# ZJU-Robotics-Lab/GEM

Measured on AMD Instinct MI355X. Metric: fused points/sec into 600x600 grid; achieved HBM GB/s vs roofline, higher is better.
Workload: dtype f32

## Files before the change

gem_amd/build.py:

```python
from __future__ import annotations

import os
import shutil
import subprocess
from pathlib import Path

ROOT = Path(__file__).resolve().parent
CSRC = ROOT / "csrc"
LIBDIR = ROOT / "lib"
LIB = LIBDIR / "libgem_hip.so"

SOURCES = [CSRC / "gem_kernels.hip", CSRC / "gem_frame_lean.hip", CSRC / "gem_sort.hip", CSRC / "gem_capi.cpp", CSRC / "gem_capi_core.cpp", CSRC / "gem_capi_pipeline.cpp", CSRC / "gem_capi_comm.cpp",
           CSRC / "gem_clean.hip", CSRC / "gem_capi_clean.cpp", CSRC / "gem_local.hip", CSRC / "gem_capi_local.cpp",
           CSRC / "gem_voxel.hip", CSRC / "gem_capi_voxel.cpp", CSRC / "gem_global.hip", CSRC / "gem_capi_global.cpp",
           CSRC / "gem_compose.hip", CSRC / "gem_capi_compose.cpp", CSRC / "gem_costmap.hip", CSRC / "gem_capi_costmap.cpp",
           CSRC / "gem_octree.hip", CSRC / "gem_capi_octree.cpp", CSRC / "gem_depth.hip", CSRC / "gem_capi_depth.cpp",
           CSRC / "gem_history.hip", CSRC / "gem_capi_history.cpp",
           CSRC / "gem_footprint.hip", CSRC / "gem_capi_footprint.cpp", CSRC / "gem_inflate.hip", CSRC / "gem_capi_inflate.cpp",
           CSRC / "gem_mapgrid.hip", CSRC / "gem_capi_mapgrid.cpp", CSRC / "gem_critics.hip", CSRC / "gem_capi_critics.cpp",
           CSRC / "gem_trajgen.hip", CSRC / "gem_capi_trajgen.cpp", CSRC / "gem_navplan.hip", CSRC / "gem_capi_navplan.cpp",
           CSRC / "gem_frontier.hip", CSRC / "gem_capi_frontier.cpp", CSRC / "gem_obstacle.hip", CSRC / "gem_capi_obstacle.cpp"]
HEADERS = [CSRC / "gem_device.hpp", CSRC / "gem_kernels.hpp", CSRC / "gem_frame_lean.hpp", CSRC / "gem_frame_tile.hpp", CSRC / "gem_frame_sort.hpp", CSRC / "gem_wave.hpp", CSRC / "gem_compact.hpp", CSRC / "gem_transport.hpp", CSRC / "gem_hostcopy.hpp", CSRC / "gem_capi_internal.hpp", CSRC / "gem_plan.hpp", CSRC / "gem_clean.hpp", CSRC / "gem_local.hpp", CSRC / "gem_voxel.hpp", CSRC / "gem_global.hpp", CSRC / "gem_compose.hpp", CSRC / "gem_costmap.hpp", CSRC / "gem_lsd.hpp", CSRC / "gem_octree.hpp", CSRC / "gem_depth.hpp", CSRC / "gem_history.hpp", CSRC / "gem_footprint.hpp", CSRC / "gem_inflate.hpp", CSRC / "gem_mapgrid.hpp", CSRC / "gem_score_device.hpp", CSRC / "gem_critics.hpp", CSRC / "gem_trajgen.hpp", CSRC / "gem_sincos.hpp",
           CSRC / "gem_navplan.hpp", CSRC / "gem_navpath.hpp", CSRC / "gem_frontier.hpp", CSRC / "gem_costmap_host.hpp", CSRC / "gem_rounds.hpp", CSRC / "gem_tile_round.hpp", CSRC / "gem_obstacle.hpp", ROOT.parent / "include" / "gem_hip_frontier.h", ROOT.parent / "include" / "gem_hip_obstacle.h",
           ROOT.parent / "include" / "gem_hip_debug.h", ROOT.parent / "include" / "gem_hip.h", ROOT.parent / "include" / "gem_hip_history.h",
           ROOT.parent / "include" / "gem_hip_footprint.h", ROOT.parent / "include" / "gem_hip_inflate.h", ROOT.parent / "include" / "gem_hip_mapgrid.h",
           ROOT.parent / "include" / "gem_hip_critics.h", ROOT.parent / "include" / "gem_hip_trajgen.h", ROOT.parent / "include" / "gem_hip_navplan.h"]

FLAGS = [
    "--offload-arch=gfx950", "-O3", *(["-g"] if os.environ.get("GEM_DEBUG_BUILD") else []), "-std=c++17", "-ffp-contract=off", "-fPIC", "-shared",
    "-Wno-unused-value", "-Wno-unused-result",
    *os.environ.get("GEM_BUILD_DEFINES", "").split(),
]

SOURCE_FLAGS = {
    "gem_frame_lean.hip": ["-mllvm", "-amdgpu-kernarg-preload-count=14"],
}


def compile_flags(src: Path, extra=()) -> list:
    return [f for f in FLAGS if f != "-shared"] + list(extra) + SOURCE_FLAGS.get(src.name, [])


def flag_line(extra=()) -> str:
    own = "".join(f" [{name}: {' '.join(fl)}]" for name, fl in sorted(SOURCE_FLAGS.items()))
    return " ".join(compile_flags(Path("-"), extra)) + own


def hipcc_path() -> str:
    for cand in (os.environ.get("HIPCC"), shutil.which("hipcc"), "/opt/rocm/bin/hipcc"):
        if cand and os.path.exists(cand):
            return cand
    raise RuntimeError("hipcc not found (need ROCm to build libgem_hip.so)")


def is_stale() -> bool:
    if not LIB.exists():
        return True
    t = LIB.stat().st_mtime
    return any(p.stat().st_mtime > t for p in SOURCES + HEADERS)


def _stale(target: Path, deps) -> bool:
    if not target.exists():
        return True
    t = target.stat().st_mtime
    return any(p.stat().st_mtime > t for p in deps)


def build(force: bool = False, verbose: bool = False) -> Path:
    if not force and not is_stale():
        return LIB
    LIBDIR.mkdir(exist_ok=True)
    objdir = LIBDIR / "obj"
    objdir.mkdir(exist_ok=True)
    rocm = os.environ.get("ROCM_PATH", "/opt/rocm")
    tag = objdir / ".flags"
    line = flag_line()
    if not tag.exists() or tag.read_text() != line:
        force = True
    jobs = []
    for src in SOURCES:
        obj = objdir / (src.stem + ".o")
        if force or _stale(obj, [src] + HEADERS):
            cmd = [hipcc_path(), *compile_flags(src), "-c", str(src), "-o", str(obj)]
            if verbose:
                print(" ".join(cmd))
            jobs.append((src, subprocess.Popen(cmd, stdout=subprocess.PIPE, stderr=subprocess.STDOUT, text=True)))
    errors = []
    for src, proc in jobs:
        out, _ = proc.communicate()
        if proc.returncode != 0:
            errors.append(f"{src.name}: hipcc failed ({proc.returncode}):\n{out}")
    if errors:
        raise RuntimeError("\n".join(errors))
    tag.write_text(line)
    cmd = [hipcc_path(), "--offload-arch=gfx950", "-shared", "-fPIC", *[str(objdir / (s.stem + ".o")) for s in SOURCES], "-o", str(LIB),
           f"-L{rocm}/lib", "-lrccl", "-pthread", f"-Wl,-rpath,{rocm}/lib"]
    if verbose:
        print(" ".join(cmd))
    res = subprocess.run(cmd, capture_output=True, text=True)
    if res.returncode != 0:
        raise RuntimeError(f"hipcc (link) failed ({res.returncode}):\n{res.stdout}\n{res.stderr}")
    return LIB


def build_variant(name: str, defines: str, verbose: bool = False) -> Path:
    out = ROOT / "lib_ab" / name
    objdir = out / "obj"
    objdir.mkdir(parents=True, exist_ok=True)
    rocm = os.environ.get("ROCM_PATH", "/opt/rocm")
    jobs = []
    for src in SOURCES:
        obj = objdir / (src.stem + ".o")
        cmd = [hipcc_path(), *compile_flags(src, defines.split()), "-c", str(src), "-o", str(obj)]
        if verbose:
            print(" ".join(cmd))
        jobs.append((src, subprocess.Popen(cmd, stdout=subprocess.PIPE, stderr=subprocess.STDOUT, text=True)))
    for src, proc in jobs:
        o, _ = proc.communicate()
        if proc.returncode != 0:
            raise RuntimeError(f"{src.name}: hipcc failed ({proc.returncode}):\n{o}")
    lib = out / "libgem_hip.so"
    res = subprocess.run([hipcc_path(), "--offload-arch=gfx950", "-shared", "-fPIC", *[str(objdir / (s.stem + ".o")) for s in SOURCES], "-o", str(lib),
                          f"-L{rocm}/lib", "-lrccl", "-pthread", f"-Wl,-rpath,{rocm}/lib"], capture_output=True, text=True)
    if res.returncode != 0:
        raise RuntimeError(f"hipcc (link) failed ({res.returncode}):\n{res.stdout}\n{res.stderr}")
    return lib


if __name__ == "__main__":
    import sys
    if len(sys.argv) >= 3 and sys.argv[1] == "--variant":
        print(build_variant(sys.argv[2], " ".join(sys.argv[3:]), verbose=True))
    else:
        print(build(force=True, verbose=True))
```

gem_amd/csrc/gem_capi.cpp:

```cpp
#include "gem_capi_internal.hpp"
#include "gem_clean.hpp"
#include "gem_costmap.hpp"

namespace gemi {

int ensure_ray(gem_handle* h)
{
    if (h->ray.p) return GEM_OK;
    const int rc = ensure(h, h->ray, ((size_t)h->cells * 2 + 4) * sizeof(uint32_t));
    if (rc) return rc;
    GEM_HIP(h, hipMemsetAsync(static_cast<uint32_t*>(h->ray.p) + h->cells, 0, 4 * sizeof(uint32_t), h->stream));
    return GEM_OK;
}

static int queue_increment(gem_handle* h, float var_update)
{
    if (!(var_update >= 0.f)) h->floor_dirty = true;
    if (h->n_pending == kMaxPending) { int rc = flush_pending(h, false); if (rc) return rc; }
    h->pending[h->n_pending++] = var_update;
    return GEM_OK;
}

static int run_batch(gem_handle* h, int n_sweeps, const gem_frame_params* params, const float4* xyzi, const long long* offsets, const float* var_updates, bool caller_device)
{
// ... 74 lines not shown
                depth = src; color = colour ? src + dp.o_color : nullptr;
            }
            slot = reinterpret_cast<float4*>(d + dp.o_xyzi);
            uint32_t* rgb = colour ? reinterpret_cast<uint32_t*>(d + dp.o_rgb) : nullptr;
            if ((rc = depth_unproject(h, ds, depth, color, fe.kind == FrontEnd::clean ? fe.clean : nullptr, slot, rgb))) return release_half(h, half, rc);
            in.xyzi = slot; in.rgb = rgb;
            break;
        }
        }
        if (fe.kind == FrontEnd::clean && c.source != AddSource::depth) {
            const hipError_t e = launch_clean_mask(h->stream, in.xyzi, slot, c.n, fe.clean->mode, fe.clean->z_min, fe.clean->z_max);
            if (e != hipSuccess) return release_half(h, half, fail(h, GEM_ERR_HIP, "launch_clean_mask", e));
            in.xyzi = slot;
        }
        if (fe.kind == FrontEnd::voxel && (rc = voxel_front(h, fe.stages, fe.n_stages, c.n, in.xyzi, in.rgb, &in.xyzi, &in.rgb)))
            return release_half(h, half, rc);
        if (c.source == AddSource::aos || c.source == AddSource::depth || fe.kind != FrontEnd::none) h->main_reads_pb = true;
    }
    return release_half(h, half, run_pipeline(h, in));
}

}

extern "C" {

int gem_abi_version(void) { return GEM_ABI_VERSION; }

const char* gem_last_error(const gem_handle* h) { return h ? h->err.c_str() : g_create_error.c_str(); }

int gem_create(const gem_map_config* cfg, gem_handle** out)
{
    if (!cfg || !out) return fail(nullptr, GEM_ERR_INVALID, "gem_create: null argument");
    *out = nullptr;
    if (cfg->length <= 0 || cfg->length > 32768 || !(cfg->resolution > 0.f))
        return fail(nullptr, GEM_ERR_INVALID, "gem_create: bad length / resolution");
    int ndev = 0;
    hipError_t e = hipGetDeviceCount(&ndev);
    if (e != hipSuccess || ndev <= 0)
        return fail(nullptr, GEM_ERR_NO_DEVICE, "gem_create: no HIP device (libgem_hip has no CPU fallback)", e);
    int dev = cfg->device;
    if (dev < 0) { if (hipGetDevice(&dev) != hipSuccess) dev = 0; }
    if (dev >= ndev) return fail(nullptr, GEM_ERR_INVALID, "gem_create: device ordinal out of range");
    if ((e = hipSetDevice(dev)) != hipSuccess) return fail(nullptr, GEM_ERR_NO_DEVICE, "hipSetDevice", e);

    gem_handle* h = new gem_handle();
    h->device = dev;
    h->cfg = *cfg;
    if (!(h->cfg.variance_floor > 0.f)) h->cfg.variance_floor = 0.0001f;
    if (!(h->cfg.mahalanobis_threshold > 0.f)) h->cfg.mahalanobis_threshold = 5.f;
    h->L = cfg->length; h->cells = cfg->length * cfg->length; h->res = cfg->resolution;
    h->row0 = 0; h->row1 = h->L;
    if (cfg->strip_rows > 0) {
        if (cfg->strip_row0 < 0 || cfg->strip_row0 + cfg->strip_rows > h->L) { delete h; return fail(nullptr, GEM_ERR_INVALID, "gem_create: bad strip"); }
        h->row0 = cfg->strip_row0; h->row1 = cfg->strip_row0 + cfg->strip_rows;
    }
    h->fuse_variant = 12;
    h->ts = 0;

    auto bail = [&](const char* what, hipError_t err) { int rc = fail(nullptr, GEM_ERR_HIP, what, err); gem_destroy(h); return rc; };
    if ((e = acquire_streams(dev, h->streams)) != hipSuccess) return bail("hipStreamCreate", e);
    h->own_stream = h->streams.s[0]; h->bin_stream = h->streams.s[1]; h->bin_stream2 = h->streams.s[2]; h->tab_stream = h->streams.s[3];
    h->stream = h->own_stream;
    if ((e = hipEventCreateWithFlags(&h->copy_done, hipEventDisableTiming)) != hipSuccess) return bail("hipEventCreate", e);
    if ((e = hipEventCreateWithFlags(&h->switch_done, hipEventDisableTiming)) != hipSuccess) return bail("hipEventCreate", e);
    for (auto& b : h->pb) {
        if ((e = hipEventCreateWithFlags(&b.bin_done, kDeviceEventFlags)) != hipSuccess) return bail("hipEventCreate", e);
        if ((e = hipEventCreateWithFlags(&b.fuse_done, kDeviceEventFlags)) != hipSuccess) return bail("hipEventCreate", e);
    }
    void* base = nullptr;
    const size_t layer_bytes = ((size_t)h->cells * 4 + 255) & ~(size_t)255;
    if ((e = hipMalloc(&base, layer_bytes * GEM_LAYER_COUNT)) != hipSuccess) return bail("hipMalloc(layers)", e);
    unsigned char* b = static_cast<unsigned char*>(base);
    h->layers.elevation = reinterpret_cast<float*>(b + layer_bytes * GEM_LAYER_ELEVATION);
    h->layers.variance  = reinterpret_cast<float*>(b + layer_bytes * GEM_LAYER_VARIANCE);
    h->layers.intensity = reinterpret_cast<float*>(b + layer_bytes * GEM_LAYER_INTENSITY);
    h->layers.traver    = reinterpret_cast<float*>(b + layer_bytes * GEM_LAYER_TRAVER);
    h->layers.lowest    = reinterpret_cast<float*>(b + layer_bytes * GEM_LAYER_LOWEST);
    h->layers.colorR    = reinterpret_cast<int*>(b + layer_bytes * GEM_LAYER_COLOR_R);
    h->layers.colorG    = reinterpret_cast<int*>(b + layer_bytes * GEM_LAYER_COLOR_G);
    h->layers.colorB    = reinterpret_cast<int*>(b + layer_bytes * GEM_LAYER_COLOR_B);
    h->layers.rough     = reinterpret_cast<float*>(b + layer_bytes * GEM_LAYER_ROUGH);
    h->layers.slope     = reinterpret_cast<float*>(b + layer_bytes * GEM_LAYER_SLOPE);
    if ((e = hipMalloc(reinterpret_cast<void**>(&h->d_counters), 2 * sizeof(unsigned long long))) != hipSuccess) return bail("hipMalloc(counters)", e);
    if ((e = launch_init(h->stream, h->layers, h->cells, 1)) != hipSuccess) return bail("k_init", e);
    if ((e = hipStreamSynchronize(h->stream)) != hipSuccess) return bail("hipStreamSynchronize", e);
    h->floor_dirty = true;
    *out = h;
    return GEM_OK;
}

void gem_destroy(gem_handle* h)
{
    if (!h) return;
    hipSetDevice(h->device);
    if (h->step.valid) {
        h->step.valid = false;
        if (h->tp_x) h->tp_x->abort();
        if (h->tp_g) h->tp_g->abort();
    }
    if (h->stream) { settle(h); hipStreamSynchronize(h->stream); }
    if (h->bin_stream) hipStreamSynchronize(h->bin_stream);
    if (h->bin_stream2) hipStreamSynchronize(h->bin_stream2);
    if (h->tab_stream) hipStreamSynchronize(h->tab_stream);
    if (h->comm_stream) hipStreamSynchronize(h->comm_stream);
    if (h->gather_stream) hipStreamSynchronize(h->gather_stream);
    h->tp_g.reset(); h->tp_x.reset();
    release_comm_stream(h->device, h->comm_stream);
    release_comm_stream(h->device, h->gather_stream);
    for (hipEvent_t e : {h->ev_sorted, h->ev_exchanged, h->ev_bounds[0], h->ev_bounds[1], h->ev_walked[0], h->ev_walked[1], h->ev_vu[0], h->ev_vu[1],
                         h->ev_published[0], h->ev_published[1], h->ev_gathered[0], h->ev_gathered[1]}) if (e) hipEventDestroy(e);
    for (hipEvent_t e : h->ev_t) if (e) hipEventDestroy(e);
    fold_events(h);
    for (auto& ep : h->pool) { hipEventDestroy(ep.a); hipEventDestroy(ep.b); }
    local_free(h);
    global_free(h);
    costmap_free(h);
    history_free(h);
    octree_free(h);
    if (h->layers.elevation) hipFree(h->layers.elevation);
    if (h->d_counters) hipFree(h->d_counters);
    for (Arena* a : {&h->stage, &h->scratch, &h->dbg, &h->color, &h->ray, &h->sh_dev, &h->sh_recv_hv[0], &h->sh_recv_key[0], &h->sh_recv_rng[0],
                     &h->sh_recv_hv[1], &h->sh_recv_key[1], &h->sh_recv_rng[1], &h->sh_ranges, &h->published[0], &h->published[1],
                     &h->clean_cnt, &h->vox_state, &h->vox_hist, &h->vox_rec, &h->vox_tmp, &h->vox_out[0], &h->vox_out[1]}) if (a->p) hipFree(a->p);
    if (h->sh_host) hipHostFree(h->sh_host);
    if (h->form_seen) hipHostFree(h->form_seen);
    for (auto& b : h->pb) {
        for (Arena* a : {&b.rec, &b.srt, &b.seg, &b.flag, &b.gflag, &b.tables, &b.s_hv1, &b.s_hv2, &b.s_key1, &b.s_key2, &b.s_src1, &b.s_src2,
                         &b.s_cnt1, &b.s_cnt2, &b.s_misc, &b.s_ranges, &b.s_shard, &b.s_blkcnt}) if (a->p) hipFree(a->p);
        if (b.host_tables) hipHostFree(b.host_tables);
        if (b.tables_done) hipEventDestroy(b.tables_done);
        if (b.bin_done) hipEventDestroy(b.bin_done);
        if (b.fuse_done) hipEventDestroy(b.fuse_done);
    }
    if (h->copy_done) hipEventDestroy(h->copy_done);
    if (h->hstage) hipHostFree(h->hstage);
    for (auto& ev : h->ev_stage) if (ev) hipEventDestroy(ev);
    if (h->stage_read) hipEventDestroy(h->stage_read);
    for (auto& ev : h->ev_half) if (ev) hipEventDestroy(ev);
    if (h->switch_done) hipEventDestroy(h->switch_done);
    release_streams(h->device, h->streams);
    delete h;
}

int gem_set_stream(gem_handle* h, void* hip_stream)
{
    if (!h) return GEM_ERR_INVALID;
    std::lock_guard<std::mutex> lk(h->mu);
    hipSetDevice(h->device);
    { const int rcd = settle(h); if (rcd) return rcd; }
    GEM_HIP(h, hipStreamSynchronize(h->stream));
    if (h->bin_stream) GEM_HIP(h, hipStreamSynchronize(h->bin_stream));
    if (h->bin_stream2) GEM_HIP(h, hipStreamSynchronize(h->bin_stream2));
    h->stream = hip_stream ? static_cast<hipStream_t>(hip_stream) : h->own_stream;
    return GEM_OK;
}

int gem_wait_event(gem_handle* h, void* hip_event)
{
    if (!h || !hip_event) return GEM_ERR_INVALID;
    std::lock_guard<std::mutex> lk(h->mu);
    hipSetDevice(h->device);
    hipEvent_t ev = static_cast<hipEvent_t>(hip_event);
    GEM_HIP(h, hipStreamWaitEvent(h->stream, ev, 0));
    if (h->bin_stream) GEM_HIP(h, hipStreamWaitEvent(h->bin_stream, ev, 0));
    if (h->bin_stream2) GEM_HIP(h, hipStreamWaitEvent(h->bin_stream2, ev, 0));
    h->main_reads_pb = true;
    return GEM_OK;
}

int gem_synchronize(gem_handle* h)
{
    ApiRange api_range(h, "gem_synchronize");
    if (!h) return GEM_ERR_INVALID;
    std::lock_guard<std::mutex> lk(h->mu);
    hipSetDevice(h->device);
    { const int rcd = settle(h); if (rcd) return rcd; }
    GEM_HIP(h, hipStreamSynchronize(h->stream));
    return GEM_OK;
}

int gem_get_pose(gem_handle* h, float out_center[2], int out_start[2])
{
    if (!h) return GEM_ERR_INVALID;
    std::lock_guard<std::mutex> lk(h->mu);
    if (out_center) { out_center[0] = h->center[0]; out_center[1] = h->center[1]; }
    if (out_start) { out_start[0] = h->start[0]; out_start[1] = h->start[1]; }
    return GEM_OK;
}

int gem_move(gem_handle* h, const float position[3], float out_center[2], int out_start[2], float out_aligned_shift[2])
{
    ApiRange api_range(h, "gem_move");
    if (!h || !position) return GEM_ERR_INVALID;
    std::lock_guard<std::mutex> lk(h->mu);
    hipSetDevice(h->device);
    { const int rcd = settle(h); if (rcd) return rcd; }
    const int L = h->L; const float res = h->res;
    h->sensor_z = position[2];
    int shift[2]; float aligned[2];
    for (int i = 0; i < 2; ++i) {
        const float d = position[i] - h->center[i];
        shift[i] = static_cast<int>(static_cast<double>(d / res) + 0.5 * (d > 0 ? 1 : -1));
        aligned[i] = static_cast<float>(shift[i]) * res;
    }
    for (int i = 0; i < 2; ++i) {
        if (shift[i] != 0) {
            h->floor_dirty = true;
            if (shift[i] >= L || shift[i] <= -L) {
                GEM_HIP(h, launch_init(h->stream, h->layers, h->cells, 0));
            } else {
                const int sign = shift[i] > 0 ? 1 : -1;
                const int start_index = h->start[i] - (sign > 0 ? 1 : 0);
                const int end_index = start_index + sign - shift[i];
                const int n_cells = std::abs(shift[i]);
                int index = index_to_range(sign < 0 ? start_index : end_index, L);
                if (index + n_cells <= L) {
                    GEM_HIP(h, launch_clear_strip(h->stream, h->layers, L, index, n_cells, i == 0));
                } else {
                    const int first_n = L - index;
                    GEM_HIP(h, launch_clear_strip(h->stream, h->layers, L, index, first_n, i == 0));
                    GEM_HIP(h, launch_clear_strip(h->stream, h->layers, L, 0, n_cells - first_n, i == 0));
                }
            }
        }
        h->start[i] = index_to_range(h->start[i] - shift[i], L);
        const int p_index = static_cast<int>(roundf(h->center[i] / res));
        const int s_index = static_cast<int>(roundf(aligned[i] / res));
        h->center[i] = static_cast<float>(p_index + s_index) * res;
    }
    if (out_center) { out_center[0] = h->center[0]; out_center[1] = h->center[1]; }
    if (out_start) { out_start[0] = h->start[0]; out_start[1] = h->start[1]; }
    if (out_aligned_shift) { out_aligned_shift[0] = aligned[0]; out_aligned_shift[1] = aligned[1]; }
    return GEM_OK;
}

int gem_process_points(gem_handle* h, const gem_frame_params* p, int n, float* x, float* y, float* z,
                       const int* orig_index, int write_back_xyz,
                       int* map_index, float* var, float* x_ts, float* y_ts, float* z_ts)
{
    ApiRange api_range(h, "gem_process_points");
    if (!h || !p || n < 0 || (n > 0 && (!x || !y || !z))) return h ? fail(h, GEM_ERR_INVALID, "gem_process_points: bad argument") : GEM_ERR_INVALID;
    std::lock_guard<std::mutex> lk(h->mu);
    hipSetDevice(h->device);
    if (n == 0) return GEM_OK;
    const size_t N = (size_t)n, S = N * 4;
    int rc;
    FrameConst fc; fill_frame(h, p, fc);
    constexpr int kRange = 65536;
    const size_t SP = (S + 255) & ~(size_t)255;
    unsigned char* stg = S >= (64u << 10) ? host_stage(h, SP * 9) : nullptr;
    if (stg && (n + kRange - 1) / kRange <= gem_handle::kStageEvents) {
        { const int rcd = drain_staging(h); if (rcd) return rcd; }
        float* sx = reinterpret_cast<float*>(stg);            float* sy = reinterpret_cast<float*>(stg + SP);
        float* sz = reinterpret_cast<float*>(stg + 2 * SP);   int* sorig = reinterpret_cast<int*>(stg + 3 * SP);
        int* sidx = reinterpret_cast<int*>(stg + 4 * SP);     float* svar = reinterpret_cast<float*>(stg + 5 * SP);
        float* sxt = reinterpret_cast<float*>(stg + 6 * SP);  float* syt = reinterpret_cast<float*>(stg + 7 * SP);
        float* szt = reinterpret_cast<float*>(stg + 8 * SP);
        const int ranges = (n + kRange - 1) / kRange;
        auto out_of = [&](int c) {
            const int first = c * kRange, cnt = std::min(kRange, n - first);
            const size_t b = (size_t)cnt * 4;
            gem::CopySeg segs[8]; int ns = 0;
            if (map_index) segs[ns++] = {map_index + first, sidx + first, b};
            if (var)  segs[ns++] = {var + first, svar + first, b};
            if (x_ts) segs[ns++] = {x_ts + first, sxt + first, b};
            if (y_ts) segs[ns++] = {y_ts + first, syt + first, b};
            if (z_ts) segs[ns++] = {z_ts + first, szt + first, b};
            if (write_back_xyz) { segs[ns++] = {x + first, sx + first, b}; segs[ns++] = {y + first, sy + first, b}; segs[ns++] = {z + first, sz + first, b}; }
            gem::CopyPool::get().run(segs, ns, h->copy_threads);
        };
        for (int c = 0; c < ranges; ++c) {
            const int first = c * kRange, cnt = std::min(kRange, n - first);
            const size_t b = (size_t)cnt * 4;
            gem::CopySeg in[4] = {{sx + first, x + first, b}, {sy + first, y + first, b}, {sz + first, z + first, b}, {sorig + first, orig_index ? orig_index + first : nullptr, orig_index ? b : 0}};
            long long t0 = host_ns();
            gem::CopyPool::get().run(in, orig_index ? 4 : 3, h->copy_threads);
            long long t1 = host_ns();
            GEM_HIP(h, launch_project(h->stream, fc, first, cnt, sx + first, sy + first, sz + first, orig_index ? sorig + first : nullptr, write_back_xyz,
                                      sidx + first, svar + first, sxt + first, syt + first, szt + first));
            GEM_HIP(h, hipEventRecord(h->ev_stage[c], h->stream));
            long long t2 = host_ns();
            h->xfer_ns[0] += t1 - t0; h->xfer_ns[1] += t2 - t1;
            if (c > 0) {
                GEM_HIP(h, hipEventSynchronize(h->ev_stage[c - 1]));
                t0 = host_ns();
                out_of(c - 1);
                h->xfer_ns[3] += t0 - t2; h->xfer_ns[4] += host_ns() - t0;
            }
        }
        long long t0 = host_ns();
        GEM_HIP(h, hipEventSynchronize(h->ev_stage[ranges - 1]));
        long long t1 = host_ns();
        out_of(ranges - 1);
        h->xfer_ns[3] += t1 - t0; h->xfer_ns[4] += host_ns() - t1;
        return GEM_OK;
    }
    if ((rc = ensure(h, h->stage, stage_words_bytes(n, 9)))) return rc;
    unsigned char* d = static_cast<unsigned char*>(h->stage.p);
    float* dx = reinterpret_cast<float*>(d);           float* dy = reinterpret_cast<float*>(d + S);
    float* dz = reinterpret_cast<float*>(d + 2 * S);   int* dorig = reinterpret_cast<int*>(d + 3 * S);
    int* didx = reinterpret_cast<int*>(d + 4 * S);     float* dvar = reinterpret_cast<float*>(d + 5 * S);
    float* dxt = reinterpret_cast<float*>(d + 6 * S);  float* dyt = reinterpret_cast<float*>(d + 7 * S);
    float* dzt = reinterpret_cast<float*>(d + 8 * S);
    HostXfer up[4] = {{x, dx, S}, {y, dy, S}, {z, dz, S}, {const_cast<int*>(orig_index), dorig, S}};
    HostXfer down[8]; int nd = 0;
    if (map_index) down[nd++] = {map_index, didx, S};
    if (var)  down[nd++] = {var, dvar, S};
    if (x_ts) down[nd++] = {x_ts, dxt, S};
    if (y_ts) down[nd++] = {y_ts, dyt, S};
    if (z_ts) down[nd++] = {z_ts, dzt, S};
    if (write_back_xyz) { down[nd++] = {x, dx, S}; down[nd++] = {y, dy, S}; down[nd++] = {z, dz, S}; }
    if ((rc = upload_arrays(h, up, orig_index ? 4 : 3))) return rc;
    GEM_HIP(h, launch_project(h->stream, fc, 0, n, dx, dy, dz, orig_index ? dorig : nullptr, write_back_xyz, didx, dvar, dxt, dyt, dzt));
    if (nd) return download_arrays(h, down, nd, SP * 4);
    GEM_HIP(h, hipStreamSynchronize(h->stream));
    return GEM_OK;
}

int gem_fuse(gem_handle* h, int n, const int* index, const int* R, const int* G, const int* B,
             const float* intensity, const float* height, const float* var)
{
    ApiRange api_range(h, "gem_fuse");
    if (!h || n < 0 || (n > 0 && (!index || !height || !var))) return h ? fail(h, GEM_ERR_INVALID, "gem_fuse: bad argument") : GEM_ERR_INVALID;
    std::lock_guard<std::mutex> lk(h->mu);
    hipSetDevice(h->device);
    { const int rcs = shard_finish_locked(h); if (rcs) return rcs; }
    const bool attr = R && G && B && intensity;
    const size_t S = (size_t)n * 4;
    PassInput in; in.src = 1; in.n = n;
    int half = -1;
    if (n > 0) {
        int rc;
        const size_t P = (S + 255) & ~(size_t)255;
        if ((rc = ensure(h, h->stage, stage_words_bytes(n, 7)))) return rc;
        unsigned char* d = static_cast<unsigned char*>(h->stage.p);
        HostXfer up[7] = {{const_cast<int*>(index), d, S}, {const_cast<float*>(height), d + P, S}, {const_cast<float*>(var), d + 2 * P, S},
                          {const_cast<int*>(R), d + 3 * P, S}, {const_cast<int*>(G), d + 4 * P, S}, {const_cast<int*>(B), d + 5 * P, S},
                          {const_cast<float*>(intensity), d + 6 * P, S}};
        unsigned char* region = nullptr;
        if ((rc = upload_arrays(h, up, attr ? 7 : 3, true, &region, &half))) return rc;
        if (region) d = region;
        in.f_index = reinterpret_cast<const int*>(d); in.f_height = reinterpret_cast<const float*>(d + P);
        in.f_var = reinterpret_cast<const float*>(d + 2 * P);
        if (attr) {
            in.f_R = reinterpret_cast<const int*>(d + 3 * P); in.f_G = reinterpret_cast<const int*>(d + 4 * P);
            in.f_B = reinterpret_cast<const int*>(d + 5 * P); in.f_I = reinterpret_cast<const float*>(d + 6 * P);
        }
    }
    return release_half(h, half, run_pipeline(h, in));
}

// ... 2 lines not shown
    ApiRange api_range(h, "gem_add_device");
    if (!h || !p || n < 0 || (n > 0 && !d_xyzi)) return h ? fail(h, GEM_ERR_INVALID, "gem_add_device: bad argument") : GEM_ERR_INVALID;
    std::lock_guard<std::mutex> lk(h->mu);
    return add_cloud(h, p, {AddSource::device, n, d_xyzi, d_rgb, d_orig_index}, {});
}

int gem_add(gem_handle* h, const gem_frame_params* p, int n, const float* xyzi, const uint32_t* rgb, const int* orig_index)
{
    ApiRange api_range(h, "gem_add");
    if (!h || !p || n < 0 || (n > 0 && !xyzi)) return h ? fail(h, GEM_ERR_INVALID, "gem_add: bad argument") : GEM_ERR_INVALID;
    std::lock_guard<std::mutex> lk(h->mu);
    return add_cloud(h, p, {AddSource::host, n, xyzi, rgb, orig_index}, {});
}

int gem_add_batch(gem_handle* h, int n_sweeps, const gem_frame_params* params, const float* const* clouds, const int* counts, const float* var_updates)
{
    ApiRange api_range(h, "gem_add_batch");
    if (!h || n_sweeps <= 0 || !params || !clouds || !counts) return h ? fail(h, GEM_ERR_INVALID, "gem_add_batch: bad argument") : GEM_ERR_INVALID;
    std::lock_guard<std::mutex> lk(h->mu);
    hipSetDevice(h->device);
    { const int rcs = shard_finish_locked(h); if (rcs) return rcs; }
    std::vector<long long> offsets(n_sweeps + 1, 0);
    for (int s = 0; s < n_sweeps; ++s) {
        if (counts[s] < 0 || (counts[s] > 0 && !clouds[s])) return fail(h, GEM_ERR_INVALID, "gem_add_batch: bad sweep");
        offsets[s + 1] = offsets[s] + counts[s];
    }
    const long long N = offsets[n_sweeps];
    if (N >= (1ll << 31)) return fail(h, GEM_ERR_INVALID, "gem_add_batch: batch too large");
    int rc;
    if ((rc = ensure(h, h->stage, (size_t)N * 16 + 256))) return rc;
    unsigned char* d = static_cast<unsigned char*>(h->stage.p);
    if (N > 0) {
        std::vector<HostXfer> up;
        for (int s = 0; s < n_sweeps; ++s)
            if (counts[s] > 0) up.push_back({const_cast<float*>(clouds[s]), d + (size_t)offsets[s] * 16, (size_t)counts[s] * 16});
        size_t i0 = 0;
        while (i0 < up.size()) {
            size_t i1 = i0, bytes = 0;
            while (i1 < up.size() && (i1 == i0 || bytes + up[i1].bytes <= (64u << 20))) bytes += (up[i1++].bytes + 255) & ~(size_t)255;
            if ((rc = upload_arrays(h, up.data() + i0, (int)(i1 - i0), true))) return rc;
            i0 = i1;
        }
    }
    return run_batch(h, n_sweeps, params, reinterpret_cast<const float4*>(d), offsets.data(), var_updates, false);
}

int gem_add_aos(gem_handle* h, const gem_frame_params* p, int n, const void* points, int point_step,
                int off_x, int off_y, int off_z, int off_intensity, int off_rgb)
{
    ApiRange api_range(h, "gem_add_aos");
    if (!h || !p || n < 0 || (n > 0 && !points)) return h ? fail(h, GEM_ERR_INVALID, "gem_add_aos: bad argument") : GEM_ERR_INVALID;
    if (!aos_fields_ok(point_step, off_x, off_y, off_z, off_intensity, off_rgb))
        return fail(h, GEM_ERR_INVALID, "gem_add_aos: fields must be 4-byte aligned inside point_step");
    std::lock_guard<std::mutex> lk(h->mu);
    return add_cloud(h, p, {AddSource::aos, n, points, nullptr, nullptr, point_step, off_x, off_y, off_z, off_intensity, off_rgb}, {});
}

int gem_add_batch_device(gem_handle* h, int n_sweeps, const gem_frame_params* params, const void* d_xyzi,
                         const long long* offsets, const float* var_updates)
{
    ApiRange api_range(h, "gem_add_batch_device");
    if (!h || n_sweeps <= 0 || !params || !offsets) return h ? fail(h, GEM_ERR_INVALID, "gem_add_batch_device: bad argument") : GEM_ERR_INVALID;
    std::lock_guard<std::mutex> lk(h->mu);
    hipSetDevice(h->device);
    { const int rcs = shard_finish_locked(h); if (rcs) return rcs; }
    for (int s = 0; s < n_sweeps; ++s) if (offsets[s + 1] < offsets[s]) return fail(h, GEM_ERR_INVALID, "gem_add_batch_device: offsets not monotone");
    return run_batch(h, n_sweeps, params, static_cast<const float4*>(d_xyzi), offsets, var_updates, true);
}

int gem_mapvar_update(gem_handle* h, float var_update)
{
    ApiRange api_range(h, "gem_mapvar_update");
    if (!h) return GEM_ERR_INVALID;
    std::lock_guard<std::mutex> lk(h->mu);
    hipSetDevice(h->device);
    { const int rcs = shard_finish_locked(h); if (rcs) return rcs; }
    return queue_increment(h, var_update);
}

static void* layer_ptr(gem_handle* h, int layer)
{
    switch (layer) {
    case GEM_LAYER_ELEVATION: return h->layers.elevation;
    case GEM_LAYER_VARIANCE:  return h->layers.variance;
    case GEM_LAYER_INTENSITY: return h->layers.intensity;
    case GEM_LAYER_TRAVER:    return h->layers.traver;
    case GEM_LAYER_LOWEST:    return h->layers.lowest;
    case GEM_LAYER_COLOR_R:   return h->layers.colorR;
    case GEM_LAYER_COLOR_G:   return h->layers.colorG;
    case GEM_LAYER_COLOR_B:   return h->layers.colorB;
    case GEM_LAYER_ROUGH:     return h->layers.rough;
    case GEM_LAYER_SLOPE:     return h->layers.slope;
    default: return nullptr;
    }
}

int gem_get_layer(gem_handle* h, int layer, int layout, void* dst_host)
{
    ApiRange api_range(h, "gem_get_layer");
    if (!h || !dst_host) return GEM_ERR_INVALID;
    std::lock_guard<std::mutex> lk(h->mu);
    hipSetDevice(h->device);
    void* src = layer_ptr(h, layer);
    if (!src) return fail(h, GEM_ERR_INVALID, "gem_get_layer: bad layer");
    int rc = flush_pending(h, false);
    if (rc) return rc;
    const size_t bytes = (size_t)h->cells * 4;
    if (layout == GEM_LAYOUT_STORAGE_ROWMAJOR) {
        HostXfer down{dst_host, src, bytes};
        return download_arrays(h, &down, 1, 0);
    } else if (layout == GEM_LAYOUT_GRIDMAP_COLMAJOR_NAN) {
        if (layer == GEM_LAYER_LOWEST) return fail(h, GEM_ERR_INVALID, "gem_get_layer: the LOWEST layer is indexed by geographic cell, it has no grid_map layout");
        if ((rc = ensure(h, h->scratch, bytes))) return rc;
        const int is_int = layer >= GEM_LAYER_COLOR_R && layer <= GEM_LAYER_COLOR_B;
        GEM_HIP(h, launch_export_gridmap(h->stream, src, h->layers.elevation, static_cast<float*>(h->scratch.p), h->L, is_int));
        HostXfer down{dst_host, h->scratch.p, bytes};
        return download_arrays(h, &down, 1, 0);
    }
    return fail(h, GEM_ERR_INVALID, "gem_get_layer: bad layout");
}

int gem_set_layer(gem_handle* h, int layer, const void* src_host)
{
    if (!h || !src_host) return GEM_ERR_INVALID;
    std::lock_guard<std::mutex> lk(h->mu);
    hipSetDevice(h->device);
    void* dst = layer_ptr(h, layer);
    if (!dst) return fail(h, GEM_ERR_INVALID, "gem_set_layer: bad layer");
    int rc = flush_pending(h, false);
    if (rc) return rc;
    HostXfer up{const_cast<void*>(src_host), dst, (size_t)h->cells * 4};
    if ((rc = upload_arrays(h, &up, 1))) return rc;
    GEM_HIP(h, hipStreamSynchronize(h->stream));
    if (layer == GEM_LAYER_VARIANCE) h->floor_dirty = true;
    return GEM_OK;
}

int gem_layer_device_ptr(gem_handle* h, int layer, void** out_device_ptr)
{
    if (!h || !out_device_ptr) return GEM_ERR_INVALID;
    std::lock_guard<std::mutex> lk(h->mu);
    hipSetDevice(h->device);
    { const int rcd = flush_pending(h, false); if (rcd) return rcd; }
    *out_device_ptr = layer_ptr(h, layer);
    return *out_device_ptr ? GEM_OK : fail(h, GEM_ERR_INVALID, "gem_layer_device_ptr: bad layer");
}

int gem_map_optmove(gem_handle* h, const float opt_position[2], float height_update, float out_aligned_position[2])
{
    if (!h || !opt_position) return GEM_ERR_INVALID;
    std::lock_guard<std::mutex> lk(h->mu);
    hipSetDevice(h->device);
    { const int rcd = settle(h); if (rcd) return rcd; }
    for (int i = 0; i < 2; ++i) {
        const float d = opt_position[i] - h->center[i];
        const int shift = static_cast<int>(static_cast<double>(d / h->res) + 0.5 * (d > 0 ? 1 : -1));
        h->center[i] = h->center[i] + h->res * static_cast<float>(shift);
    }
    if (out_aligned_position) { out_aligned_position[0] = h->center[0]; out_aligned_position[1] = h->center[1]; }
    GEM_HIP(h, launch_update_height(h->stream, h->layers.elevation, h->cells, height_update));
    return GEM_OK;
}

int gem_map_closeloop(gem_handle* h, const float update_position[2], float height_update)
{
    if (!h || !update_position) return GEM_ERR_INVALID;
    std::lock_guard<std::mutex> lk(h->mu);
    hipSetDevice(h->device);
    { const int rcd = settle(h); if (rcd) return rcd; }
    for (int i = 0; i < 2; ++i) {
        const float d = update_position[i] - h->center[i];
        const int shift = static_cast<int>(static_cast<double>(d / h->res) + 0.5 * (d > 0 ? 1 : -1));
        const float aligned = static_cast<float>(shift) * h->res;
        const int p_index = static_cast<int>(roundf(h->center[i] / h->res));
        const int s_index = static_cast<int>(roundf(aligned / h->res));
        h->center[i] = static_cast<float>(p_index + s_index) * h->res;
    }
    GEM_HIP(h, launch_update_height(h->stream, h->layers.elevation, h->cells, height_update));
    return GEM_OK;
}

int gem_map_feature(gem_handle* h, float* elevation, float* variance, int* colorR, int* colorG, int* colorB,
                    float* rough, float* slope, float* traver, float* intensity)
{
    ApiRange api_range(h, "gem_map_feature");
    if (!h) return GEM_ERR_INVALID;
    std::lock_guard<std::mutex> lk(h->mu);
    hipSetDevice(h->device);
    int rc = flush_pending(h, false);
    if (rc) return rc;
    GEM_HIP(h, launch_map_feature(h->stream, h->layers.elevation, h->layers.traver, h->layers.rough, h->layers.slope,
                                  h->L, h->res, h->start[0], h->start[1], h->row0, h->row1));
    const size_t bytes = (size_t)h->cells * 4;
    struct { void* dst; const void* src; } out[9] = {
        {elevation, h->layers.elevation}, {variance, h->layers.variance}, {colorR, h->layers.colorR}, {colorG, h->layers.colorG},
        {colorB, h->layers.colorB}, {rough, h->layers.rough}, {slope, h->layers.slope}, {traver, h->layers.traver},
        {intensity, h->layers.intensity}};
    HostXfer down[9]; int nd = 0;
    for (auto& o : out) if (o.dst) down[nd++] = {o.dst, const_cast<void*>(o.src), bytes};
    return nd ? download_arrays(h, down, nd, 0) : GEM_OK;
}

int gem_show(gem_handle* h, double map_length, double resolution, const double position[2],
             float* visual, float* points_xyz, unsigned char* points_rgb, int* out_count, unsigned char* image_bgr)
{
    ApiRange api_range(h, "gem_show");
    if (!h) return GEM_ERR_INVALID;
    std::lock_guard<std::mutex> lk(h->mu);
    hipSetDevice(h->device);
    int rc = flush_pending(h, false);
    if (rc) return rc;
    const size_t cells = (size_t)h->cells, blocks = (cells + 1023) / 1024;
    const size_t o_cnt = 0, o_total = o_cnt + blocks * 4, o_vis = (o_total + 4 + 255) & ~(size_t)255, o_xyz = o_vis + cells * 36,
                 o_rgb = o_xyz + cells * 12, o_img = (o_rgb + cells * 3 + 255) & ~(size_t)255, total_bytes = o_img + cells * 3;
    if ((rc = ensure(h, h->scratch, total_bytes))) return rc;
    unsigned char* d = static_cast<unsigned char*>(h->scratch.p);
    const double res = resolution > 0.0 ? resolution : (double)h->res;
    const double len = map_length > 0.0 ? map_length : (double)h->L * res;
    const double px = position ? position[0] : (double)h->center[0], py = position ? position[1] : (double)h->center[1];
    if (image_bgr) GEM_HIP(h, hipMemsetAsync(d + o_img, 0, cells * 3, h->stream));
    GEM_HIP(h, launch_show(h->stream, h->layers, h->L, h->start[0], h->start[1], len, res, px, py, reinterpret_cast<uint32_t*>(d + o_cnt),
                           visual ? reinterpret_cast<float*>(d + o_vis) : nullptr, (points_xyz || points_rgb) ? reinterpret_cast<float*>(d + o_xyz) : nullptr,
                           points_rgb ? d + o_rgb : nullptr, image_bgr ? d + o_img : nullptr, reinterpret_cast<uint32_t*>(d + o_total)));
    uint32_t n = 0;
    {
        HostXfer down[3] = {{&n, d + o_total, 4}, {nullptr, nullptr, 0}, {nullptr, nullptr, 0}};
        int nd = 1;
        if (visual) down[nd++] = {visual, d + o_vis, cells * 36};
        if (image_bgr) down[nd++] = {image_bgr, d + o_img, cells * 3};
        if ((rc = download_arrays(h, down, nd, 0))) return rc;
    }
    if (n) {
        HostXfer down[2]; int nd = 0;
        if (points_xyz) down[nd++] = {points_xyz, d + o_xyz, (size_t)n * 12};
        if (points_rgb) down[nd++] = {points_rgb, d + o_rgb, (size_t)n * 3};
        if (nd && (rc = download_arrays(h, down, nd, 0))) return rc;
    }
    if (out_count) *out_count = (int)n;
    return GEM_OK;
}

static int colorize_device(gem_handle* h, const gem_camera* cam, int n, float* d_xyzi, const unsigned char* d_image, size_t stride, uint32_t* d_rgb)
{
    if (!cam || n < 0 || (n > 0 && (!d_xyzi || !d_image || !d_rgb))) return fail(h, GEM_ERR_INVALID, "gem_colorize: null argument");
    if (cam->width <= 0 || cam->height <= 0 || (long long)cam->width * cam->height > (1ll << 26))
        return fail(h, GEM_ERR_INVALID, "gem_colorize: image size out of range");
    if (stride == 0) stride = (size_t)cam->width * 3;
    if (stride < (size_t)cam->width * 3) return fail(h, GEM_ERR_INVALID, "gem_colorize: row stride below width * 3");
    if (n == 0) return GEM_OK;
    const long long pixels = (long long)cam->width * cam->height;
    SortArgs sa{};
    sa.id_bits = std::max(2, ceil_log2((int)std::min<long long>(pixels, 1ll << 30)));
    sa.n_passes = sa.id_bits <= 10 ? 1 : (sa.id_bits <= 20 ? 2 : 3);
    int shift = 0;
    for (int i = 0; i < sa.n_passes; ++i) {
        const int left = sa.n_passes - i;
        const int bits = i == sa.n_passes - 1 ? sa.id_bits - shift : (sa.id_bits - shift + left - 1) / left;
        sa.dshift[i] = shift; sa.dbits[i] = bits;
        sa.dbins[i] = i == sa.n_passes - 1 ? (int)((pixels - 1) >> shift) + 1 : 1 << bits;
        shift += bits;
    }
    const size_t N = (size_t)n, NC = (N + kSortChunkRecords - 1) / kSortChunkRecords;
    size_t o = 0;
    auto take = [&](size_t bytes) { const size_t at = o; o = (o + bytes + 255) & ~(size_t)255; return at; };
    const SortPlan sp = sort_plan(sa.n_passes, sa.dbins, n, NC, NC, 1, false, 0, false);
    const size_t o_hv1 = take(sp.hv), o_hv2 = take(sp.hv), o_key1 = take(sp.key), o_key2 = take(sp.key);
    const size_t o_cnt1 = take(sp.cnt1), o_cnt2 = take(sp.cnt2), o_misc = take(sp.misc);
    const size_t o_first = take((size_t)pixels * 4), o_pix = take(N * 4), o_link = take(N * 4);
    int rc;
    if ((rc = ensure(h, h->color, o))) return rc;
    unsigned char* d = static_cast<unsigned char*>(h->color.p);
    sa.n_sweeps = 1; sa.n = n; sa.xyzi = reinterpret_cast<const float4*>(d_xyzi);
    for (int k = 0; k < 12; ++k) sa.cam.P[k] = cam->lidar_to_image[k];
    sa.cam.width = cam->width; sa.cam.height = cam->height;
    sa.tiles_per_row = 1; sa.T = 1; sa.n_chunks1 = (int)NC; sa.chunk = kSortChunkRecords;
    bind_sort_buffers(sp, sa.n_passes, {d + o_hv1, d + o_hv2, d + o_key1, d + o_key2, nullptr, nullptr, d + o_cnt1, d + o_cnt2, d + o_misc}, sa);
    sa.odd_flag = nullptr;
    const LaunchEvents ev[9] = {};
    GEM_HIP(h, hipMemsetAsync(d + o_first, 0xff, (size_t)pixels * 4, h->stream));
    GEM_HIP(h, hipMemsetAsync(d + o_pix, 0xff, N * 4, h->stream));
    GEM_HIP(h, launch_sort(h->stream, sa, 3, false, ev));
    const bool final_b = (sa.n_passes & 1) != 0;
    ColorArgs ca{};
    ca.key = final_b ? sa.key_b : sa.key_a; ca.hv = final_b ? sa.hv_b : sa.hv_a; ca.total = sa.total;
    ca.first = reinterpret_cast<uint32_t*>(d + o_first); ca.pix = reinterpret_cast<uint32_t*>(d + o_pix); ca.link = reinterpret_cast<uint32_t*>(d + o_link);
    ca.n = n; ca.width = cam->width; ca.height = cam->height; ca.image = d_image; ca.stride = stride;
    ca.xyzi = reinterpret_cast<float4*>(d_xyzi); ca.rgb = d_rgb;
    GEM_HIP(h, launch_colorize(h->stream, ca));
    return GEM_OK;
}

int gem_colorize_device(gem_handle* h, const gem_camera* cam, int n, float* d_xyzi, const unsigned char* d_image_bgr, size_t row_stride,
                        uint32_t* d_rgb)
{
    ApiRange api_range(h, "gem_colorize_device");
    if (!h) return GEM_ERR_INVALID;
    std::lock_guard<std::mutex> lk(h->mu);
    hipSetDevice(h->device);
    return colorize_device(h, cam, n, d_xyzi, d_image_bgr, row_stride, d_rgb);
}

int gem_colorize(gem_handle* h, const gem_camera* cam, int n, float* xyzi, const unsigned char* image_bgr, size_t row_stride, uint32_t* rgb)
{
    ApiRange api_range(h, "gem_colorize");
    if (!h) return GEM_ERR_INVALID;
    std::lock_guard<std::mutex> lk(h->mu);
    hipSetDevice(h->device);
    if (!cam || n < 0 || (n > 0 && (!xyzi || !image_bgr || !rgb))) return fail(h, GEM_ERR_INVALID, "gem_colorize: null argument");
    if (cam->width <= 0 || cam->height <= 0) return fail(h, GEM_ERR_INVALID, "gem_colorize: image size out of range");
    if (n == 0) return GEM_OK;
    if (row_stride == 0) row_stride = (size_t)cam->width * 3;
    { const int rcd = settle(h); if (rcd) return rcd; }
    const size_t N = (size_t)n, b_xyzi = (N * 16 + 255) & ~(size_t)255, b_rgb = (N * 4 + 255) & ~(size_t)255, b_img = row_stride * cam->height;
    int rc;
    if ((rc = ensure(h, h->stage, b_xyzi + b_rgb + b_img))) return rc;
    unsigned char* d = static_cast<unsigned char*>(h->stage.p);
    HostXfer up[2] = {{xyzi, d, N * 16}, {const_cast<unsigned char*>(image_bgr), d + b_xyzi + b_rgb, b_img}};
    if ((rc = upload_arrays(h, up, 2))) return rc;
    if ((rc = colorize_device(h, cam, n, reinterpret_cast<float*>(d), d + b_xyzi + b_rgb, row_stride, reinterpret_cast<uint32_t*>(d + b_xyzi)))) return rc;
    HostXfer down[2] = {{xyzi, d, N * 16}, {rgb, d + b_xyzi, N * 4}};
    return download_arrays(h, down, 2, 0);
}

int gem_set_lowest_tracking(gem_handle* h, int enabled)
{
    if (!h) return GEM_ERR_INVALID;
    std::lock_guard<std::mutex> lk(h->mu);
    hipSetDevice(h->device);
    { const int rcd = settle(h); if (rcd) return rcd; }
    h->track_lowest = enabled != 0;
    return GEM_OK;
}

int gem_raytracing(gem_handle* h)
{
    ApiRange api_range(h, "gem_raytracing");
    if (!h) return GEM_ERR_INVALID;
    std::lock_guard<std::mutex> lk(h->mu);
    hipSetDevice(h->device);
    if (h->row0 != 0 || h->row1 != h->L) return fail(h, GEM_ERR_INVALID, "gem_raytracing: not available on a row-strip handle");
    int rc = flush_pending(h, false);
    if (rc) return rc;
    if ((rc = ensure_ray(h))) return rc;
    uint32_t* list = static_cast<uint32_t*>(h->ray.p);
    GEM_HIP(h, launch_raytracing(h->stream, h->layers, h->L, h->start[0], h->start[1], h->sensor_z, h->cfg.obstacle_threshold,
                                 h->row0, h->row1, list, list + h->cells, (int)(h->ray_calls++ & 1u), reinterpret_cast<float*>(list + h->cells + 4), h->ray_depth, h->ray_lanes));
    return GEM_OK;
}

int gem_set_timing(gem_handle* h, int enabled)
{
    if (!h) return GEM_ERR_INVALID;
    std::lock_guard<std::mutex> lk(h->mu);
    hipSetDevice(h->device);
    { const int rcd = settle(h); if (rcd) return rcd; }
    h->timing = enabled != 0;
    h->step_timed = h->timing && h->tp_x != nullptr && h->nranks > 1;
    return GEM_OK;
}

int gem_set_counting(gem_handle* h, int enabled)
{
    if (!h) return GEM_ERR_INVALID;
    std::lock_guard<std::mutex> lk(h->mu);
    hipSetDevice(h->device);
    { const int rcd = settle(h); if (rcd) return rcd; }
    h->counting = enabled != 0;
    return GEM_OK;
}

int gem_get_stats(gem_handle* h, gem_stats* out, int reset)
{
    if (!h || !out) return GEM_ERR_INVALID;
    std::lock_guard<std::mutex> lk(h->mu);
    hipSetDevice(h->device);
    { const int rcd = settle(h); if (rcd) return rcd; }
    GEM_HIP(h, hipStreamSynchronize(h->stream));
    fold_events(h);
    if (h->counting) {
        unsigned long long c[2] = {0, 0};
        GEM_HIP(h, hipMemcpy(c, h->d_counters, sizeof(c), hipMemcpyDeviceToHost));
        h->stats.points_binned = (long long)c[0];
        h->stats.cells_touched = (long long)c[1];
    }
    *out = h->stats;
    if (reset) { const long long pin = h->stats.points_in; h->stats = gem_stats{}; h->stats.points_in = pin; }
    return GEM_OK;
}

int gem_debug_set(gem_handle* h, const char* key, long long value)
{
    if (!h || !key) return GEM_ERR_INVALID;
    std::lock_guard<std::mutex> lk(h->mu);
    hipSetDevice(h->device);
    { const int rcd = settle(h); if (rcd) return rcd; }
    const std::string k(key);
    if (k == "fuse_variant")            { if (value < 10 || value > 12) return fail(h, GEM_ERR_INVALID, "fuse_variant: 10..12"); h->fuse_variant = (int)value; }
    else if (k == "tile_shift")         { if (value != 0 && value != 4 && value != 5) return fail(h, GEM_ERR_INVALID, "tile_shift: 0, 4 or 5"); h->ts = (int)value; }
    else if (k == "defer")              h->defer = value != 0;
    else if (k == "walk_always_wait")   h->walk_always_wait = value != 0;
    else if (k == "defer_walk")         { const int rcw = flush_walk(h); if (rcw) return rcw; h->defer_walk = value != 0; }
    else if (k == "dense_min")          { if (value < 0 || value > 0xffffffffll) return fail(h, GEM_ERR_INVALID, "dense_min: 0 .. 2^32 - 1"); h->dense_min = (unsigned)value; }
    else if (k == "dbg_sweep")          h->dbg_sweep = (int)value;
    else if (k == "dbg_frame")          h->dbg_frame = value != 0;
    else if (k == "frame_lean")         { if (value < 0 || value > 2) return fail(h, GEM_ERR_INVALID, "frame_lean: 0 (generic), 1 (lean) or 2 (the host picks)"); h->frame_lean = (int)value; }
    else if (k == "overlap")            h->overlap = value != 0;
    else if (k == "overlap_min_points") { if (value < 0) return fail(h, GEM_ERR_INVALID, "overlap_min_points: >= 0"); h->overlap_min_points = value; h->sort_overlap_min_points = value; }
    else if (k == "sort_path")          h->sort_path = value != 0;
    else if (k == "sort_min_points")    { if (value < 0) return fail(h, GEM_ERR_INVALID, "sort_min_points: >= 0"); h->sort_min_points = value; h->sort_min_points_batch = value; }
    else if (k == "walk_permute")       h->walk_permute = value != 0;
    else if (k == "trace")              h->trace = value != 0;
    else if (k == "stream_roles") {
        if (h->stream != h->own_stream) return fail(h, GEM_ERR_INVALID, "stream_roles: caller-provided stream in use");
        for (hipStream_t st : {h->own_stream, h->bin_stream, h->bin_stream2, h->tab_stream}) hipStreamSynchronize(st);
        const hipStream_t cur[4] = {h->own_stream, h->bin_stream, h->bin_stream2, h->tab_stream};
        const int d[4] = {(int)(value / 1000 % 10), (int)(value / 100 % 10), (int)(value / 10 % 10), (int)(value % 10)};
        bool seen[4] = {false, false, false, false};
        for (int i = 0; i < 4; ++i) { if (d[i] < 0 || d[i] > 3 || seen[d[i]]) return fail(h, GEM_ERR_INVALID, "stream_roles: not a permutation of 0123"); seen[d[i]] = true; }
        h->own_stream = cur[d[0]]; h->bin_stream = cur[d[1]]; h->bin_stream2 = cur[d[2]]; h->tab_stream = cur[d[3]];
        h->stream = h->own_stream;
    }
    else if (k == "sort_ring")          { if (value < 2 || value > 4) return fail(h, GEM_ERR_INVALID, "sort_ring: 2..4"); h->sort_ring = (int)value; }
    else if (k == "sort_streams")       { if (value != 1 && value != 2) return fail(h, GEM_ERR_INVALID, "sort_streams: 1 or 2"); h->sort_streams = (int)value; }
    else if (k == "sort_passes")        { if (value < 0 || value > 3) return fail(h, GEM_ERR_INVALID, "sort_passes: 0..3"); h->sort_passes = (int)value; }
    else if (k == "rank_by_ballot")     h->rank_by_ballot = value != 0;
    else if (k == "lane_sort")          h->lane_sort = value != 0;
    else if (k == "plain_loop")         h->plain_loop = value != 0;
    else if (k == "cache_tables")       h->cache_tables = value != 0;
    else if (k == "light_fast")         h->light_fast = value != 0;
    else if (k == "walk_lds_pad")       { if (value < 0 || value > 100 * 1024) return fail(h, GEM_ERR_INVALID, "walk_lds_pad: 0 .. 102400 bytes"); h->walk_lds_pad = (int)value; }
    else if (k == "ride_events")        { if (value < 0 || value > 1) return fail(h, GEM_ERR_INVALID, "ride_events: 0 or 1"); h->ride_events = value != 0; }
    else if (k == "roctx")              { if (value != 0 && !roctx_load()) return fail(h, GEM_ERR_INVALID, "roctx: no ROCm marker library (librocprofiler-sdk-roctx / libroctx64) to load"); h->roctx = value != 0; }
    else if (k == "download_groups")    { if (value < 1 || value > 14) return fail(h, GEM_ERR_INVALID, "download_groups: 1 .. 14"); h->download_groups = (int)value; }
    else if (k == "copy_threads")       { if (value < 0 || value > gem::CopyPool::kMaxThreads) return fail(h, GEM_ERR_INVALID, "copy_threads: 0 (the runtime's pageable path) .. 16"); h->copy_threads = (int)value; }
    else if (k == "fuse_count")         { if (value < 0 || value > 2) return fail(h, GEM_ERR_INVALID, "fuse_count: 0 (never), 1 (small passes) or 2 (always)"); h->fuse_count = (int)value; }
    else if (k == "sort_chunk")         { if (value != 0 && value != kSortChunkSmall && value != kSortChunkRecords) return fail(h, GEM_ERR_INVALID, "sort_chunk: 0 (by pass), 1024 or 4096"); h->sort_chunk = (int)value; }
    else if (k == "walk_prio")          { if (value < 0 || value > (1 << 30)) return fail(h, GEM_ERR_INVALID, "walk_prio: 0 (off) or a record count"); h->walk_prio = (int)value; }
    else if (k == "blk_batch")          { if (value != 0 && value != 512 && value != 2048) return fail(h, GEM_ERR_INVALID, "blk_batch: 0 (by pass), 512 or 2048"); h->blk_batch = (int)value; }
    else if (k == "few_bins")           { if (value < -1 || value > 64) return fail(h, GEM_ERR_INVALID, "few_bins: -1 (one ballot per digit bit), 0 (by pass), 1..64"); h->few_bins = (int)value; }
    else if (k == "ray_depth")          { if (value != 4 && value != 8) return fail(h, GEM_ERR_INVALID, "ray_depth: 4 or 8"); h->ray_depth = (int)value; }
    else if (k == "ray_lanes")          { if (value != 1 && value != 4 && value != 8 && value != 16) return fail(h, GEM_ERR_INVALID, "ray_lanes: 1, 4, 8 or 16"); h->ray_lanes = (int)value; }
    else if (k == "fast_laser")         h->fast_laser = value != 0;
    else if (k == "sort_form")          { if (value < 0 || value > 2) return fail(h, GEM_ERR_INVALID, "sort_form: 0 (by pass), 1 (cell-sorted), 2 (block-sorted)"); h->sort_form = (int)value; }
    else if (k == "history_cull")       { if (value < 0 || value > 1) return fail(h, GEM_ERR_INVALID, "history_cull: 0 or 1"); h->history_cull = value != 0; }
    else if (k == "obstacle_direct")    { if (value < 0 || value > 1) return fail(h, GEM_ERR_INVALID, "obstacle_direct: 0 or 1"); h->obstacle_direct = value != 0; }
    else if (k == "nav_chunk")          { if (value < 0 || value > (1 << 20)) return fail(h, GEM_ERR_INVALID, "nav_chunk: 0 (tiles_x + tiles_y) or 1 .. 2^20 rounds"); h->nav_chunk = (int)value; }
    else if (k == "front_chunk")        { if (value < 0 || value > (1 << 20)) return fail(h, GEM_ERR_INVALID, "front_chunk: 0 (tiles_x + tiles_y) or 1 .. 2^20 rounds"); h->front_chunk = (int)value; }
    else return fail(h, GEM_ERR_INVALID, "gem_debug_set: unknown key");
    return GEM_OK;
}

int gem_debug_get(gem_handle* h, const char* key, long long* out)
{
    if (!h || !key || !out) return GEM_ERR_INVALID;
    std::lock_guard<std::mutex> lk(h->mu);
    const std::string k(key);
    if (k == "arena_allocations") *out = h->arena_allocations;
    else if (k == "hstage_allocations") *out = h->hstage_allocations;
    else if (k == "copy_threads") *out = h->copy_threads;
    else if (k == "xfer_upload_memcpy_ns") *out = h->xfer_ns[0];
    else if (k == "xfer_upload_enqueue_ns") *out = h->xfer_ns[1];
    else if (k == "xfer_download_enqueue_ns") *out = h->xfer_ns[2];
    else if (k == "xfer_download_wait_ns") *out = h->xfer_ns[3];
    else if (k == "xfer_download_memcpy_ns") *out = h->xfer_ns[4];
    else if (k == "sort_fallbacks") *out = h->sort_fallbacks;
    else if (k == "compose_far_points") *out = h->compose.far_points;
    else if (k == "compose_sum_ns") *out = h->compose.sum_ns;
    else if (k == "walks_unwaited") *out = h->walks_unwaited;
    else if (k == "frame_lean_launches") *out = h->frame_lean_launches;
    else if (k == "frame_generic_launches") *out = h->frame_generic_launches;
    else if (k == "frame_form_seen") *out = h->form_seen ? (long long)*static_cast<volatile const uint32_t*>(h->form_seen) : 0;
    else if (k == "walks_left") *out = h->walks_left;
    else if (k == "history_cull") *out = h->history_cull ? 1 : 0;
    else if (k == "obstacle_direct") *out = h->obstacle_direct ? 1 : 0;
    else if (k == "nav_chunk") *out = h->nav_chunk;
    else if (k == "front_chunk") *out = h->front_chunk;
    else if (k == "history_blocks") *out = h->history.enabled ? cost_mark_blocks(h->history.len) : 0;
    else if (k == "history_blocks_culled") { hipSetDevice(h->device); return history_blocks_culled(h, out); }
    else if (k == "step_pending") *out = h->step.valid ? 1 : 0;
    else if (k == "step_exchange_bytes_out") *out = h->xbytes_out;
    else if (k == "step_exchange_bytes_in") *out = h->xbytes_in;
    else if (k == "gather_bytes_out") *out = h->gbytes_out;
    else if (k == "gather_bytes_in") *out = h->gbytes_in;
    else if (k.rfind("step_", 0) == 0) {
        int a = -1, b = -1;
        if (k == "step_exchange_ns") { a = 2; b = 3; }
        else if (k == "step_walk_ns") { a = 4; b = 5; }
        else if (k == "step_publish_ns") { a = 6; b = 7; }
        else if (k == "step_gather_ns") { a = 7; b = 8; }
        else if (k == "step_exchange_to_walk_ns") { a = 3; b = 4; }
        else return fail(h, GEM_ERR_INVALID, "gem_debug_get: unknown key");
        hipSetDevice(h->device);
        float ms = 0.f;
        if (!h->ev_t[a] || hipEventElapsedTime(&ms, h->ev_t[a], h->ev_t[b]) != hipSuccess) { (void)hipGetLastError(); *out = -(1ll << 62); return GEM_OK; }
        *out = (long long)((double)ms * 1e6);
    }
    else return fail(h, GEM_ERR_INVALID, "gem_debug_get: unknown key");
    return GEM_OK;
}

int gem_debug_fuse_stamps(gem_handle* h, int enable, unsigned long long* out, int max_tiles)
{
    if (!h) return GEM_ERR_INVALID;
    std::lock_guard<std::mutex> lk(h->mu);
    hipSetDevice(h->device);
    { const int rcd = settle(h); if (rcd) return rcd; }
    h->dbg_on = enable != 0;
    if (out && h->dbg.p) {
        GEM_HIP(h, hipStreamSynchronize(h->stream));
        const int rows = h->dbg_rows ? h->dbg_rows : h->T;
        const int n = max_tiles < rows ? max_tiles : rows;
        GEM_HIP(h, hipMemcpy(out, h->dbg.p, (size_t)n * 16 * 8, hipMemcpyDeviceToHost));
        return n;
    }
    return 0;
}

int gem_comm_unique_id(void* out_128_bytes)
{
    if (!out_128_bytes) return GEM_ERR_INVALID;
    static_assert(sizeof(ncclUniqueId) == 128, "ncclUniqueId is 128 bytes");
    ncclUniqueId id;
    if (ncclGetUniqueId(&id) != ncclSuccess) return GEM_ERR_COMM;
    memcpy(out_128_bytes, &id, sizeof(id));
    return GEM_OK;
}

}
```

gem_amd/csrc/gem_capi_comm.cpp:

```cpp
#include "gem_capi_internal.hpp"


namespace gemi {

int comm_attach(gem_handle* h, int nranks, int rank, bool tile_strips)
{
    h->nranks = nranks; h->rank = rank; h->tile_strips = tile_strips;
    if (!h->comm_stream) {
        GEM_HIP(h, acquire_comm_stream(h->device, &h->comm_stream));
        GEM_HIP(h, acquire_comm_stream(h->device, &h->gather_stream));
        for (hipEvent_t* e : {&h->ev_sorted, &h->ev_exchanged, &h->ev_bounds[0], &h->ev_bounds[1], &h->ev_walked[0], &h->ev_walked[1], &h->ev_vu[0], &h->ev_vu[1],
                              &h->ev_published[0], &h->ev_published[1], &h->ev_gathered[0], &h->ev_gathered[1]})
            GEM_HIP(h, hipEventCreateWithFlags(e, hipEventDisableTiming));
        for (hipEvent_t& e : h->ev_t) GEM_HIP(h, hipEventCreate(&e));
    }
    const int tile_rows = (h->L + 31) / 32;
    for (int k = 0; k <= nranks; ++k)
        h->strip_row[k] = tile_strips ? std::min(h->L, 32 * (int)((long long)tile_rows * k / nranks)) : (int)((long long)h->L * k / nranks);
    h->row0 = h->strip_row[rank]; h->row1 = h->strip_row[rank + 1];
    if (nranks > 1)
        for (int g = 0; g < 2; ++g) { const int rc = ensure(h, h->published[g], (size_t)(h->row1 - h->row0) * h->L * 4 * 6 + 256); if (rc) return rc; }
    return GEM_OK;
}

int comm_init_common(gem_handle* h, const void* unique_id_128_bytes, int nranks, int rank, bool tile_strips)
{
    if (!h || !unique_id_128_bytes || nranks <= 0 || nranks > kMaxRanks || rank < 0 || rank >= nranks) return GEM_ERR_INVALID;
    std::lock_guard<std::mutex> lk(h->mu);
    hipSetDevice(h->device);
    { const int rcd = settle(h); if (rcd) return rcd; }
    if (h->tp_x) return fail(h, GEM_ERR_COMM, "gem_comm_init: the handle already joined a communicator");
    ncclUniqueId id;
    memcpy(&id, unique_id_128_bytes, sizeof(id));
    std::unique_ptr<RcclTransport> x(new RcclTransport()), g(new RcclTransport());
    ncclResult_t r = ncclCommInitRank(&x->comm, nranks, id, rank);
    if (r != ncclSuccess) { x->comm = nullptr; return fail(h, GEM_ERR_COMM, ncclGetErrorString(r)); }
    r = ncclCommSplit(x->comm, 0, rank, &g->comm, nullptr);
    if (r != ncclSuccess || !g->comm) { g->comm = x->comm; g->owns = false; }
    x->nranks = g->nranks = nranks; x->rank = g->rank = rank;
    h->tp_x = std::move(x); h->tp_g = std::move(g);
    return comm_attach(h, nranks, rank, tile_strips);
}

}

extern "C" {

int gem_comm_init(gem_handle* h, const void* unique_id_128_bytes, int nranks, int rank)
{
    return comm_init_common(h, unique_id_128_bytes, nranks, rank, false);
}

int gem_comm_init_tiles(gem_handle* h, const void* unique_id_128_bytes, int nranks, int rank)
{
    return comm_init_common(h, unique_id_128_bytes, nranks, rank, true);
}

int gem_comm_init_loopback(gem_handle* h, long long world_id, int nranks, int rank, int tile_strips)
{
    if (!h || nranks <= 0 || nranks > kMaxRanks || rank < 0 || rank >= nranks) return GEM_ERR_INVALID;
    std::lock_guard<std::mutex> lk(h->mu);
    hipSetDevice(h->device);
    { const int rcd = settle(h); if (rcd) return rcd; }
    if (h->tp_x) return fail(h, GEM_ERR_COMM, "gem_comm_init_loopback: the handle already joined a communicator");
    std::string why;
    std::shared_ptr<LoopWorld> w = loop_world(world_id, nranks, &why);
    if (!w) return fail(h, GEM_ERR_COMM, why.c_str());
    std::unique_ptr<LoopbackTransport> x(new LoopbackTransport()), g(new LoopbackTransport());
    if (!x->join(w, 0, rank)) return fail(h, GEM_ERR_COMM, x->err.c_str());
    if (!g->join(w, 1, rank)) return fail(h, GEM_ERR_COMM, g->err.c_str());
    h->tp_x = std::move(x); h->tp_g = std::move(g);
    return comm_attach(h, nranks, rank, tile_strips != 0);
}

int gem_get_strip(gem_handle* h, int* out_row0, int* out_row1)
{
    if (!h) return GEM_ERR_INVALID;
    std::lock_guard<std::mutex> lk(h->mu);
    if (out_row0) *out_row0 = h->row0;
    if (out_row1) *out_row1 = h->row1;
    return GEM_OK;
}

}

namespace gemi {

int gather_layers_locked(gem_handle* h, int with_attributes)
{
    const int W = h->nranks;
    if (W == 1) return GEM_OK;
    const int nl = with_attributes ? 6 : 2;
    void* ptrs[6] = {h->layers.elevation, h->layers.variance, h->layers.intensity, h->layers.colorR, h->layers.colorG, h->layers.colorB};
    const size_t own = (size_t)(h->strip_row[h->rank + 1] - h->strip_row[h->rank]) * h->L;
    const int g = (int)(h->gather_seq++ & 1u);
    int rc;
    if ((rc = ensure(h, h->published[g], own * 4 * 6 + 256))) return step_abort(h, rc);
    unsigned char* pub = static_cast<unsigned char*>(h->published[g].p);
    if (h->gathered_recorded[g]) GEM_HIP_STEP(h, hipStreamWaitEvent(h->stream, h->ev_gathered[g], 0));
    if (h->step_timed) GEM_HIP_STEP(h, hipEventRecord(h->ev_t[6], h->stream));
    if (own)
        for (int l = 0; l < nl; ++l)
            GEM_HIP_STEP(h, hipMemcpyAsync(pub + (size_t)l * own * 4, static_cast<unsigned char*>(ptrs[l]) + (size_t)h->strip_row[h->rank] * h->L * 4, own * 4,
                                      hipMemcpyDeviceToDevice, h->stream));
    GEM_HIP_STEP(h, hipEventRecord(h->ev_published[g], h->stream));
    GEM_HIP_STEP(h, hipStreamWaitEvent(h->gather_stream, h->ev_published[g], 0));
    if (h->step_timed) GEM_HIP_STEP(h, hipEventRecord(h->ev_t[7], h->gather_stream));
    Transport& tp = *h->tp_g;
    bool ok = tp.group_begin();
    h->gbytes_out = h->gbytes_in = 0;
    for (int p = 0; p < W && ok; ++p) {
        if (p == h->rank) continue;
        const size_t theirs = (size_t)(h->strip_row[p + 1] - h->strip_row[p]) * h->L;
        h->gbytes_out += 4ll * (long long)own * nl; h->gbytes_in += 4ll * (long long)theirs * nl;
        for (int l = 0; l < nl && ok; ++l) {
            if (own) ok = tp.send(pub + (size_t)l * own * 4, own, p, h->gather_stream);
            if (ok && theirs) ok = tp.recv(static_cast<unsigned char*>(ptrs[l]) + (size_t)h->strip_row[p] * h->L * 4, theirs, p, h->gather_stream);
        }
    }
    ok = tp.group_end(h->gather_stream) && ok;
    if (!ok) return step_abort(h, fail(h, GEM_ERR_COMM, tp.err.c_str()));
    if (h->step_timed) GEM_HIP_STEP(h, hipEventRecord(h->ev_t[8], h->gather_stream));
    GEM_HIP_STEP(h, hipEventRecord(h->ev_gathered[g], h->gather_stream));
    h->gathered_recorded[g] = true;
    h->gather_outstanding[g] = true;
    return GEM_OK;
}

}

extern "C" {

int gem_allgather_layers(gem_handle* h, int with_attributes)
{
    ApiRange api_range(h, "gem_allgather_layers");
    if (!h) return GEM_ERR_INVALID;
    std::lock_guard<std::mutex> lk(h->mu);
    hipSetDevice(h->device);
    if (!h->tp_g) return fail(h, GEM_ERR_COMM, "gem_allgather_layers: gem_comm_init not called");
    if (h->step.valid) {
        h->step.gather = true; h->step.gather_attrs = with_attributes;
        return GEM_OK;
    }
    { const int rc = flush_local(h); if (rc) return rc; }
    if (h->n_pending) { const int rc = flush_pending(h, false); if (rc) return rc; }
    return gather_layers_locked(h, with_attributes);
}

}

namespace gemi {

int ensure_shard_tables(gem_handle* h, size_t blocks)
{
    if (!h->sh_host) GEM_HIP(h, hipHostMalloc(&h->sh_host, kShardHostBytes, hipHostMallocDefault));
    int rc = ensure(h, h->sh_dev, kShardDevBytes);
    return rc ? rc : ensure(h, h->sh_ranges, blocks * sizeof(uint2));
}

int shard_checks(gem_handle* h, int n_global_sweeps, SortGeometry* geo)
{
    if (h->track_lowest) return fail(h, GEM_ERR_INVALID, "sharded path: lowest tracking is not supported (use the replicated path)");
    *geo = sort_geometry(h, n_global_sweeps, true);
    if (!geo->ok) return fail(h, GEM_ERR_INVALID, "sharded path: map or batch too large for the record key");
    return GEM_OK;
}

int shard_sort_locked(gem_handle* h, int n_local_sweeps, const gem_frame_params* params, const void* d_xyzi, const long long* offsets,
                             int first_global_sweep, int n_global_sweeps, int first_point_in_sweep, int nstrips, const int* strip_rows,
                             uint32_t* out_bounds, const void** out_d_hv, const void** out_d_key, const void** out_d_ranges, bool bounds_stay_on_device)
{
    if (first_point_in_sweep < 0) return fail(h, GEM_ERR_INVALID, "gem_shard_sort_device: negative first_point_in_sweep");
// ... 295 lines not shown
```

gem_amd/csrc/gem_capi_core.cpp:

```cpp
#include "gem_capi_internal.hpp"

#include <cfloat>
#include <dlfcn.h>

namespace gemi {

thread_local std::string g_create_error;

namespace {
typedef int (*roctx_push_fn)(const char*);
typedef int (*roctx_pop_fn)();
std::once_flag g_roctx_once;
roctx_push_fn g_roctx_push = nullptr;
roctx_pop_fn g_roctx_pop = nullptr;
}

bool roctx_load()
{
    std::call_once(g_roctx_once, [] {
        for (const char* lib : {"librocprofiler-sdk-roctx.so", "librocprofiler-sdk-roctx.so.1", "libroctx64.so", "libroctx64.so.4"}) {
            void* so = dlopen(lib, RTLD_NOW | RTLD_GLOBAL);
            if (!so) continue;
            g_roctx_push = reinterpret_cast<roctx_push_fn>(dlsym(so, "roctxRangePushA"));
            g_roctx_pop = reinterpret_cast<roctx_pop_fn>(dlsym(so, "roctxRangePop"));
            if (g_roctx_push && g_roctx_pop) return;
            g_roctx_push = nullptr; g_roctx_pop = nullptr;
        }
    });
    return g_roctx_push != nullptr;
}
void roctx_push(const char* name) { if (g_roctx_push) g_roctx_push(name); }
void roctx_pop() { if (g_roctx_pop) g_roctx_pop(); }
ApiRange::ApiRange(const gem_handle* h, const char* name) : on(h && h->roctx && g_roctx_push != nullptr) { if (on) roctx_push(name); }

int fail(gem_handle* h, int code, const char* what, hipError_t e)
{
    char buf[512];
    if (e != hipSuccess) snprintf(buf, sizeof(buf), "%s: %s", what, hipGetErrorString(e));
    else snprintf(buf, sizeof(buf), "%s", what);
    if (h) h->err = buf; else g_create_error = buf;
    return code;
}

int ensure(gem_handle* h, Arena& a, size_t bytes)
{
    if (bytes <= a.cap) return GEM_OK;
    GEM_HIP(h, hipStreamSynchronize(h->stream));
    if (h->bin_stream) GEM_HIP(h, hipStreamSynchronize(h->bin_stream));
    if (h->bin_stream2) GEM_HIP(h, hipStreamSynchronize(h->bin_stream2));
    if (h->tab_stream) GEM_HIP(h, hipStreamSynchronize(h->tab_stream));
    if (h->comm_stream) GEM_HIP(h, hipStreamSynchronize(h->comm_stream));
    if (h->gather_stream) GEM_HIP(h, hipStreamSynchronize(h->gather_stream));
    if (a.p) GEM_HIP(h, hipFree(a.p));
    a.p = nullptr; a.cap = 0;
    size_t want = bytes + bytes / 4 + 4096;
    hipError_t e = hipMalloc(&a.p, want);
    if (e != hipSuccess) return fail(h, GEM_ERR_NOMEM, "hipMalloc(arena)", e);
    a.cap = want;
    ++h->arena_allocations;
    return GEM_OK;
}

int ensure_zeroed(gem_handle* h, Arena& a, size_t bytes)
{
    if (bytes <= a.cap) return GEM_OK;
    const int rc = ensure(h, a, bytes);
    if (rc) return rc;
    GEM_HIP(h, hipMemsetAsync(a.p, 0, a.cap, h->stream));
    GEM_HIP(h, hipStreamSynchronize(h->stream));
    return GEM_OK;
}

unsigned char* host_stage(gem_handle* h, size_t bytes)
{
    if (h->copy_threads <= 0 || h->hstage_failed || bytes > h->hstage_max) return nullptr;
    if (bytes > h->hstage_cap) {
        if (h->hstage) {
            if (hipStreamSynchronize(h->stream) != hipSuccess) return nullptr;
            h->stage_read_pending = false; h->half_pending[0] = h->half_pending[1] = false;
            hipHostFree(h->hstage); h->hstage = nullptr; h->hstage_cap = 0;
        }
        const size_t want = bytes + bytes / 4 + 4096;
        if (hipHostMalloc(&h->hstage, want, hipHostMallocDefault) != hipSuccess) { (void)hipGetLastError(); h->hstage = nullptr; h->hstage_failed = true; return nullptr; }
        h->hstage_cap = want;
        ++h->hstage_allocations;
    }
    for (auto& ev : h->ev_stage) if (!ev && hipEventCreateWithFlags(&ev, hipEventDisableTiming) != hipSuccess) { ev = nullptr; return nullptr; }
    if (!h->stage_read && hipEventCreateWithFlags(&h->stage_read, hipEventDisableTiming) != hipSuccess) { h->stage_read = nullptr; return nullptr; }
    return static_cast<unsigned char*>(h->hstage);
}

int drain_staging(gem_handle* h)
{
    for (int p = 0; p < 2; ++p) if (h->half_pending[p]) { GEM_HIP(h, hipEventSynchronize(h->ev_half[p])); h->half_pending[p] = false; }
    if (h->stage_read_pending) { GEM_HIP(h, hipEventSynchronize(h->stage_read)); h->stage_read_pending = false; }
    return GEM_OK;
}

int upload_arrays(gem_handle* h, const HostXfer* x, int n, bool defer_ok, unsigned char** zero_copy_region, int* zero_copy_half)
{
    if (zero_copy_region) *zero_copy_region = nullptr;
    size_t total = 0;
    for (int i = 0; i < n; ++i) total += (x[i].bytes + 255) & ~(size_t)255;
    unsigned char* stg = (total >= (128u << 10) && total < (16u << 20)) ? host_stage(h, defer_ok ? 2 * total + 512 : total) : nullptr;
    if (!stg) {
        for (int i = 0; i < n; ++i) if (x[i].bytes) GEM_HIP(h, hipMemcpyAsync(x[i].dev, x[i].host, x[i].bytes, hipMemcpyHostToDevice, h->stream));
        GEM_HIP(h, hipEventRecord(h->copy_done, h->stream));
        GEM_HIP(h, hipEventSynchronize(h->copy_done));
        return GEM_OK;
    }
    int par = -1;
    if (defer_ok) {
        for (auto& ev : h->ev_half) if (!ev) GEM_HIP(h, hipEventCreateWithFlags(&ev, hipEventDisableTiming));
        if (h->stage_read_pending) { GEM_HIP(h, hipEventSynchronize(h->stage_read)); h->stage_read_pending = false; }
        par = (int)(h->stage_par++ & 1u);
        const size_t half_at = (h->hstage_cap / 2) & ~(size_t)255;
        if (h->half_pending[par]) { GEM_HIP(h, hipEventSynchronize(h->ev_half[par])); h->half_pending[par] = false; }
        if (half_at < total || h->hstage_cap - half_at < total) { const int rcd = drain_staging(h); if (rcd) return rcd; par = 0; }
        else stg += (size_t)par * half_at;
        if (zero_copy_region) {
            size_t off = 0;
            gem::CopySeg segs[16]; int ns = 0;
            const long long t0 = host_ns();
            for (int i = 0; i < n; ++i) {
                if (x[i].bytes) segs[ns++] = {stg + off, x[i].host, x[i].bytes};
                off += (x[i].bytes + 255) & ~(size_t)255;
                if (ns == 16 || i == n - 1) { if (ns) gem::CopyPool::get().run(segs, ns, h->copy_threads); ns = 0; }
            }
            h->xfer_ns[0] += host_ns() - t0;
            *zero_copy_region = stg; *zero_copy_half = par;
            return GEM_OK;
        }
    } else { const int rcd = drain_staging(h); if (rcd) return rcd; }
    auto pad = [](size_t b) { return (b + 255) & ~(size_t)255; };
    size_t off = 0;
    for (int i = 0; i < n;) {
        int e = i + 1;
        size_t len = pad(x[i].bytes);
        while (e < n && e - i < 16 && static_cast<unsigned char*>(x[e].dev) == static_cast<unsigned char*>(x[i].dev) + len) len += pad(x[e++].bytes);
        const size_t real_len = len - pad(x[e - 1].bytes) + x[e - 1].bytes;
        const size_t group = pad(len <= (8u << 20) ? (par >= 0 ? len : std::max<size_t>(len / 2, 512u << 10)) : (4u << 20));
        for (size_t a = 0; a < len; a += group) {
            const size_t b = std::min(len, a + group);
            gem::CopySeg segs[16]; int ns = 0;
            size_t m_off = 0;
            for (int m = i; m < e; ++m) {
                const size_t lo = std::max(a, m_off), hi = std::min(b, m_off + x[m].bytes);
                if (lo < hi) segs[ns++] = {stg + off + lo, static_cast<const unsigned char*>(x[m].host) + (lo - m_off), hi - lo};
                m_off += pad(x[m].bytes);
            }
            const long long t0 = host_ns();
            gem::CopyPool::get().run(segs, ns, h->copy_threads);
            const long long t1 = host_ns();
            const size_t b_real = std::min(b, real_len);
            if (a < b_real) GEM_HIP(h, hipMemcpyAsync(static_cast<unsigned char*>(x[i].dev) + a, stg + off + a, b_real - a, hipMemcpyHostToDevice, h->stream));
            h->xfer_ns[0] += t1 - t0; h->xfer_ns[1] += host_ns() - t1;
        }
        off += len;
        i = e;
    }
    if (par >= 0) {
        GEM_HIP(h, hipEventRecord(h->ev_half[par], h->stream));
        h->half_pending[par] = true;
        h->main_reads_pb = true;
        return GEM_OK;
    }
    GEM_HIP(h, hipEventRecord(h->stage_read, h->stream));
    GEM_HIP(h, hipEventSynchronize(h->stage_read));
    h->stage_read_pending = false;
    return GEM_OK;
}

CloudLayout cloud_layout(long long n, bool rgb, bool orig)
{
    const size_t S = (size_t)n * 4, P = (S + 255) & ~(size_t)255, P4 = (S * 4 + 255) & ~(size_t)255;
    CloudLayout l;
    l.rgb = P4;
    l.orig = P4 + (rgb ? P : 0);
    l.bytes = l.orig + (orig ? P : 0);
    return l;
}

int stage_cloud(gem_handle* h, long long n, const float* xyzi, const uint32_t* rgb, const int* orig, StagedCloud& out)
{
    const CloudLayout l = cloud_layout(n, rgb, orig);
    int rc;
    if ((rc = ensure(h, h->stage, l.bytes))) return rc;
    unsigned char* d = static_cast<unsigned char*>(h->stage.p);
    const size_t S = (size_t)n * 4;
    HostXfer up[3] = {{const_cast<float*>(xyzi), d, S * 4}};
    int nu = 1;
    if (rgb) up[nu++] = {const_cast<uint32_t*>(rgb), d + l.rgb, S};
    if (orig) up[nu++] = {const_cast<int*>(orig), d + l.orig, S};
    unsigned char* region = nullptr;
    out.half = -1;
    if ((rc = upload_arrays(h, up, nu, true, &region, &out.half))) return rc;
    const unsigned char* src = region ? region : d;
    out.xyzi = reinterpret_cast<const float4*>(src);
    out.rgb = rgb ? reinterpret_cast<const uint32_t*>(src + l.rgb) : nullptr;
    out.orig = orig ? reinterpret_cast<const int*>(src + l.orig) : nullptr;
    out.arena_xyzi = reinterpret_cast<float4*>(d);
    return GEM_OK;
}

int release_half(gem_handle* h, int half, int rc)
{
    if (half < 0) return rc;
    const hipError_t e = hipEventRecord(h->ev_half[half], h->stream);
    if (e != hipSuccess && rc == GEM_OK) rc = fail(h, GEM_ERR_HIP, "hipEventRecord(staging half)", e);
    h->half_pending[half] = true;
    return rc;
}

float to_float_rn(double v)
{
    const double lim = (double)FLT_MAX + std::ldexp(1.0, 103);
    if (v >= lim) return INFINITY;
    if (v <= -lim) return -INFINITY;
    return static_cast<float>(v);
}

int download_arrays(gem_handle* h, const HostXfer* x, int n, size_t stage_off)
{
    size_t total = 0;
    for (int i = 0; i < n; ++i) total += (x[i].bytes + 255) & ~(size_t)255;
    stage_off = (stage_off + 255) & ~(size_t)255;
    { const int rcd = drain_staging(h); if (rcd) return rcd; }
    unsigned char* stg = total >= (128u << 10) ? host_stage(h, stage_off + total) : nullptr;
    if (!stg) {
        for (int i = 0; i < n; ++i) if (x[i].bytes) GEM_HIP(h, hipMemcpyAsync(x[i].host, x[i].dev, x[i].bytes, hipMemcpyDeviceToHost, h->stream));
        GEM_HIP(h, hipStreamSynchronize(h->stream));
        h->stage_read_pending = false;
        return GEM_OK;
    }
    stg += stage_off;
    const long long t_begin = host_ns();
    const size_t n_groups = (size_t)std::max(1, std::min(h->download_groups, (int)gem_handle::kStageEvents - 10));
    size_t group = std::max<size_t>(n_groups > 8 ? (256u << 10) : (768u << 10), (total + n_groups - 1) / n_groups);
    group = (group + 255) & ~(size_t)255;
    gem::CopySeg segs[gem_handle::kStageEvents][kCopyListMax];
    int nseg[gem_handle::kStageEvents] = {};
    int ng = 0;
    {
        CopyList cl; cl.n = 0;
        size_t in_group = 0, off = 0;
        auto flush = [&]() -> int {
            if (!cl.n) return GEM_OK;
            if (ng == gem_handle::kStageEvents) return fail(h, GEM_ERR_INVALID, "download_arrays: too many groups");
            GEM_HIP(h, launch_copy_list(h->stream, cl));
            GEM_HIP(h, hipEventRecord(h->ev_stage[ng], h->stream));
            nseg[ng++] = cl.n; cl.n = 0; in_group = 0;
            return GEM_OK;
        };
        for (int i = 0; i < n; ++i) {
            for (size_t o = 0; o < x[i].bytes;) {
                const size_t b = std::min(x[i].bytes - o, group - in_group);
                cl.piece[cl.n] = {stg + off + o, static_cast<const unsigned char*>(x[i].dev) + o, b};
                segs[ng][cl.n] = {static_cast<unsigned char*>(x[i].host) + o, stg + off + o, b};
                ++cl.n; in_group += b; o += b;
                if (in_group >= group || cl.n == kCopyListMax) { const int rcf = flush(); if (rcf) return rcf; }
            }
            off += (x[i].bytes + 255) & ~(size_t)255;
        }
        { const int rcf = flush(); if (rcf) return rcf; }
    }
    long long t0 = host_ns();
    h->xfer_ns[2] += t0 - t_begin;
    for (int g = 0; g < ng; ++g) {
        GEM_HIP(h, hipEventSynchronize(h->ev_stage[g]));
        const long long t1 = host_ns();
        gem::CopyPool::get().run(segs[g], nseg[g], h->copy_threads);
        const long long t2 = host_ns();
        h->xfer_ns[3] += t1 - t0; h->xfer_ns[4] += t2 - t1; t0 = t2;
    }
    h->stage_read_pending = false;
    return GEM_OK;
}

void fill_frame(const gem_handle* h, const gem_frame_params* p, FrameConst& f)
{
    memset(&f, 0, sizeof(f));
    if (p) {
        for (int i = 0; i < 12; ++i) f.T[i] = p->T[i];
        f.lower = p->lower; f.upper = p->upper;
        f.lower_f = (float)p->lower; if ((double)f.lower_f > p->lower) f.lower_f = nextafterf(f.lower_f, -INFINITY);
        f.upper_f = (float)p->upper; if ((double)f.upper_f < p->upper) f.upper_f = nextafterf(f.upper_f, INFINITY);
        for (int i = 0; i < 8; ++i) f.sp[i] = p->sensor_params[i];
        for (int i = 0; i < 3; ++i) { f.Js[i] = p->sensor_jacobian[i]; f.P[i] = p->P_mul_C_BM_T[i]; }
        for (int i = 0; i < 9; ++i) { f.Q[i] = p->rotation_variance[i]; f.C[i] = p->C_SB_T[i]; f.Bs[i] = p->B_r_BS_skew[i]; }
        f.filter_on = p->filter.enabled;
        f.fbx = p->filter.box_x; f.fby = p->filter.box_y; f.fband = p->filter.band_y; f.fplane = p->filter.plane_y;
        f.model = p->sensor_model;
        f.orig_width = p->original_width;
    }
    f.cx = h->center[0]; f.cy = h->center[1];
    f.sx = h->start[0];  f.sy = h->start[1];
    f.L = h->L; f.res = h->res;
    f.row0 = h->row0; f.row1 = h->row1;
    f.beam_a = (float)f.sp[1]; f.beam_c = (float)f.sp[2];
    f.t2 = 0.f; f.fast_laser = 0;
    if (p && f.model == GEM_MODEL_LASER && h->fast_laser) {
        const float min_r = (float)f.sp[0], vn = min_r * min_r;
        const float c0 = f.Js[0] * 0.0f, c1 = f.Js[1] * 0.0f, c2 = f.Js[2] * vn;
        const float b2 = c0 + (c1 + c2);
        const float t2 = b2 * f.Js[2];
        auto small = [](float v, float bound) { return std::isfinite(v) && std::fabs(v) <= bound; };
        bool ok = t2 > 0.f && std::isfinite(t2) && small(f.beam_a, 1e6f) && small(f.beam_c, 1e6f);
        for (int i = 0; i < 9; ++i) ok = ok && f.Q[i] == 0.0f && small(f.C[i], 1e6f) && small(f.Bs[i], 1e6f);
        for (int i = 0; i < 3; ++i) ok = ok && small(f.Js[i], 1e6f) && small(f.P[i], 1e6f);
        for (int i = 0; i < 3 && ok; ++i)
            for (int j = i; j < 3; ++j) {
                double d = 0.0;
                for (int k = 0; k < 3; ++k) d += (double)f.T[4 * i + k] * (double)f.T[4 * j + k];
                ok = ok && std::fabs(d - (i == j ? 1.0 : 0.0)) <= 0.01;
            }
        for (int i = 0; i < 3; ++i) ok = ok && small(f.T[4 * i + 3], 1e9f);
        ok = ok && std::isfinite(f.lower) && std::isfinite(f.upper) && std::fabs(f.lower) <= 1e9 && std::fabs(f.upper) <= 1e9;
        ok = ok && small(f.cx, 1e9f) && small(f.cy, 1e9f) && (double)f.L * (double)f.res <= 1e9;
        ok = ok && f.res >= 9.5367431640625e-7f && f.res <= 1048576.0f && f.L >= 2;
        if (ok) { f.t2 = t2; f.fast_laser = 1; }
    }
}

hipEvent_t get_event(gem_handle* h)
{
    hipEvent_t e = nullptr;
    hipEventCreate(&e);
    (void)h;
    return e;
}

void fold_events(gem_handle* h)
{
    for (auto& ep : h->events) {
        float ms = 0.f;
        if (hipEventSynchronize(ep.b) == hipSuccess && hipEventElapsedTime(&ms, ep.a, ep.b) == hipSuccess) {
            if (ep.kind == 0)      { h->stats.ms_bin += ms; h->stats.launches_bin++; }
            else if (ep.kind == 1) { h->stats.ms_fuse += ms; h->stats.launches_fuse++; }
            else if (ep.kind == 2) { h->stats.ms_frame += ms; h->stats.launches_frame++; }
            else if (ep.kind == 9) { h->stats.ms_walk += ms; h->stats.launches_walk++; }
            else                   { h->stats.ms_sort[ep.kind - 3] += ms; if (ep.kind == 3) h->stats.launches_sort++; }
        }
        else (void)hipGetLastError();
        h->pool.push_back(ep);
    }
    h->events.clear();
}

bool frame_launch_lean(gem_handle* h, bool fused_lean, bool bin_fast)
{
    const bool seen = h->form_seen && *static_cast<volatile const uint32_t*>(h->form_seen) != 0u;
    const bool lean = fused_lean && bin_fast && (h->frame_lean == 1 || (h->frame_lean == 2 && !seen));
    ++(lean ? h->frame_lean_launches : h->frame_generic_launches);
    return lean;
}

int flush_deferred(gem_handle* h)
{
    if (!h->deferred.valid) return GEM_OK;
    h->deferred.valid = false;
    h->main_reads_pb = true;
    if (h->dbg_frame) h->deferred.fa.dbg = nullptr;
    Timed t(h, 1);
    gem::BinArgs no_bin{};
    const bool lean = frame_launch_lean(h, h->deferred.lean_binned, true);
    GEM_HIP(h, launch_frame(h->stream, h->deferred.fa, no_bin, h->deferred.attr, lean, t.events()));
    return GEM_OK;
}

int flush_walk(gem_handle* h)
{
    if (!h->dwalk.valid) return GEM_OK;
    h->dwalk.valid = false;
    gem_handle::PassBuffers& pb = h->pb[h->dwalk.slot];
    if (!h->walk_always_wait && hipEventQuery(pb.bin_done) == hipSuccess) ++h->walks_unwaited;
    else { (void)hipGetLastError(); GEM_HIP(h, hipStreamWaitEvent(h->stream, pb.bin_done, 0)); }
    {
        Timed t(h, 9);
        GEM_HIP(h, h->dwalk.block_form ? launch_block_walk(h->stream, h->dwalk.wa, h->dwalk.attr, t.events()) : launch_walk(h->stream, h->dwalk.wa, h->dwalk.attr, t.events()));
    }
    GEM_HIP(h, hipEventRecord(pb.fuse_done, h->stream)); pb.fuse_recorded = true;
    return GEM_OK;
}

int flush_local(gem_handle* h)
{
    { const int rc = flush_walk(h); if (rc) return rc; }
    return flush_deferred(h);
}

int wait_gather(gem_handle* h)
{
    for (int g = 0; g < 2; ++g) {
        if (!h->gather_outstanding[g]) continue;
        GEM_HIP(h, hipStreamWaitEvent(h->stream, h->ev_gathered[g], 0));
        h->gather_outstanding[g] = false;
    }
    return GEM_OK;
}

int settle(gem_handle* h)
{
    { const int rc = shard_finish_locked(h); if (rc) return rc; }
    { const int rc = flush_local(h); if (rc) return rc; }
    return wait_gather(h);
}

int flush_pending(gem_handle* h, bool with_floor)
{
    { const int rc = settle(h); if (rc) return rc; }
    if (h->n_pending == 0 && !with_floor) return GEM_OK;
    GEM_HIP(h, launch_dense_variance(h->stream, h->layers.variance, h->cells, h->n_pending, h->pending, with_floor ? 1 : 0,
                                     h->cfg.variance_floor));
    h->n_pending = 0;
    if (with_floor) h->floor_dirty = false;
    return GEM_OK;
}

int index_to_range(int index, int L)
{
    if (index < 0) index += ((-index / L) + 1) * L;
    return index % L;
}

static std::mutex g_stream_pool_mu;
static std::vector<StreamSet> g_stream_pool[64];

hipError_t acquire_streams(int device, StreamSet& out)
{
    {
        std::lock_guard<std::mutex> lk(g_stream_pool_mu);
        if (device >= 0 && device < 64 && !g_stream_pool[device].empty()) {
            out = g_stream_pool[device].back(); g_stream_pool[device].pop_back();
            return hipSuccess;
        }
    }
    int prio_lo = 0, prio_hi = 0;
    if (hipDeviceGetStreamPriorityRange(&prio_lo, &prio_hi) != hipSuccess) { prio_lo = prio_hi = 0; (void)hipGetLastError(); }
    for (int i = 0; i < 4; ++i) {
        const hipError_t e = i == 0 ? hipStreamCreateWithPriority(&out.s[i], hipStreamNonBlocking, prio_hi)
                                    : hipStreamCreateWithFlags(&out.s[i], hipStreamNonBlocking);
        if (e != hipSuccess) { for (int j = 0; j < i; ++j) hipStreamDestroy(out.s[j]); out = StreamSet{}; return e; }
    }
    return hipSuccess;
}

static std::vector<hipStream_t> g_comm_pool[64];

hipError_t acquire_comm_stream(int device, hipStream_t* out)
{
    {
        std::lock_guard<std::mutex> lk(g_stream_pool_mu);
        if (device >= 0 && device < 64 && !g_comm_pool[device].empty()) { *out = g_comm_pool[device].back(); g_comm_pool[device].pop_back(); return hipSuccess; }
    }
    return hipStreamCreateWithFlags(out, hipStreamNonBlocking);
}

void release_comm_stream(int device, hipStream_t st)
{
    if (!st) return;
    hipStreamSynchronize(st);
    if (device < 0 || device >= 64) { hipStreamDestroy(st); return; }
    std::lock_guard<std::mutex> lk(g_stream_pool_mu);
    g_comm_pool[device].push_back(st);
}

void release_streams(int device, const StreamSet& set)
{
    if (!set.s[0]) return;
    for (hipStream_t st : set.s) hipStreamSynchronize(st);
    if (device < 0 || device >= 64) { for (hipStream_t st : set.s) hipStreamDestroy(st); return; }
    std::lock_guard<std::mutex> lk(g_stream_pool_mu);
    g_stream_pool[device].push_back(set);
}

}
```

gem_amd/csrc/gem_capi_internal.hpp:

```cpp
#pragma once

#include "../../include/gem_hip.h"
#include "../../include/gem_hip_debug.h"
#include "gem_kernels.hpp"
#include "gem_plan.hpp"
#include "gem_hostcopy.hpp"
#include "gem_transport.hpp"

#include <hip/hip_runtime.h>
#include <rccl/rccl.h>

#include <chrono>
#include <cmath>
#include <cstdio>
#include <cstdlib>
#include <cstring>
#include <memory>
#include <mutex>
#include <string>
#include <vector>

using namespace gem;

namespace gem { struct CriticsArgs; struct FootSpec; struct CostGeom; }

namespace gemi {

extern thread_local std::string g_create_error;

struct Arena {
    void*  p = nullptr;
    size_t cap = 0;
};

struct EventPair { hipEvent_t a, b; int kind; };

}

using namespace gemi;

struct StreamSet { hipStream_t s[4] = {nullptr, nullptr, nullptr, nullptr}; };

struct gem_handle {
    std::mutex  mu;
    std::string err;
    int         device = 0;
    hipStream_t own_stream = nullptr;
    StreamSet streams;
    hipStream_t stream = nullptr;
    gem_map_config cfg{};
    int   L = 0, cells = 0;
    float res = 0.f;
    LayerPtrs layers{};
    float center[2] = {0.f, 0.f};
    int   start[2] = {0, 0};
    float sensor_z = 0.f;
    int   row0 = 0, row1 = 0;
    int   ts = 0, T = 0;

    Arena stage;
    struct PassBuffers {
        Arena rec, srt, seg, flag, gflag;
        Arena bkt, bcnt, spill, fctl;
        Arena s_hv1, s_hv2, s_key1, s_key2, s_src1, s_src2, s_cnt1, s_cnt2, s_misc;
        bool blkcnt_dirty = false;
        Arena s_blkcnt;
        Arena s_ranges, s_shard;
        Arena tables;
        void* host_tables = nullptr;
        size_t host_cap = 0;
        hipEvent_t tables_done = nullptr;
        bool tables_recorded = false;
        std::vector<unsigned char> tab_key;
        int tab_src = 0;
        hipStream_t tab_upload_stream = nullptr;
        hipEvent_t bin_done = nullptr, fuse_done = nullptr;
        bool fuse_recorded = false;
        uint32_t epoch = 0;
    } pb[4];
    unsigned pass = 0, sort_pass = 0;
    uint32_t sort_epoch = 0;
    int sort_streams = 2;
    bool trace = false;
    int sort_ring = 3;
    struct Deferred { bool valid = false; FuseArgs fa{}; int ts = 0, attr = 0; bool lean_binned = false; } deferred;
    uint32_t* form_seen = nullptr;
    int  frame_lean = 2;
    long long frame_lean_launches = 0, frame_generic_launches = 0;
    struct DeferredWalk { bool valid = false; WalkArgs wa{}; bool block_form = false; int attr = 0; unsigned slot = 0; } dwalk;
    bool defer_walk = true;
    long long xbytes_out = 0, xbytes_in = 0, gbytes_out = 0, gbytes_in = 0;
    bool roctx = false;
    bool walk_always_wait = false;
    long long walks_unwaited = 0, walks_left = 0;
    bool defer = true;
    hipStream_t bin_stream = nullptr;
    hipStream_t bin_stream2 = nullptr;
    hipStream_t tab_stream = nullptr;
    hipEvent_t switch_done = nullptr;
    bool main_reads_pb = false;
    bool overlap = true;
    long long overlap_min_points = 1000000;
    long long sort_overlap_min_points = 100000;
    bool sort_path = true;
    long long sort_min_points = 200000, sort_min_points_batch = 390000;
    bool walk_permute = true;
    int  sort_passes = 0;
    int few_bins = 0;
    int blk_batch = 0;
    int ray_depth = 4, ray_lanes = 16;
    bool fast_laser = true;
    bool rank_by_ballot = false;
    bool lane_sort = true;
    bool ride_events = true;
    int  walk_lds_pad = 0;
    int  walk_prio = 4096;
    int  fuse_count = 1;
    int  sort_chunk = 0;
    bool light_fast = true;
    bool cache_tables = true;
    std::vector<unsigned char> key_scratch;
    bool plain_loop = true;
    int  sort_form = 0;
    int dbg_sweep = 0;
    bool track_lowest = false;
    unsigned dense_min = 2048;
    Arena scratch;
    unsigned long long* d_counters = nullptr;

    float pending[kMaxPending] = {0, 0, 0, 0};
    int   n_pending = 0;
    bool  floor_dirty = true;

    bool  timing = false, counting = false;
    std::vector<EventPair> events;
    std::vector<EventPair> pool;
    gem_stats stats{};
    hipEvent_t copy_done = nullptr;

    static constexpr int kStageEvents = 24;
    void*  hstage = nullptr;
    size_t hstage_cap = 0;
    bool   hstage_failed = false;
    size_t hstage_max = 256u << 20;
    int    copy_threads = 4;
    int    download_groups = 8;
    hipEvent_t ev_stage[kStageEvents] = {};
    hipEvent_t stage_read = nullptr;
    bool   stage_read_pending = false;
    hipEvent_t ev_half[2] = {nullptr, nullptr};
    bool   half_pending[2] = {false, false};
    unsigned stage_par = 0;
    long long hstage_allocations = 0;
    long long xfer_ns[5] = {0, 0, 0, 0, 0};

    std::unique_ptr<Transport> tp_x, tp_g;
    int nranks = 1, rank = 0;
    int strip_row[kMaxRanks + 1] = {0};
    bool tile_strips = false;
    struct Shard {
        bool valid = false;
        const uint2* hv = nullptr; const uint32_t* key = nullptr;
        const uint2* ranges = nullptr;
        uint32_t bounds[kMaxRanks + 1] = {0};
        const uint32_t* d_bounds = nullptr;
        int nstrips = 0, n_global_sweeps = 0;
        long long points = 0;
        int slot = -1;
        hipStream_t stream = nullptr;
    } shard;
    struct Step {
        bool valid = false;
        int parity = 0;
        int n_global_sweeps = 0;
        bool has_vu = false; float vu[512];
        Shard sd;
        bool gather = false; int gather_attrs = 0;
    } step;
    unsigned step_seq = 0;
    Arena sh_dev, sh_ranges;
    Arena sh_recv_hv[2], sh_recv_key[2], sh_recv_rng[2];
    hipStream_t comm_stream = nullptr, gather_stream = nullptr;
    hipEvent_t ev_sorted = nullptr, ev_exchanged = nullptr;
    hipEvent_t ev_bounds[2] = {nullptr, nullptr};
    hipEvent_t ev_walked[2] = {nullptr, nullptr};
    bool walk_recorded[2] = {false, false};
    hipEvent_t ev_vu[2] = {nullptr, nullptr};
    bool vu_recorded[2] = {false, false};
    unsigned vu_seq = 0;
    Arena published[2];
    hipEvent_t ev_published[2] = {nullptr, nullptr}, ev_gathered[2] = {nullptr, nullptr};
    bool gather_outstanding[2] = {false, false};
    bool gathered_recorded[2] = {false, false};
    unsigned gather_seq = 0;
    long long recv_bound = 0;
    void* sh_host = nullptr;
    hipEvent_t ev_t[10] = {};
    bool step_timed = false;

    Arena dbg;
    Arena ray;
    unsigned ray_calls = 0;
    Arena color;
    Arena clean_cnt;
    Arena vox_state, vox_hist;
    Arena vox_rec, vox_tmp;
    Arena vox_out[2];
    unsigned vox_flip = 0;
    struct Local {
        bool enabled = false;
        struct Capture { Arena rec, lin; double off = 0, res = 0, px = 0, py = 0; int sx = 0, sy = 0; } slot[2];
        int cur = -1, prev = -1;
        Arena log[2];
        int act = 0;
        Arena keys, vals;
        Arena spill_cnt, exp_cnt;
        Arena small;
        long long log_cap = 0, log_len = 0, table_cap = 0, live = 0;
    } local;
    struct Compose {
        Arena grid, dist, far;
        Arena road, obstacle;
        Arena cnt;
        Arena small;
        std::vector<float> host_dist;
        long long far_points = 0;
        long long sum_ns = 0;
    } compose;
    struct Global {
        bool enabled = false;
        Arena stack[2];
        int act = 0;
        long long cap = 0, used = 0;
        std::vector<long long> off, room, cnt;
        Arena cnts;
        Arena out[2], keys[2], tkeys[2], tvals[2], blk[2];
        Arena small;
    } global;
    struct Costmaps {
        static constexpr int kMax = 8;
        struct Map {
            bool used = false;
            gem_costmap_config cfg{};
            Arena grid[2];
            int act = 0;
            Arena stamps;
            Arena infl_table;
            gem_inflation_params infl_key{};
            bool infl_valid = false;
            Arena mg_dist[3];
            Arena mg_status;
            unsigned long long gen = 0;
            unsigned long long mg_gen[3] = {0, 0, 0};
            Arena nav_pot, nav_act, nav_path, nav_status;
            unsigned long long nav_gen = 0;
            int nav_n_path = 0;
            gem_navplan_status nav_last{};
            Arena fr_label, fr_index, fr_act, fr_rec, fr_out, fr_words;
            unsigned long long fr_gen = 0;
            int fr_n_kept = 0;
        } map[kMax];
        unsigned long long generation = 0;
        Arena small;
        Arena in, win;
        std::vector<unsigned char> host_rows;
        Arena infl_bits, infl_flags;
        void* mg_pin[2] = {nullptr, nullptr};
        size_t mg_pin_cap[2] = {0, 0};
        hipEvent_t mg_ev[2] = {nullptr, nullptr};
        bool mg_ev_pending[2] = {false, false};
        unsigned mg_turn = 0;
        Arena mg_pose, mg_traj;
        std::vector<double> mg_plan;
        Arena nav_w;
        void* nav_pin = nullptr;
        std::vector<int> nav_cells;
        Arena fr_blocks;
        void* fr_pin = nullptr;
        Arena cr_cand, cr_pose, cr_len, cr_ext, cr_total, cr_best;
        Arena tg_pose, tg_len, tg_ext;
        Arena ob_bits, ob_rays, ob_cnt;
        Arena fp_pose, fp_cost, fp_traj;
    } costmap;
    struct History {
        bool enabled = false;
        Arena log[2];
        int act = 0;
        long long len = 0, cap = 0;
        Arena box;
        long long box_cap = 0;
        Arena small;
    } history;
    int  nav_chunk = 0;
    int  front_chunk = 0;
    bool obstacle_direct = true;
    bool history_cull = true;
    struct Octree {
        static constexpr int kSlots = 4;
        Arena state, hist;
        bool dirty = false;
        Arena tab;
        double tab_key[3] = {-1, -1, -1};
        Arena in, work;
        struct Slot {
            Arena out;
            long long bytes = 0;
            gem_octree_stats stats{};
        } slot[kSlots];
    } octree;
    bool  dbg_on = false;
    bool  dbg_frame = false;
    long long sort_fallbacks = 0;
    long long arena_allocations = 0;
    int   dbg_rows = 0;
    int fuse_variant = 12;
};

namespace gemi {

int fail(gem_handle* h, int code, const char* what, hipError_t e = hipSuccess);

bool roctx_load();
void roctx_push(const char* name);
void roctx_pop();
struct ApiRange {
    bool on;
    ApiRange(const gem_handle* h, const char* name);
    ~ApiRange() { if (on) roctx_pop(); }
};

#define GEM_HIP(h, call)                                                        \
    do { hipError_t _e = (call); if (_e != hipSuccess) return fail(h, GEM_ERR_HIP, #call, _e); } while (0)

#define GEM_ENTRY(name)                                                         \
    ApiRange api_range(h, name);                                                \
    if (!h) return GEM_ERR_INVALID;                                             \
    std::lock_guard<std::mutex> lk(h->mu);                                      \
    hipSetDevice(h->device)

int step_abort(gem_handle* h, int rc);
#define GEM_HIP_STEP(h, call)                                                   \
    do { hipError_t _e = (call); if (_e != hipSuccess) return step_abort(h, fail(h, GEM_ERR_HIP, #call, _e)); } while (0)

int ensure(gem_handle* h, Arena& a, size_t bytes);
int ensure_zeroed(gem_handle* h, Arena& a, size_t bytes);
int ensure_ray(gem_handle* h);

struct HostXfer { void* host; void* dev; size_t bytes; };

inline long long host_ns()
{
    return std::chrono::duration_cast<std::chrono::nanoseconds>(std::chrono::steady_clock::now().time_since_epoch()).count();
}

unsigned char* host_stage(gem_handle* h, size_t bytes);
int drain_staging(gem_handle* h);
int upload_arrays(gem_handle* h, const HostXfer* x, int n, bool defer_ok = false, unsigned char** zero_copy_region = nullptr, int* zero_copy_half = nullptr);
int download_arrays(gem_handle* h, const HostXfer* x, int n, size_t stage_off);

struct CloudLayout { size_t rgb, orig, bytes; };
CloudLayout cloud_layout(long long n, bool rgb, bool orig);
struct StagedCloud {
    const float4* xyzi = nullptr; const uint32_t* rgb = nullptr; const int* orig = nullptr;
    float4* arena_xyzi = nullptr;
    int half = -1;
};
int stage_cloud(gem_handle* h, long long n, const float* xyzi, const uint32_t* rgb, const int* orig, StagedCloud& out);
int release_half(gem_handle* h, int half, int rc);
float to_float_rn(double v);

void fill_frame(const gem_handle* h, const gem_frame_params* p, FrameConst& f);
hipEvent_t get_event(gem_handle* h);

struct Timed {
    gem_handle* h; EventPair ep{};
    bool on;
    Timed(gem_handle* hh, int kind) : h(hh), on(hh->timing && kind >= 0)
    {
        if (!on) return;
        if (!h->pool.empty()) { ep = h->pool.back(); h->pool.pop_back(); }
        else { ep.a = get_event(h); ep.b = get_event(h); }
        ep.kind = kind;
    }
    LaunchEvents events() const { LaunchEvents e; if (on) { e.start = ep.a; e.stop = ep.b; } return e; }
    ~Timed() { if (on) h->events.push_back(ep); }
};

void fold_events(gem_handle* h);
int flush_deferred(gem_handle* h);
bool frame_launch_lean(gem_handle* h, bool fused_lean, bool bin_fast);
int flush_walk(gem_handle* h);
int flush_local(gem_handle* h);
int wait_gather(gem_handle* h);
void local_free(gem_handle* h);
int local_grid_count(gem_handle* h, uint32_t* n);
int local_export_to(gem_handle* h, void* dst, uint32_t n_grid, bool clear);
void compose_free(gem_handle* h);
int compose_check(gem_handle* h, const gem_compose_params* p, const char* what);
int compose_split(gem_handle* h, const gem_compose_params* p, bool want_road, bool want_obstacle, uint32_t tot[3], double* out_threshold);
void octree_free(gem_handle* h);
void global_free(gem_handle* h);
void history_free(gem_handle* h);
int history_check_room(gem_handle* h, long long n, const char* what);
int history_reserve(gem_handle* h, long long extra);
int history_append_device(gem_handle* h, const void* d_src, long long n);
int history_blocks_culled(gem_handle* h, long long* out);
struct CriticsCall {
    const char* what;
    const gem_critic* critics;
    int n_critics;
    const gem_footprint_pose* poses;
    const int* traj_len;
    long long n_traj;
    int T;
    const double* spec_xy;
    int n_vertices;
    const double* ext;
    int n_ext;
    double* out_total;
    gem_best_trajectory* out_best;
    bool on_device;
    bool own_arrays = false;
};
int critics_prepare(gem_handle* h, int id, const CriticsCall& c, gem::CriticsArgs& a, gem::FootSpec& spec, gem::CostGeom& geom);
void costmap_free(gem_handle* h);
int voxel_reserve(gem_handle* h, long long max_points);
int settle(gem_handle* h);
int flush_pending(gem_handle* h, bool with_floor);
int index_to_range(int index, int L);

struct PassInput {
    int src = 0;
    bool device_input = false;
    bool caller_device = false;
    int n_sweeps = 1;
    long long n = 0;
    const gem_frame_params* params = nullptr;
    const long long* offsets = nullptr;
    const float* var_updates = nullptr;
    const int* sweep_orig0 = nullptr;
    const float4* xyzi = nullptr; const uint32_t* rgb = nullptr; const int* orig = nullptr;
    const int* f_index = nullptr; const float* f_height = nullptr; const float* f_var = nullptr;
    const int* f_R = nullptr; const int* f_G = nullptr; const int* f_B = nullptr; const float* f_I = nullptr;
};

constexpr unsigned  kDeviceEventFlags = hipEventDisableTiming | hipEventDisableSystemFence;

hipError_t acquire_streams(int device, StreamSet& out);
void release_streams(int device, const StreamSet& set);
hipError_t acquire_comm_stream(int device, hipStream_t* out);
void release_comm_stream(int device, hipStream_t st);

PlanEnv plan_env(const gem_handle* h);
SortGeometry sort_geometry(const gem_handle* h, int n_sweeps, bool block_form);
struct SortBuffers { void *hv1, *hv2, *key1, *key2, *src1, *src2, *cnt1, *cnt2, *misc; };
void bind_sort_buffers(const SortPlan& p, int n_passes, const SortBuffers& b, SortArgs& sa);

constexpr size_t kShardHostBytes = 8192 + 2 * 2048, kShardDevBytes = 8192 + 2 * 2048;
struct ShardOpts { int sweep_id0; int nstrips; const int* strip_rows; bool bounds_stay_on_device; };

int run_sort_pipeline(gem_handle* h, const PassInput& in, int attr, const SortGeometry& geo, const ShardOpts* shard = nullptr);
int run_pipeline(gem_handle* h, const PassInput& in0);

enum class AddSource { host, device, aos, depth };
enum class FrontEnd { none, clean, voxel };
struct DepthSource {
    gem_depth_image img;
    float k[4], unit;
    bool on_device;
};
struct AddCloud {
    AddSource source;
    int n;
    const void* xyzi; const void* rgb = nullptr; const void* orig = nullptr;
    int point_step = 0, off_x = 0, off_y = 0, off_z = 0, off_intensity = -1, off_rgb = -1;
    const DepthSource* image = nullptr;
};
struct AddFront {
    FrontEnd kind = FrontEnd::none;
    const gem_clean_params* clean = nullptr;
    const gem_voxel_params* stages = nullptr; int n_stages = 0;
};
int add_cloud(gem_handle* h, const gem_frame_params* p, const AddCloud& c, const AddFront& fe);
bool aos_fields_ok(int point_step, int off_x, int off_y, int off_z, int off_intensity, int off_rgb);
int voxel_front(gem_handle* h, const gem_voxel_params* stages, int ns, int n, const float4* xyzi, const uint32_t* rgb,
                const float4** out, const uint32_t** rgb_out);
bool voxel_stages_ok(const gem_voxel_params* stages, int ns);
int depth_unproject(gem_handle* h, const DepthSource& s, const void* depth, const void* color, const gem_clean_params* clean,
                    float4* xyzi, uint32_t* rgb);

int shard_finish_locked(gem_handle* h);
int ensure_recv(gem_handle* h, int parity, size_t records);
int ensure_shard_tables(gem_handle* h, size_t blocks = 0);
size_t strip_blocks_of(const gem_handle* h, int p);
bool shard_sort_rotates(const gem_handle* h, long long n);
int shard_checks(gem_handle* h, int n_global_sweeps, SortGeometry* geo);

}
```

gem_amd/csrc/gem_capi_pipeline.cpp:

```cpp
#include "gem_capi_internal.hpp"
#include "gem_clean.hpp"

namespace gemi {

static bool sort_bins_fit(int bins) { return sort_shape(bins, true, kSortChunkRecords).lds <= 160 * 1024; }
PlanEnv plan_env(const gem_handle* h)
{
    PlanEnv e{};
    e.L = h->L; e.ts = h->ts; e.sort_form = h->sort_form; e.sort_passes = h->sort_passes; e.sort_chunk = h->sort_chunk; e.sort_ring = h->sort_ring;
    e.sort_path = h->sort_path; e.track_lowest = h->track_lowest; e.sort_min_points = h->sort_min_points; e.sort_min_points_batch = h->sort_min_points_batch;
    return e;
}
SortGeometry sort_geometry(const gem_handle* h, int n_sweeps, bool block_form) { return sort_digits(h->L, h->sort_passes, n_sweeps, block_form, sort_bins_fit); }

static int stage_batch_tables(gem_handle* h, gem_handle::PassBuffers& pb, const TablesPlan& t, unsigned char** host = nullptr)
{
    if (t.total > pb.tables.cap) pb.tab_key.clear();
    const int rc = ensure(h, pb.tables, t.total);
    if (rc) return rc;
    if (t.total > pb.host_cap) {
        if (pb.tables_recorded) GEM_HIP(h, hipEventSynchronize(pb.tables_done));
        if (pb.host_tables) GEM_HIP(h, hipHostFree(pb.host_tables));
        pb.host_tables = nullptr; pb.host_cap = 0;
        GEM_HIP(h, hipHostMalloc(&pb.host_tables, t.total * 2, hipHostMallocDefault));
        pb.host_cap = t.total * 2;
    }
    if (!host || !t.total) return GEM_OK;
    if (!pb.tables_done) GEM_HIP(h, hipEventCreateWithFlags(&pb.tables_done, hipEventDisableTiming));
    if (pb.tables_recorded) GEM_HIP(h, hipEventSynchronize(pb.tables_done));
    pb.tab_key.clear();
    *host = static_cast<unsigned char*>(pb.host_tables);
    memset(*host, 0, t.total);
    return GEM_OK;
}
static int fill_batch_tables(const gem_handle* h, unsigned char* host, const TablesPlan& t, const PassInput& in, const int* first0)
{
    bool laser = in.src == 0, fast = true;
    for (int s = 0; s < in.n_sweeps; ++s) {
        FrameConst& fc = reinterpret_cast<FrameConst*>(host + t.o_frames)[s];
        fill_frame(h, in.src == 0 ? &in.params[s] : nullptr, fc);
        laser = laser && in.params[s].sensor_model == GEM_MODEL_LASER;
        fast = fast && fc.fast_laser != 0;
    }
    memcpy(host + t.o_first0, first0, sizeof(int) * (in.n_sweeps + 1));
    memcpy(host + t.o_first, in.offsets, sizeof(long long) * (in.n_sweeps + 1));
    if (in.sweep_orig0) memcpy(host + t.o_orig, in.sweep_orig0, sizeof(int) * in.n_sweeps);
    if (in.var_updates) memcpy(host + t.o_var, in.var_updates, sizeof(float) * in.n_sweeps);
    return laser ? (fast ? 4 : 2) : 0;
}
static int ensure_sort_buffers(gem_handle* h, gem_handle::PassBuffers& pb, const SortPlan& p)
{
    int rc;
    if ((rc = ensure(h, pb.s_hv1, p.hv)) || (rc = ensure(h, pb.s_hv2, p.hv)) || (rc = ensure(h, pb.s_key1, p.key)) || (rc = ensure(h, pb.s_key2, p.key)) ||
        (rc = ensure(h, pb.s_src1, p.src)) || (rc = ensure(h, pb.s_src2, p.src)) ||
        (rc = ensure(h, pb.s_cnt1, p.cnt1)) || (rc = ensure(h, pb.s_cnt2, p.cnt2)) || (rc = ensure(h, pb.s_misc, p.misc)) ||
        (rc = ensure_zeroed(h, pb.s_blkcnt, p.blkcnt)) || (rc = ensure(h, pb.s_ranges, p.ranges)) || (rc = ensure(h, pb.s_shard, p.shard))) return rc;
    return stage_batch_tables(h, pb, p.tables);
}
void bind_sort_buffers(const SortPlan& p, int n_passes, const SortBuffers& b, SortArgs& sa)
{
    unsigned char* misc = static_cast<unsigned char*>(b.misc);
    for (int i = 0; i < n_passes; ++i) {
        sa.cnt[i] = static_cast<uint32_t*>(i == 0 ? b.cnt1 : b.cnt2);
        sa.segtot[i] = reinterpret_cast<uint32_t*>(misc + p.o_seg[i]);
    }
    sa.total = reinterpret_cast<uint32_t*>(misc + p.o_total); sa.bin_base = reinterpret_cast<uint32_t*>(misc + p.o_base);
    sa.odd_flag = sa.total + 1;
    sa.seg_cnt = reinterpret_cast<uint32_t*>(misc + p.o_segcnt);
    sa.hv_a = static_cast<uint2*>(b.hv2); sa.hv_b = static_cast<uint2*>(b.hv1);
    sa.key_a = static_cast<uint32_t*>(b.key2); sa.key_b = static_cast<uint32_t*>(b.key1);
    sa.src_a = p.src ? static_cast<uint32_t*>(b.src2) : nullptr; sa.src_b = p.src ? static_cast<uint32_t*>(b.src1) : nullptr;
}
static int ensure_tile_buffers(gem_handle* h, gem_handle::PassBuffers& pb, const TilePlan& p, hipStream_t st, bool frame, unsigned char** host = nullptr)
{
    int rc;
    if ((rc = ensure(h, pb.rec, p.rec)) || (rc = ensure(h, pb.srt, p.srt))) return rc;
    if (p.seg > pb.seg.cap) {
        if ((rc = ensure(h, pb.seg, p.seg))) return rc;
        GEM_HIP(h, hipMemsetAsync(pb.seg.p, 0, pb.seg.cap, st));
    }
    if (p.flag > pb.flag.cap || p.gflag > pb.gflag.cap) {
        if ((rc = ensure(h, pb.flag, p.flag)) || (rc = ensure(h, pb.gflag, p.gflag))) return rc;
        GEM_HIP(h, hipMemsetAsync(pb.flag.p, 0, pb.flag.cap, st));
        GEM_HIP(h, hipMemsetAsync(pb.gflag.p, 0, pb.gflag.cap, st));
        pb.epoch = 0;
    }
    if (!frame) return stage_batch_tables(h, pb, p.tables, host);
    if ((rc = ensure(h, pb.bkt, p.bkt)) || (rc = ensure_zeroed(h, pb.bcnt, p.bcnt)) || (rc = ensure_zeroed(h, pb.fctl, p.fctl))) return rc;
    if (!h->form_seen) {
        GEM_HIP(h, hipHostMalloc(reinterpret_cast<void**>(&h->form_seen), 64, hipHostMallocDefault));
        *h->form_seen = 0u;
    }
    if (p.spill > pb.spill.cap) {
        if ((rc = ensure(h, pb.spill, p.spill))) return rc;
        GEM_HIP(h, hipMemsetAsync(pb.spill.p, 0xff, pb.spill.cap, h->stream));
    }
    return stage_batch_tables(h, pb, p.tables, host);
}
static int pass_done(gem_handle* h, long long n)
{
    h->n_pending = 0;
    h->floor_dirty = false;
    h->stats.points_in = n;
    return GEM_OK;
}
static int switch_to_bin_streams(gem_handle* h, bool overlap)
{
    if (!overlap) h->main_reads_pb = true;
    if (!overlap || !h->main_reads_pb) return GEM_OK;
    GEM_HIP(h, hipEventRecord(h->switch_done, h->stream));
    GEM_HIP(h, hipStreamWaitEvent(h->bin_stream, h->switch_done, 0));
    if (h->bin_stream2) GEM_HIP(h, hipStreamWaitEvent(h->bin_stream2, h->switch_done, 0));
    if (h->tab_stream) GEM_HIP(h, hipStreamWaitEvent(h->tab_stream, h->switch_done, 0));
    h->main_reads_pb = false;
    for (auto& b : h->pb) b.fuse_recorded = false;
    return GEM_OK;
}

void batch_tables_key(const gem_handle* h, const PassInput& in, int kind, const void* device_tables, const std::vector<int>& first_of_sweep, std::vector<unsigned char>& key)
{
    key.clear();
    auto put = [&](const void* p, size_t n) { const unsigned char* b = static_cast<const unsigned char*>(p); key.insert(key.end(), b, b + n); };
    const int head[8] = {kind, in.n_sweeps, in.var_updates ? 1 : 0, in.sweep_orig0 ? 1 : 0, h->L, h->row0, h->row1, h->fast_laser ? 1 : 0};
    put(head, sizeof(head));
    put(&device_tables, sizeof(device_tables));
    put(h->center, sizeof(h->center)); put(h->start, sizeof(h->start)); put(&h->res, sizeof(h->res));
    put(in.params, sizeof(gem_frame_params) * in.n_sweeps);
    put(in.offsets, sizeof(long long) * (in.n_sweeps + 1));
    if (in.var_updates) put(in.var_updates, sizeof(float) * in.n_sweeps);
    if (in.sweep_orig0) put(in.sweep_orig0, sizeof(int) * in.n_sweeps);
    put(first_of_sweep.data(), sizeof(int) * first_of_sweep.size());
}


int run_sort_pipeline(gem_handle* h, const PassInput& in, int attr, const SortGeometry& geo, const ShardOpts* shard)
{
    const bool batched = in.n_sweeps > 1;
    const bool with_src = (attr & 3) != 0;
    const int chunk = sort_chunk_for(in.n, h->sort_chunk);
    const long long nc2max = (in.n + chunk - 1) / chunk;
    std::vector<int> chunk0(batched ? in.n_sweeps + 1 : 0, 0);
    for (int s = 0; batched && s < in.n_sweeps; ++s) chunk0[s + 1] = chunk0[s] + (int)((in.offsets[s + 1] - in.offsets[s] + chunk - 1) / chunk);
    const int NC1 = batched ? chunk0[in.n_sweeps] : (int)nc2max;
    const SortPlan plan = sort_plan(geo.n_passes, geo.dbins, in.n, (size_t)NC1, (size_t)nc2max, in.n_sweeps, with_src, walk_blocks(geo, shard != nullptr), shard != nullptr);
    const bool dense = h->n_pending > 0 || h->floor_dirty || (batched && in.var_updates != nullptr);
    const int T = geo.T;
    h->T = T;

    bool overlap = h->overlap && in.n >= std::min(h->overlap_min_points, h->sort_overlap_min_points) && h->stream == h->own_stream && !h->counting &&
                   (!shard || shard->bounds_stay_on_device);
    { const int rcd = flush_deferred(h); if (rcd) return rcd; }
    const bool leave_walk = overlap && !shard && h->defer_walk && in.caller_device && attr == 0 && !h->timing && !h->dbg_on;
    if (!leave_walk) { const int rcd = flush_walk(h); if (rcd) return rcd; }
    const int keep_row0 = h->row0, keep_row1 = h->row1;
    struct RestoreRows { gem_handle* h; int r0, r1; ~RestoreRows() { h->row0 = r0; h->row1 = r1; } } restore{h, keep_row0, keep_row1};
    if (shard) { h->row0 = 0; h->row1 = h->L; }
    const unsigned seq = overlap ? h->sort_pass++ : 0u;
    const unsigned slot = overlap ? seq % (unsigned)h->sort_ring : 0u;
    gem_handle::PassBuffers& pb = h->pb[slot];
    hipStream_t sbin = overlap ? (((seq & 1u) && h->sort_streams > 1 && h->bin_stream2) ? h->bin_stream2 : h->bin_stream) : h->stream;
    int rc;
    if ((rc = switch_to_bin_streams(h, overlap))) return rc;
    if (h->trace)
        fprintf(stderr, "[gem] sorted pass: n=%lld sweeps=%d overlap=%d (knob %d, min %lld, own stream %d, counting %d, shard %d) slot=%u stream=%s\n",
                (long long)in.n, in.n_sweeps, (int)overlap, (int)h->overlap, (long long)std::min(h->overlap_min_points, h->sort_overlap_min_points), (int)(h->stream == h->own_stream),
                (int)h->counting, (int)(shard != nullptr), slot, sbin == h->stream ? "main" : (sbin == h->bin_stream ? "bin" : "bin2"));

    if ((rc = ensure_sort_buffers(h, pb, plan))) return rc;
    if (overlap && pb.fuse_recorded) GEM_HIP(h, hipEventSynchronize(pb.fuse_done));

    SortArgs sa{};
    WalkArgs wa{};
    int batch_src = -1;
    if (batched) {
        const TablesPlan& t = plan.tables;
        batch_tables_key(h, in, 0, pb.tables.p, chunk0, h->key_scratch);
        const bool tables_cached = h->cache_tables && h->key_scratch == pb.tab_key;
        if (!tables_cached) {
            unsigned char* host;
            if ((rc = stage_batch_tables(h, pb, t, &host))) return rc;
            pb.tab_src = fill_batch_tables(h, host, t, in, chunk0.data());
            hipStream_t stab = sbin;
            if (overlap && h->tab_stream) stab = h->tab_stream;
            GEM_HIP(h, hipMemcpyAsync(pb.tables.p, host, t.total, hipMemcpyHostToDevice, stab));
            GEM_HIP(h, hipEventRecord(pb.tables_done, stab)); pb.tables_recorded = true;
            if (stab != sbin) GEM_HIP(h, hipStreamWaitEvent(sbin, pb.tables_done, 0));
            pb.tab_key = h->key_scratch;
            pb.tab_upload_stream = stab;
        } else if (pb.tab_upload_stream != sbin && pb.tables_recorded) {
            GEM_HIP(h, hipStreamWaitEvent(sbin, pb.tables_done, 0));
        }
        batch_src = pb.tab_src;
        unsigned char* d = static_cast<unsigned char*>(pb.tables.p);
        sa.frames = reinterpret_cast<const FrameConst*>(d + t.o_frames);
        sa.sweep_chunk0 = reinterpret_cast<const int*>(d + t.o_first0);
        sa.sweep_first = reinterpret_cast<const long long*>(d + t.o_first);
        sa.sweep_orig0 = in.sweep_orig0 ? reinterpret_cast<const int*>(d + t.o_orig) : nullptr;
        wa.var_updates = in.var_updates ? reinterpret_cast<const float*>(d + t.o_var) : nullptr;
    } else {
        fill_frame(h, in.src == 0 ? in.params : nullptr, sa.frame0);
        sa.orig0_single = in.sweep_orig0 ? in.sweep_orig0[0] : 0;
    }
    sa.n_sweeps = in.n_sweeps; sa.n = in.n; sa.sweep_id0 = shard ? shard->sweep_id0 : 0;
    sa.xyzi = in.xyzi; sa.rgb = in.rgb; sa.orig = in.orig;
    sa.f_index = in.f_index; sa.f_height = in.f_height; sa.f_var = in.f_var;
    sa.f_R = in.f_R; sa.f_G = in.f_G; sa.f_B = in.f_B; sa.f_I = in.f_I;
    sa.keep_sentinel = h->track_lowest ? 1 : 0;
    sa.rank_by_ballot = h->rank_by_ballot ? 1 : 0; sa.few_bins = h->few_bins;
    sa.tiles_per_row = geo.tiles_per_row; sa.T = T;
    sa.id_bits = geo.id_bits; sa.n_passes = geo.n_passes;
    for (int i = 0; i < 3; ++i) { sa.dshift[i] = geo.dshift[i]; sa.dbits[i] = geo.dbits[i]; sa.dbins[i] = geo.dbins[i]; }
    sa.n_chunks1 = NC1; sa.chunk = chunk;
    constexpr long long kFuseCountMaxPoints = 600000;
    sa.fuse_count = (geo.n_passes >= 2 && (h->fuse_count == 2 || (h->fuse_count == 1 && in.n <= kFuseCountMaxPoints))) ? 1 : 0;
    bind_sort_buffers(plan, geo.n_passes, {pb.s_hv1.p, pb.s_hv2.p, pb.s_key1.p, pb.s_key2.p, pb.s_src1.p, pb.s_src2.p, pb.s_cnt1.p, pb.s_cnt2.p, pb.s_misc.p}, sa);
    sa.epoch = ++h->sort_epoch; if (sa.epoch == 0u) sa.epoch = ++h->sort_epoch;
    wa.odd_flag = sa.odd_flag; wa.epoch = sa.epoch;
    sa.blk_cnt = nullptr;
    if (plan.blkcnt) {
        sa.blk_cnt = static_cast<uint32_t*>(pb.s_blkcnt.p);
        if (pb.blkcnt_dirty) GEM_HIP(h, hipMemsetAsync(pb.s_blkcnt.p, 0, pb.s_blkcnt.cap, sbin));
        pb.blkcnt_dirty = true;
    }
    sa.counters = h->counting ? h->d_counters : nullptr;

    const bool final_b = (geo.n_passes & 1) != 0;
    wa.hv = final_b ? sa.hv_b : sa.hv_a; wa.key = final_b ? sa.key_b : sa.key_a; wa.src = final_b ? sa.src_b : sa.src_a; wa.bin_base = sa.bin_base;
    wa.walk_order = (h->walk_permute && 4ll * T <= 4096) ? 1 : 0;
    wa.center_tr = ((h->L / 2 + h->start[0]) % h->L) >> 5;
    wa.T = T; wa.tiles_per_row = geo.tiles_per_row; wa.L = h->L; wa.row0 = h->row0; wa.row1 = h->row1;
    wa.id_bits = geo.id_bits; wa.bin_shift = geo.dshift[geo.n_passes - 1]; wa.n_sweeps = in.n_sweeps;
    wa.exact_bins = (geo.block_form && geo.n_passes == 1) ? 1 : 0;
    wa.lane_sort = h->lane_sort ? 1 : 0;
    wa.light_blocks = h->blk_batch ? (h->blk_batch <= 512 ? 1 : 0) : ((long long)in.n <= 768ll * 4 * T ? 1 : 0);
    if (wa.light_blocks) wa.lane_sort = 0;
    wa.mahal = h->cfg.mahalanobis_threshold; wa.var_floor = h->cfg.variance_floor;
    wa.dense = dense ? 1 : 0;
    wa.n_pending = h->n_pending;
    for (int i = 0; i < kMaxPending; ++i) wa.pending[i] = h->pending[i];
    wa.plain_env = h->plain_loop ? walk_plain_env(wa.var_floor, wa.mahal, h->pending, h->n_pending, batched ? in.var_updates : nullptr, in.n_sweeps) : 0;
    wa.prio_records = h->walk_prio; wa.lds_pad = h->walk_lds_pad; wa.light_fast = h->light_fast ? 1 : 0;
    wa.elevation = h->layers.elevation; wa.variance = h->layers.variance; wa.lowest = h->layers.lowest;
    wa.start0 = h->start[0]; wa.start1 = h->start[1];
    wa.intensity = h->layers.intensity; wa.colorR = h->layers.colorR; wa.colorG = h->layers.colorG; wa.colorB = h->layers.colorB;
    wa.xyzi = in.xyzi; wa.rgb = in.rgb; wa.f_R = in.f_R; wa.f_G = in.f_G; wa.f_B = in.f_B; wa.f_I = in.f_I;
    wa.counters = sa.counters;
    wa.count_per_pass = batched ? 0 : 1;

    if (h->counting) GEM_HIP(h, hipMemsetAsync(h->d_counters, 0, 2 * sizeof(unsigned long long), h->stream));
    bool ride_bin = false;
    {
        const bool two = geo.n_passes >= 2, three = geo.n_passes == 3;
        Timed t0(h, 3), t1(h, 4), t2(h, 5), t3(h, two && !sa.fuse_count ? 6 : -1), t4(h, two ? 7 : -1), t5(h, two ? 8 : -1), t6(h, three ? 6 : -1), t7(h, three ? 7 : -1), t8(h, three ? 8 : -1);
        LaunchEvents ev[9] = {t0.events(), t1.events(), t2.events(), t3.events(), t4.events(), t5.events(), t6.events(), t7.events(), t8.events()};
        ride_bin = overlap && h->ride_events && !h->timing && !shard && !(geo.block_form && geo.n_passes > 1);
        if (ride_bin) ev[3 * geo.n_passes - 1].stop = pb.bin_done;
        int src = in.src;
        if (src == 0 && batched) { if (batch_src > 0) src = batch_src; }
        else if (src == 0) {
            if (in.params[0].sensor_model == GEM_MODEL_LASER) src = sa.frame0.fast_laser ? 4 : 2;
        }
        GEM_HIP(h, launch_sort(sbin, sa, src, with_src, ev));
    }
    if (shard) {
        gem_handle::Shard& sd = h->shard;
        sd.valid = false;
        if ((rc = ensure_shard_tables(h))) return rc;
        uint32_t* host = static_cast<uint32_t*>(h->sh_host);
        for (int k = 0; k <= shard->nstrips; ++k) {
            const int tile_row = shard->strip_rows[k] >= h->L ? geo.tiles_per_row : shard->strip_rows[k] / 32;
            host[k] = (uint32_t)(tile_row * geo.tiles_per_row) << 10;
        }
        uint32_t* d_ids = static_cast<uint32_t*>(pb.s_shard.p), *d_bounds = d_ids + 16;
        const uint32_t* keys = final_b ? sa.key_b : sa.key_a;
        GEM_HIP(h, hipMemcpyAsync(d_ids, host, sizeof(uint32_t) * (shard->nstrips + 1), hipMemcpyHostToDevice, sbin));
        GEM_HIP(h, launch_strip_bounds(sbin, keys, sa.total, geo.id_bits, d_ids, d_bounds, shard->nstrips + 1));
        GEM_HIP(h, launch_block_prefix(sbin, sa.blk_cnt, 4 * T, static_cast<uint2*>(pb.s_ranges.p)));
        pb.blkcnt_dirty = false;
        sd.hv = final_b ? sa.hv_b : sa.hv_a; sd.key = keys; sd.ranges = static_cast<const uint2*>(pb.s_ranges.p);
        sd.d_bounds = d_bounds; sd.nstrips = shard->nstrips; sd.slot = overlap ? (int)slot : -1; sd.stream = sbin;
        h->stats.points_in = in.n;
        if (shard->bounds_stay_on_device) {
            for (int k = 0; k <= shard->nstrips; ++k) sd.bounds[k] = 0;
            if (overlap) GEM_HIP(h, hipEventRecord(pb.bin_done, sbin));
            sd.valid = true;
            return GEM_OK;
        }
        GEM_HIP(h, hipMemcpyAsync(host + 32, d_bounds, sizeof(uint32_t) * (shard->nstrips + 1), hipMemcpyDeviceToHost, sbin));
        GEM_HIP(h, hipStreamSynchronize(sbin));
        for (int k = 0; k <= shard->nstrips; ++k) sd.bounds[k] = host[32 + k];
        sd.valid = true;
        return GEM_OK;
    }
    if (geo.block_form && geo.n_passes > 1) {
        GEM_HIP(h, launch_block_prefix(sbin, sa.blk_cnt, 4 * T, static_cast<uint2*>(pb.s_ranges.p)));
        pb.blkcnt_dirty = false;
        wa.ranges = static_cast<const uint2*>(pb.s_ranges.p);
    }
    { const int rcd = flush_walk(h); if (rcd) return rcd; }
    if (leave_walk) {
        if (!ride_bin) GEM_HIP(h, hipEventRecord(pb.bin_done, sbin));
        h->dwalk.wa = wa; h->dwalk.block_form = geo.block_form; h->dwalk.attr = attr; h->dwalk.slot = slot; h->dwalk.valid = true;
        ++h->walks_left;
        h->dbg_rows = 0;
        return pass_done(h, in.n);
    }
    if (overlap) {
        if (!ride_bin) GEM_HIP(h, hipEventRecord(pb.bin_done, sbin));
        GEM_HIP(h, hipStreamWaitEvent(h->stream, pb.bin_done, 0));
    }
    h->dbg_rows = 0;
    if (h->dbg_on && geo.block_form) {
        if ((rc = ensure(h, h->dbg, (size_t)T * 4 * 16 * 8))) return rc;
        GEM_HIP(h, hipMemsetAsync(h->dbg.p, 0, (size_t)T * 4 * 16 * 8, h->stream));
        wa.dbg = static_cast<unsigned long long*>(h->dbg.p);
        h->dbg_rows = T * 4;
    }
    { Timed t(h, 9); GEM_HIP(h, geo.block_form ? launch_block_walk(h->stream, wa, attr, t.events()) : launch_walk(h->stream, wa, attr, t.events())); }
    if (overlap) { GEM_HIP(h, hipEventRecord(pb.fuse_done, h->stream)); pb.fuse_recorded = true; }
    return pass_done(h, in.n);
}

int run_pipeline(gem_handle* h, const PassInput& in0)
{
    const PlanEnv env = plan_env(h);
    const PassChoice choice = choose_pass(env, in0.n, in0.n_sweeps, sort_bins_fit);
    if (choice.fell_back) ++h->sort_fallbacks;
    int attr = 0;
    if (in0.src == 0 && in0.rgb) attr = 1;
    if (in0.src == 1 && in0.f_R && in0.f_G && in0.f_B && in0.f_I) attr = 2;
    if (h->track_lowest) attr |= 4;
    if (choice.geo.ok) return run_sort_pipeline(h, in0, attr, choice.geo);
    { const int rcw = flush_walk(h); if (rcw) return rcw; }
    TilePlan plan = tile_plan(env, in0.n, in0.n_sweeps, in0.offsets);
    if (plan.err) return fail(h, GEM_ERR_INVALID, plan.err == 1 ? "cloud too large" : "lowest tracking: the pass is too large for 16x16 tiles (cut it into smaller calls)");
    PassInput in = in0;
    std::vector<gem_frame_params> cut_params;
    std::vector<long long> cut_offsets;
    std::vector<int> orig0;
    if (plan.n_sweeps != in.n_sweeps) {
        const int ns = plan.n_sweeps;
        if (in.src == 0) cut_params.assign(ns, *in.params);
        cut_offsets.resize(ns + 1); orig0.resize(ns);
        for (int s = 0; s <= ns; ++s) cut_offsets[s] = std::min<long long>(in.n, (long long)s * kSweepPoints);
        for (int s = 0; s < ns; ++s) orig0[s] = (int)cut_offsets[s];
        in.n_sweeps = ns; in.params = in.src == 0 ? cut_params.data() : nullptr; in.offsets = cut_offsets.data(); in.var_updates = nullptr; in.sweep_orig0 = orig0.data();
    }
    const bool batched = in.n_sweeps > 1;
    const int U = kUnit, B = plan.B, bpad = plan.bpad;
    const bool dense = h->n_pending > 0 || h->floor_dirty || (batched && in.var_updates != nullptr);

    if (B == 0) {
        if (batched && in.var_updates)
            for (int s = 0; s < in.n_sweeps; ++s) {
                if (h->n_pending == kMaxPending) { int rc = flush_pending(h, true); if (rc) return rc; }
                h->pending[h->n_pending++] = in.var_updates[s];
            }
        return (h->n_pending || h->floor_dirty) ? flush_pending(h, true) : GEM_OK;
    }
    const int ts = plan.ts, tiles_per_row = plan.tiles_per_row, T = plan.T;
    h->T = T;
    if (fuse_lds_bytes(ts, h->fuse_variant, attr & 3) > 160 * 1024) return fail(h, GEM_ERR_INVALID, "fuse kernel geometry exceeds the LDS");

    bool overlap = h->overlap && in.n >= h->overlap_min_points && h->stream == h->own_stream && !h->counting && !h->dbg_on;
    const bool defer = h->defer && in.device_input && in.src == 0 && !batched && (attr & 3) == 0 && ts == 4 && !overlap &&
                       !h->counting && (!h->dbg_on || h->dbg_frame);
    if (!defer) { const int rcd = flush_deferred(h); if (rcd) return rcd; }
    gem_handle::PassBuffers& pb = h->pb[(overlap || defer) ? (h->pass++ & 1u) : 0u];
    hipStream_t sbin = overlap ? h->bin_stream : h->stream;
    int rc;
    if ((rc = switch_to_bin_streams(h, overlap))) return rc;
    if (overlap && pb.fuse_recorded) GEM_HIP(h, hipEventSynchronize(pb.fuse_done));
    static_assert(kSweepPoints <= (1ll << 22), "k_frame's record format");
    unsigned char* host = nullptr;
    if ((rc = ensure_tile_buffers(h, pb, plan, sbin, defer, &host))) return rc;
    if (pb.epoch >= kFlagEpochMax) {
        GEM_HIP(h, hipMemsetAsync(pb.flag.p, 0, pb.flag.cap, sbin));
        GEM_HIP(h, hipMemsetAsync(pb.gflag.p, 0, pb.gflag.cap, sbin));
        pb.epoch = 0;
    }
    ++pb.epoch;

    BinArgs ba{};
    FuseArgs fa{};
    const TablesPlan& tab = plan.tables;
    if (batched) {
        std::vector<int> unit0(in.n_sweeps + 1, 0);
        for (int s = 0; s < in.n_sweeps; ++s) unit0[s + 1] = unit0[s] + (int)sweep_units(in.offsets[s + 1] - in.offsets[s]);
        (void)fill_batch_tables(h, host, tab, in, unit0.data());
        GEM_HIP(h, hipMemcpyAsync(pb.tables.p, host, tab.total, hipMemcpyHostToDevice, sbin));
        GEM_HIP(h, hipEventRecord(pb.tables_done, sbin)); pb.tables_recorded = true;
        unsigned char* d = static_cast<unsigned char*>(pb.tables.p);
        ba.frames = reinterpret_cast<const FrameConst*>(d + tab.o_frames);
        ba.sweep_unit0 = reinterpret_cast<const int*>(d + tab.o_first0);
        ba.sweep_first = reinterpret_cast<const long long*>(d + tab.o_first);
        ba.sweep_orig0 = in.sweep_orig0 ? reinterpret_cast<const int*>(d + tab.o_orig) : nullptr;
        fa.sweep_unit0 = ba.sweep_unit0;
        fa.var_updates = in.var_updates ? reinterpret_cast<const float*>(d + tab.o_var) : nullptr;
    } else {
        fill_frame(h, in.src == 0 ? in.params : nullptr, ba.frame0);
    }
    ba.n_sweeps = in.n_sweeps; ba.n = in.n;
    ba.xyzi = in.xyzi; ba.rgb = in.rgb; ba.orig = in.orig;
    ba.f_index = in.f_index; ba.f_height = in.f_height; ba.f_var = in.f_var;
    ba.f_R = in.f_R; ba.f_G = in.f_G; ba.f_B = in.f_B; ba.f_I = in.f_I;
    ba.T = T; ba.tiles_per_row = tiles_per_row; ba.B = B; ba.Bpad = bpad;
    ba.tile_bits = 0; while ((1 << ba.tile_bits) < T) ++ba.tile_bits;
    ba.epoch = pb.epoch;
    ba.rec_words = (attr & 3) != 0 ? 4 : 3;
    ba.rec = static_cast<uint4*>(pb.rec.p); ba.seg = static_cast<uint16_t*>(pb.seg.p); ba.flag = static_cast<uint32_t*>(pb.flag.p); ba.gflag = static_cast<uint32_t*>(pb.gflag.p);
    ba.counters = h->counting ? h->d_counters : nullptr;
    ba.keep_sentinel = h->track_lowest ? 1 : 0;
    ba.srt_top = reinterpret_cast<uint32_t*>(static_cast<unsigned char*>(pb.srt.p) + pb.srt.cap - 16);

    fa.epoch = pb.epoch;
    fa.rec = ba.rec; fa.seg = ba.seg; fa.flag = ba.flag; fa.gflag = ba.gflag; fa.B_total = B; fa.U = U; fa.n_sweeps = in.n_sweeps; fa.Bpad = bpad;
    fa.T = T; fa.tiles_per_row = tiles_per_row; fa.L = h->L; fa.row0 = h->row0; fa.row1 = h->row1;
    fa.center_tr = ((h->L / 2 + h->start[0]) % h->L) >> ts; fa.center_tc = ((h->L / 2 + h->start[1]) % h->L) >> ts;
    fa.mahal = h->cfg.mahalanobis_threshold; fa.var_floor = h->cfg.variance_floor;
    fa.dense = dense ? 1 : 0;
    fa.n_pending = h->n_pending;
    for (int i = 0; i < kMaxPending; ++i) fa.pending[i] = h->pending[i];
    fa.elevation = h->layers.elevation; fa.variance = h->layers.variance;
    fa.intensity = h->layers.intensity; fa.colorR = h->layers.colorR; fa.colorG = h->layers.colorG; fa.colorB = h->layers.colorB;
    fa.xyzi = in.xyzi; fa.rgb = in.rgb; fa.f_R = in.f_R; fa.f_G = in.f_G; fa.f_B = in.f_B; fa.f_I = in.f_I;
    fa.counters = ba.counters;
    fa.srt = static_cast<uint4*>(pb.srt.p); fa.srt_top = ba.srt_top; fa.dense_min = h->dense_min;
    fa.lowest = h->layers.lowest; fa.start0 = h->start[0]; fa.start1 = h->start[1];
    fa.count_per_pass = orig0.empty() ? 0 : 1;
    fa.dbg = nullptr;
    fa.dbg_sweep = h->dbg_sweep;
    if (h->dbg_on) {
        const int nbin = (B + 3) / 4;
        if ((rc = ensure(h, h->dbg, (size_t)(T + nbin) * 16 * 8))) return rc;
        GEM_HIP(h, hipMemsetAsync(h->dbg.p, 0, (size_t)(T + nbin) * 16 * 8, h->stream));
        fa.dbg = static_cast<unsigned long long*>(h->dbg.p);
        if (h->dbg_frame) { ba.dbg = fa.dbg + (size_t)T * 16; h->dbg_rows = T + nbin; }
    }

    if (defer) {
        ba.bkt = static_cast<uint32_t*>(pb.bkt.p); ba.bcount = static_cast<uint32_t*>(pb.bcnt.p); ba.spill = static_cast<uint4*>(pb.spill.p);
        ba.ctl = static_cast<uint32_t*>(pb.fctl.p);
        fa.bkt = ba.bkt; fa.bcount = ba.bcount; fa.spill = ba.spill; fa.ctl = ba.ctl; fa.form_seen = h->form_seen;
        if (h->deferred.valid && h->deferred.attr != attr) { const int rcd = flush_deferred(h); if (rcd) return rcd; }
        const bool lean = frame_launch_lean(h, !h->deferred.valid || h->deferred.lean_binned, ba.frame0.fast_laser != 0 && !ba.rgb);
        ba.lean = lean ? 1 : 0;
        if (h->deferred.valid) { Timed t(h, 2); GEM_HIP(h, launch_frame(h->stream, h->deferred.fa, ba, attr, lean, t.events())); }
        else                   { Timed t(h, 0); GEM_HIP(h, launch_frame(h->stream, FuseArgs{}, ba, attr, lean, t.events())); }
        h->deferred.fa = fa; h->deferred.ts = ts; h->deferred.attr = attr; h->deferred.valid = true; h->deferred.lean_binned = lean;
        return pass_done(h, in.n);
    }
    if (h->counting) GEM_HIP(h, hipMemsetAsync(h->d_counters, 0, 2 * sizeof(unsigned long long), h->stream));
    { Timed t(h, 0); GEM_HIP(h, launch_bin(sbin, ba, in.src, ts, t.events())); }
    if (overlap) {
        GEM_HIP(h, hipEventRecord(pb.bin_done, sbin));
        GEM_HIP(h, hipStreamWaitEvent(h->stream, pb.bin_done, 0));
    }
    { Timed t(h, 1); GEM_HIP(h, launch_fuse(h->stream, fa, ts, attr, h->fuse_variant, t.events())); }
    if (overlap) { GEM_HIP(h, hipEventRecord(pb.fuse_done, h->stream)); pb.fuse_recorded = true; }
    return pass_done(h, in.n);
}

}

int gem_reserve(gem_handle* h, long long max_points, int max_sweeps, int with_colours)
{
    if (!h || max_points < 0 || max_sweeps < 1 || max_points >= (1ll << 31)) return h ? fail(h, GEM_ERR_INVALID, "gem_reserve: bad argument") : GEM_ERR_INVALID;
    std::lock_guard<std::mutex> lk(h->mu);
    hipSetDevice(h->device);
    { const int rcd = settle(h); if (rcd) return rcd; }
    if (max_points == 0) return GEM_OK;
    int rc;
    if ((rc = ensure(h, h->stage, std::max({cloud_layout(max_points, true, true).bytes, stage_words_bytes(max_points, 9), depth_stage_bytes(max_points)})))) return rc;
    if ((rc = ensure(h, h->clean_cnt, clean_scratch_bytes(max_points)))) return rc;
    if ((rc = voxel_reserve(h, max_points))) return rc;
    const size_t one = stage_words_bytes(max_points, 7);
    size_t want = one < (16u << 20) ? 2 * one + 512 : 0;
    for (const size_t nine : {stage_words_bytes(max_points, 9), stage_words_bytes(h->cells, 9)}) if (nine <= (64u << 20)) want = std::max(want, nine);
    if (want) (void)host_stage(h, want);
    const bool sharded = h->tp_x && h->tile_strips;
    const PlanEnv env = plan_env(h);
    BoundPlan plan[kMaxBoundPlans];
    const int n_plans = bound_plans(env, max_points, max_sweeps, sharded ? h->nranks : 0, with_colours != 0, sort_bins_fit, plan);
    for (int i = 0; i < n_plans; ++i) {
        const BoundPlan& p = plan[i];
        for (int k = 0; p.kind == 1 && k < env.sort_ring; ++k) if ((rc = ensure_sort_buffers(h, h->pb[k], p.sort))) return rc;
        for (int k = 0; p.kind == 2 && k < 2; ++k) if ((rc = ensure_tile_buffers(h, h->pb[k], p.tile, h->stream, true))) return rc;
        if (sharded && p.kind == 1 && (rc = ensure_shard_tables(h, p.sort.blocks))) return rc;
    }
    if (sharded) {
        h->recv_bound = max_points;
        for (int q = 0; h->nranks > 1 && q < 2; ++q) if ((rc = ensure_recv(h, q, (size_t)max_points + 4 * h->nranks))) return rc;
    } else if (h->track_lowest && (rc = ensure_ray(h))) return rc;
    GEM_HIP(h, hipStreamSynchronize(h->stream));
    return GEM_OK;
}
```

gem_amd/csrc/gem_frame_lean.hip:

```cpp
#include "gem_frame_tile.hpp"

#include <hip/hip_ext.h>

namespace gem {

#define GEM_FRAME_HEAD_PARAMS int nf, int T, int tiles_per_row, uint32_t tile_div, int center_tr, int center_tc, \
                              const uint32_t* bkt, uint32_t* bcount, const float4* xyzi, int B, uint32_t n
#define GEM_FRAME_HEAD_PASS   nf, T, tiles_per_row, tile_div, center_tr, center_tc, bkt, bcount, xyzi, B, n

template <int FLAGS, bool STAMPS>
__device__ __forceinline__ void frame_lean_body(GEM_FRAME_HEAD_PARAMS, const FrameLeanArgs& la)
{
    extern __shared__ __attribute__((aligned(16))) unsigned char lds_dyn[];
    if ((int)blockIdx.x < nf) {
        FrameLeanTile t = la.t;
        t.nf = nf; t.T = T; t.tiles_per_row = tiles_per_row; t.tile_div = tile_div; t.center_tr = center_tr; t.center_tc = center_tc;
        t.bkt = bkt; t.bcount = bcount;
        frame_tile<FLAGS, STAMPS>(t, (int)blockIdx.x, lds_dyn);
    } else {
        const int block = (int)blockIdx.x - nf;
        FrameLeanBin b = la.b;
        b.xyzi = xyzi; b.B = B; b.n = n;
        [[maybe_unused]] unsigned long long c_start = 0, r_start = 0;
        if constexpr (STAMPS) { c_start = (unsigned long long)__builtin_readcyclecounter(); r_start = (unsigned long long)__builtin_amdgcn_s_memrealtime(); }
        bin_unit_lean(b, (int)(block * 4 + (threadIdx.x >> 6)));
        if (block == 0 && threadIdx.x == 0) b.ctl[1] = 0u;
        if constexpr (STAMPS) {
            if (b.dbg && threadIdx.x == 0) {
                b.dbg[(size_t)block * 16] = c_start; b.dbg[(size_t)block * 16 + 15] = (unsigned long long)blockIdx.x + 1ull;
                b.dbg[(size_t)block * 16 + 12] = r_start;
                b.dbg[(size_t)block * 16 + 14] = (unsigned long long)__builtin_amdgcn_s_getreg((3 << 11) | 20) + 1ull;
            }
        }
        bin_stamp_end<STAMPS>(b, block);
        __builtin_amdgcn_s_waitcnt(0xc07f);
    }
}

#ifndef GEM_FRAME_LEAN_STAMPS
#define GEM_FRAME_LEAN_STAMPS 0
#endif
constexpr bool kFrameLeanStamps = GEM_FRAME_LEAN_STAMPS != 0;

template <int FLAGS, bool LEAN>
__global__ __launch_bounds__(256, kFrameLeanWG) void k_frame(GEM_FRAME_HEAD_PARAMS, FrameLeanArgs la)
{
    static_assert(LEAN, "the generic form takes FuseArgs and BinArgs (gem_kernels.hip)");
    frame_lean_body<FLAGS, kFrameLeanStamps>(GEM_FRAME_HEAD_PASS, la);
}

template <int FLAGS>
__global__ __launch_bounds__(256, kFrameLeanWG) void k_frame_stamped(GEM_FRAME_HEAD_PARAMS, FrameLeanArgs la) { frame_lean_body<FLAGS, true>(GEM_FRAME_HEAD_PASS, la); }

#define GEM_LAUNCH(k, grid, block, lds, st, ev, ...)                                              \
    do {                                                                                           \
        if ((ev).start || (ev).stop) hipExtLaunchKernelGGL(k, grid, block, (uint32_t)(lds), st, (ev).start, (ev).stop, 0, __VA_ARGS__); \
        else hipLaunchKernelGGL(k, grid, block, lds, st, __VA_ARGS__);                             \
    } while (0)

hipError_t launch_frame_lean(hipStream_t st, const FuseArgs& fa, const BinArgs& ba, int attr, unsigned blocks, LaunchEvents ev)
{
    const dim3 grid(blocks), block(256);
    const FrameLeanArgs la = frame_lean_args(fa, ba);
    const FrameLeanHead h = frame_lean_head(la);
#define GEM_FRAME_HEAD_ARGS h.nf, h.T, h.tiles_per_row, h.tile_div, h.center_tr, h.center_tc, h.bkt, h.bcount, h.xyzi, h.B, h.n
    if (la.t.dbg || la.b.dbg) {
        if (attr == 4) GEM_LAUNCH((k_frame_stamped<4>), grid, block, kFrameLds, st, ev, GEM_FRAME_HEAD_ARGS, la);
        else           GEM_LAUNCH((k_frame_stamped<0>), grid, block, kFrameLds, st, ev, GEM_FRAME_HEAD_ARGS, la);
        return hipGetLastError();
    }
    if (attr == 4) GEM_LAUNCH((k_frame<4, true>), grid, block, kFrameLds, st, ev, GEM_FRAME_HEAD_ARGS, la);
    else           GEM_LAUNCH((k_frame<0, true>), grid, block, kFrameLds, st, ev, GEM_FRAME_HEAD_ARGS, la);
#undef GEM_FRAME_HEAD_ARGS
    return hipGetLastError();
}

}
```

gem_amd/csrc/gem_frame_lean.hpp:

```cpp
#pragma once

#include "gem_kernels.hpp"

namespace gem {

constexpr int kFrameRunBits = 3;
constexpr int kFrameGridUnit = 8 << kFrameRunBits;

struct FrameLeanTile {
    int       nf;
    int       T, tiles_per_row;
    uint32_t  tile_div;
    unsigned long long* dbg;
    const uint32_t* bkt; uint32_t* bcount;
    float *elevation, *variance, *lowest;
    uint4*    spill; uint32_t* ctl; uint32_t* form_seen;
    int   L, center_tr, center_tc, row0, row1, start0, start1;
    int   n_pending; float pending[kMaxPending];
    int   dense; float mahal, var_floor;
    uint32_t nspill;
};

struct FrameLeanBin {
    const float4* xyzi;
    int       B; uint32_t n;
    int       keep_sentinel, tile_bits, tiles_per_row;
    int       filter_on;
    uint32_t* bkt; uint32_t* bcount; uint4* spill; uint32_t* ctl;
    unsigned long long* dbg;
    float  T[12];
    float  lower_f, upper_f;
    float  fbx, fby, fband, fplane;
    float  cx, cy; int sx, sy, L; float res;
    int    row0, row1;
    float  beam_a, beam_c, t2;
    float  Js[2];
};

struct FrameLeanArgs { FrameLeanTile t; FrameLeanBin b; };
static_assert(sizeof(FrameLeanArgs) <= 352, "the lean form's kernel arguments: six 64-byte lines at most");

__host__ __device__ inline uint32_t frame_div_mul(int d) { return (uint32_t)((1ull << 31) / (unsigned long long)d) + 1u; }
__host__ __device__ inline int frame_div_by(int n, uint32_t m) { return (int)(((unsigned long long)((uint32_t)n << 1) * m) >> 32); }

__host__ __device__ inline int frame_rank_div(const FuseArgs& a, int rnk) { return rnk / a.tiles_per_row; }
__host__ __device__ inline int frame_rank_div(const FrameLeanTile& a, int rnk) { return frame_div_by(rnk, a.tile_div); }
__host__ __device__ inline uint32_t frame_spill_slots(const FuseArgs& a) { return (uint32_t)a.B_total * (uint32_t)a.U; }
__host__ __device__ inline uint32_t frame_spill_slots(const FrameLeanTile& a) { return a.nspill; }

template <class A>
__host__ __device__ inline bool frame_tile_of(const A& a, int block, int& tr, int& tc)
{
    const int tpr = a.tiles_per_row;
    const int x = block & 7, i = block >> 3;
    const int rnk = ((((i >> kFrameRunBits) << 3) + x) << kFrameRunBits) + (i & ((1 << kFrameRunBits) - 1));
    if (rnk >= a.T) return false;
    const int bi = frame_rank_div(a, rnk), bj = rnk - bi * tpr;
    const int oi = (bi & 1) ? -((bi + 1) >> 1) : (bi >> 1);
    const int cj = bj >> kFrameRunBits, t = bj & ((1 << kFrameRunBits) - 1);
    const int oj = (cj & 1) ? -(((cj - 1) >> 1) << kFrameRunBits) - 1 - t : ((cj >> 1) << kFrameRunBits) + t;
    tr = a.center_tr + oi; tr = tr < 0 ? tr + tpr : (tr >= tpr ? tr - tpr : tr);
    tc = a.center_tc + oj; tc = tc < 0 ? tc + tpr : (tc >= tpr ? tc - tpr : tc);
    return true;
}

__host__ __device__ inline int frame_tile_blocks(int T) { return (T + kFrameGridUnit - 1) & ~(kFrameGridUnit - 1); }

inline FrameLeanArgs frame_lean_args(const FuseArgs& fa, const BinArgs& ba)
{
    FrameLeanArgs la{};
    FrameLeanTile& t = la.t;
    t.nf = frame_tile_blocks(fa.T); t.T = fa.T; t.tiles_per_row = fa.tiles_per_row;
    t.tile_div = frame_div_mul(fa.tiles_per_row > 0 ? fa.tiles_per_row : 1);
    t.dbg = fa.dbg; t.bkt = fa.bkt; t.bcount = fa.bcount;
    t.elevation = fa.elevation; t.variance = fa.variance; t.lowest = fa.lowest;
    t.spill = fa.spill; t.ctl = fa.ctl; t.form_seen = fa.form_seen;
    t.L = fa.L; t.center_tr = fa.center_tr; t.center_tc = fa.center_tc; t.row0 = fa.row0; t.row1 = fa.row1;
    t.start0 = fa.start0; t.start1 = fa.start1;
    t.n_pending = fa.n_pending;
    for (int i = 0; i < kMaxPending; ++i) t.pending[i] = fa.pending[i];
    t.dense = fa.dense; t.mahal = fa.mahal; t.var_floor = fa.var_floor;
    t.nspill = (uint32_t)fa.B_total * (uint32_t)fa.U;
    FrameLeanBin& b = la.b;
    const FrameConst& fc = ba.frame0;
    b.xyzi = ba.xyzi; b.B = ba.B; b.n = (uint32_t)ba.n;
    b.keep_sentinel = ba.keep_sentinel; b.tile_bits = ba.tile_bits; b.tiles_per_row = ba.tiles_per_row;
    b.filter_on = fc.filter_on;
    b.bkt = ba.bkt; b.bcount = ba.bcount; b.spill = ba.spill; b.ctl = ba.ctl; b.dbg = ba.dbg;
    for (int i = 0; i < 12; ++i) b.T[i] = fc.T[i];
    b.lower_f = fc.lower_f; b.upper_f = fc.upper_f;
    b.fbx = fc.fbx; b.fby = fc.fby; b.fband = fc.fband; b.fplane = fc.fplane;
    b.cx = fc.cx; b.cy = fc.cy; b.sx = fc.sx; b.sy = fc.sy; b.L = fc.L; b.res = fc.res;
    b.row0 = fc.row0; b.row1 = fc.row1;
    b.beam_a = fc.beam_a; b.beam_c = fc.beam_c; b.t2 = fc.t2;
    b.Js[0] = fc.Js[0]; b.Js[1] = fc.Js[1];
    return la;
}

struct FrameLeanHead {
    int       nf, T, tiles_per_row;
    uint32_t  tile_div;
    int       center_tr, center_tc;
    const uint32_t* bkt; uint32_t* bcount;
    const float4* xyzi; int B; uint32_t n;
};
constexpr int kFrameHeadDwords = (int)(sizeof(FrameLeanHead) / 4);
static_assert(sizeof(FrameLeanHead) == 56 && kFrameHeadDwords <= 14, "the head of a lean launch: no padding, at most the 14 dwords the hardware preloads");

inline FrameLeanHead frame_lean_head(const FrameLeanArgs& la)
{
    FrameLeanHead h{};
    h.nf = la.t.nf; h.T = la.t.T; h.tiles_per_row = la.t.tiles_per_row; h.tile_div = la.t.tile_div;
    h.center_tr = la.t.center_tr; h.center_tc = la.t.center_tc;
    h.bkt = la.t.bkt; h.bcount = la.t.bcount;
    h.xyzi = la.b.xyzi; h.B = la.b.B; h.n = la.b.n;
    return h;
}

}
```

gem_amd/csrc/gem_kernels.hpp:

```cpp
#pragma once

#include "gem_device.hpp"

namespace gem {

constexpr int kMaxPending = 4;
constexpr int kMaxRanks = 8;

constexpr int      kSegCountBits  = 7;
constexpr uint32_t kSegCountMask  = (1u << kSegCountBits) - 1u;
constexpr uint32_t kSegStartMask  = 63u;
constexpr uint32_t kFlagEpochMax  = 0xfffffff0u;

struct LayerPtrs {
    float *elevation, *variance, *intensity, *traver, *lowest;
    int   *colorR, *colorG, *colorB;
    float *rough, *slope;
};

constexpr int      kFrameBucket   = 768;
constexpr uint32_t kSpillFree     = 0xffffffffu;

struct BinArgs {
    FrameConst frame0;
// ... 35 lines not shown
    uint16_t* seg;
    const uint32_t* flag;
    const uint32_t* gflag;
    uint32_t epoch;
    int   B_total;
    int   U;
    int   n_sweeps;
    const int* sweep_unit0;
    int   Bpad;
    int   T, tiles_per_row, L;
    int   center_tr, center_tc;
    int   row0, row1;
    float mahal, var_floor;
    int   dense;
    int   n_pending; float pending[kMaxPending];
    const float* var_updates;
    float *elevation, *variance;
    float* intensity; int *colorR, *colorG, *colorB;
    const float4* xyzi; const uint32_t* rgb;
    const int* f_R; const int* f_G; const int* f_B; const float* f_I;
    unsigned long long* counters;
    uint4*            srt;
    uint32_t*         srt_top;
    float*            lowest;
    int               start0, start1;
    int               dbg_sweep;
    uint32_t          dense_min;
    int   count_per_pass;
    unsigned long long* dbg;
    const uint32_t* bkt;
    uint32_t* bcount;
    uint4*    spill;
    uint32_t* ctl;
    uint32_t* form_seen;
};

struct SortArgs {
    FrameConst frame0;
    const FrameConst* frames;
    const int*        sweep_chunk0;
    const long long*  sweep_first;
    const int*        sweep_orig0;
    int               orig0_single;
    int               n_sweeps;
    int               sweep_id0;
    long long         n;
    const float4*   xyzi; const uint32_t* rgb; const int* orig;
    const int* f_index; const float* f_height; const float* f_var;
    const int* f_R; const int* f_G; const int* f_B; const float* f_I;
    int keep_sentinel;
    int few_bins;
    int rank_by_ballot;
    CameraConst cam;
    int tiles_per_row, T;
    int id_bits;
    int n_passes;
    int dshift[3], dbits[3], dbins[3];
    int n_chunks1;
    uint32_t *cnt[3], *segtot[3];
    uint32_t *seg_cnt;
    uint32_t *total;
    uint32_t *blk_cnt;
    uint32_t *bin_base;
    uint2 *hv_a, *hv_b;
    uint32_t *key_a, *key_b, *src_a, *src_b;
    unsigned long long* counters;
    uint32_t* odd_flag; uint32_t epoch;
    int chunk;
    int fuse_count;
};

struct PassArgs {
    const uint2* hv_in; const uint32_t* key_in; const uint32_t* src_in;
    uint2* hv_out; uint32_t* key_out; uint32_t* src_out;
    uint32_t* cnt; const uint32_t* segtot;
    int n_chunks;
    int bins, shift, digit_bits; uint32_t mask;
    const uint32_t* n_dev; long long n_host;
    const uint32_t* seg_cnt;
    const int* sweep_chunk0; const long long* sweep_first; int n_sweeps;
    uint32_t* bin_base;
    unsigned long long* counters;
    int few_bins;
    int coherent;
    int chunk;
    uint32_t* next_cnt; int next_bins, next_shift; uint32_t next_mask;
};

struct WalkArgs {
    const uint2* hv; const uint32_t* key; const uint32_t* src; const uint32_t* bin_base;
    int   T, tiles_per_row, L, row0, row1, id_bits, bin_shift, n_sweeps;
    int   walk_order;
    int   center_tr;
    float mahal, var_floor;
    int   dense;
    int   n_pending; float pending[kMaxPending];
    const float* var_updates;
    float *elevation, *variance, *lowest;
    int   start0, start1;
    float* intensity; int *colorR, *colorG, *colorB;
    const float4* xyzi; const uint32_t* rgb;
    const int* f_R; const int* f_G; const int* f_B; const float* f_I;
    unsigned long long* counters;
    int   count_per_pass;
    unsigned long long* dbg;
    const uint2* ranges;
    int   lane_sort;
    int light_blocks;
    int   exact_bins;
    const uint32_t* odd_flag; uint32_t epoch;
    int   light_fast;
    int   lds_pad;
    int   prio_records;
    int   plain_env;
    int   n_src;
    const uint2* src_hv[kMaxRanks]; const uint32_t* src_key[kMaxRanks]; uint32_t src_n[kMaxRanks];
    const uint2* src_ranges[kMaxRanks]; uint32_t src_base[kMaxRanks]; uint32_t blk0;
};

inline int walk_plain_env(float var_floor, float mahal, const float* pending, int n_pending, const float* var_updates, int n_sweeps)
{
    auto inc_ok = [](float u) { return u >= 0.0f && u <= 262144.0f; };
    bool ok = var_floor >= 3.7252902984619140625e-9f && var_floor <= 268435456.0f && mahal > 0.0f && mahal <= 268435456.0f && n_sweeps <= 512;
    for (int i = 0; i < n_pending; ++i) ok = ok && inc_ok(pending[i]);
    if (var_updates) for (int i = 0; i < n_sweeps && ok; ++i) ok = ok && inc_ok(var_updates[i]);
    return ok ? 1 : 0;
}

struct LaunchEvents { hipEvent_t start = nullptr, stop = nullptr; };
struct SortShape { int nt, chunk; size_t lds; };
SortShape  sort_shape(int bins, bool attr, int chunk);
hipError_t launch_sort(hipStream_t st, const SortArgs& a, int src, bool attr, const LaunchEvents ev[9]);
hipError_t launch_walk(hipStream_t st, const WalkArgs& a, int flags, LaunchEvents ev);
hipError_t launch_block_prefix(hipStream_t st, uint32_t* blk_cnt, int n_blocks, uint2* ranges);
hipError_t launch_block_walk(hipStream_t st, const WalkArgs& a, int flags, LaunchEvents ev);
constexpr int kOnePassMaxBins = 2048;
hipError_t launch_strip_bounds(hipStream_t st, const uint32_t* keys, const uint32_t* n_records, int id_bits, const uint32_t* ids, uint32_t* out, int n);
constexpr int kSortChunkRecords = 4096, kSortSegsPerChunk = 4;
constexpr int kSortChunkSmall = 1024;
inline int sort_chunk_for(long long n, int forced = 0)
{
    if (forced == kSortChunkRecords || forced == kSortChunkSmall) return forced;
    return n / kSortChunkRecords < 2 * 256 ? kSortChunkSmall : kSortChunkRecords;
}
constexpr int kSortMaxBins = 8000;

hipError_t launch_project(hipStream_t st, const FrameConst& fc, int first, int n, float* x, float* y, float* z, const int* orig,
                          int write_back, int* map_idx, float* var, float* xt, float* yt, float* zt);

hipError_t launch_bin(hipStream_t st, const BinArgs& a, int src, int ts, LaunchEvents ev);
hipError_t launch_fuse(hipStream_t st, const FuseArgs& a, int ts, int attr, int variant, LaunchEvents ev);
hipError_t launch_frame(hipStream_t st, const FuseArgs& fuse_prev, const BinArgs& bin_this, int attr, bool lean, LaunchEvents ev);
hipError_t launch_frame_lean(hipStream_t st, const FuseArgs& fuse_prev, const BinArgs& bin_this, int attr, unsigned blocks, LaunchEvents ev);
size_t     fuse_lds_bytes(int ts, int variant, int attr);
hipError_t launch_init(hipStream_t st, const LayerPtrs& m, int cells, int clear_lowest);
hipError_t launch_unpack_aos(hipStream_t st, const void* src, int n, int step, int ox, int oy, int oz, int oi, int orgb, float4* xyzi, uint32_t* rgb);
hipError_t launch_raytracing(hipStream_t st, const LayerPtrs& m, int L, int start0, int start1, float sensor_z, float obstacle_threshold,
                             int row0, int row1, uint32_t* list, uint32_t* counts, int parity, float* lowest_snapshot, int depth = 4, int lanes = 16);
hipError_t launch_clear_strip(hipStream_t st, const LayerPtrs& m, int L, int start, int count, int is_row);
hipError_t launch_dense_variance(hipStream_t st, float* variance, int cells, int n_pending, const float* pending,
                                 int apply_floor, float var_floor);
hipError_t launch_update_height(hipStream_t st, float* elevation, int cells, float dz);
hipError_t launch_map_feature(hipStream_t st, const float* elevation, float* traver, float* rough, float* slope,
                              int L, float res, int sx, int sy, int row0, int row1);
hipError_t launch_show(hipStream_t st, const LayerPtrs& m, int L, int sx, int sy, double map_length, double resolution, double px, double py,
                       uint32_t* block_count, float* visual, float* xyz, unsigned char* rgb, unsigned char* image, uint32_t* total);

struct ColorArgs {
    const uint32_t* key; const uint2* hv; const uint32_t* total;
    uint32_t* first;
    uint32_t* pix;
    uint32_t* link;
    int n, width, height;
    const unsigned char* image; size_t stride;
    float4* xyzi; uint32_t* rgb;
};
hipError_t launch_colorize(hipStream_t st, const ColorArgs& a);
constexpr int kCopyListMax = 12;
struct CopyPiece { void* dst; const void* src; size_t bytes; };
struct CopyList { CopyPiece piece[kCopyListMax]; int n; };
hipError_t launch_copy_list(hipStream_t st, const CopyList& l);
hipError_t launch_export_gridmap(hipStream_t st, const void* src, const float* elevation, float* dst, int L, int is_int);

}
```

Before: 25.20 billion.

## Add steady-state frame fast path reusing cached lean launch arguments

Adds a steady-state path to run_pipeline. When consecutive frames keep the same point count, attributes, stream and handle generation, it skips planning and argument building and patches a cached lean launch buffer (pointers, pose, epoch, pending variance) before issuing the fused lean kernel directly. FrameConst construction is also cached, and only the pose part is recomputed when the map and sensor parameters are unchanged. A generation counter bumped by every state-changing API call invalidates the cache. The cost is the risk of stale arguments if some state change is missed, so a check mode (2) compares the fast path against the full path.

```diff
diff --git a/gem_amd/build.py b/gem_amd/build.py
--- a/gem_amd/build.py
+++ b/gem_amd/build.py
@@ -20,7 +20,7 @@
            CSRC / "gem_mapgrid.hip", CSRC / "gem_capi_mapgrid.cpp", CSRC / "gem_critics.hip", CSRC / "gem_capi_critics.cpp",
            CSRC / "gem_trajgen.hip", CSRC / "gem_capi_trajgen.cpp", CSRC / "gem_navplan.hip", CSRC / "gem_capi_navplan.cpp",
            CSRC / "gem_frontier.hip", CSRC / "gem_capi_frontier.cpp", CSRC / "gem_obstacle.hip", CSRC / "gem_capi_obstacle.cpp"]
-HEADERS = [CSRC / "gem_device.hpp", CSRC / "gem_kernels.hpp", CSRC / "gem_frame_lean.hpp", CSRC / "gem_frame_tile.hpp", CSRC / "gem_frame_sort.hpp", CSRC / "gem_wave.hpp", CSRC / "gem_compact.hpp", CSRC / "gem_transport.hpp", CSRC / "gem_hostcopy.hpp", CSRC / "gem_capi_internal.hpp", CSRC / "gem_plan.hpp", CSRC / "gem_clean.hpp", CSRC / "gem_local.hpp", CSRC / "gem_voxel.hpp", CSRC / "gem_global.hpp", CSRC / "gem_compose.hpp", CSRC / "gem_costmap.hpp", CSRC / "gem_lsd.hpp", CSRC / "gem_octree.hpp", CSRC / "gem_depth.hpp", CSRC / "gem_history.hpp", CSRC / "gem_footprint.hpp", CSRC / "gem_inflate.hpp", CSRC / "gem_mapgrid.hpp", CSRC / "gem_score_device.hpp", CSRC / "gem_critics.hpp", CSRC / "gem_trajgen.hpp", CSRC / "gem_sincos.hpp",
+HEADERS = [CSRC / "gem_device.hpp", CSRC / "gem_kernels.hpp", CSRC / "gem_frame_lean.hpp", CSRC / "gem_frame_steady.hpp", CSRC / "gem_frame_tile.hpp", CSRC / "gem_frame_sort.hpp", CSRC / "gem_wave.hpp", CSRC / "gem_compact.hpp", CSRC / "gem_transport.hpp", CSRC / "gem_hostcopy.hpp", CSRC / "gem_capi_internal.hpp", CSRC / "gem_plan.hpp", CSRC / "gem_clean.hpp", CSRC / "gem_local.hpp", CSRC / "gem_voxel.hpp", CSRC / "gem_global.hpp", CSRC / "gem_compose.hpp", CSRC / "gem_costmap.hpp", CSRC / "gem_lsd.hpp", CSRC / "gem_octree.hpp", CSRC / "gem_depth.hpp", CSRC / "gem_history.hpp", CSRC / "gem_footprint.hpp", CSRC / "gem_inflate.hpp", CSRC / "gem_mapgrid.hpp", CSRC / "gem_score_device.hpp", CSRC / "gem_critics.hpp", CSRC / "gem_trajgen.hpp", CSRC / "gem_sincos.hpp",
            CSRC / "gem_navplan.hpp", CSRC / "gem_navpath.hpp", CSRC / "gem_frontier.hpp", CSRC / "gem_costmap_host.hpp", CSRC / "gem_rounds.hpp", CSRC / "gem_tile_round.hpp", CSRC / "gem_obstacle.hpp", ROOT.parent / "include" / "gem_hip_frontier.h", ROOT.parent / "include" / "gem_hip_obstacle.h",
            ROOT.parent / "include" / "gem_hip_debug.h", ROOT.parent / "include" / "gem_hip.h", ROOT.parent / "include" / "gem_hip_history.h",
            ROOT.parent / "include" / "gem_hip_footprint.h", ROOT.parent / "include" / "gem_hip_inflate.h", ROOT.parent / "include" / "gem_hip_mapgrid.h",
diff --git a/gem_amd/csrc/gem_capi.cpp b/gem_amd/csrc/gem_capi.cpp
--- a/gem_amd/csrc/gem_capi.cpp
+++ b/gem_amd/csrc/gem_capi.cpp
@@ -250,6 +250,7 @@
     if (h->bin_stream) GEM_HIP(h, hipStreamSynchronize(h->bin_stream));
     if (h->bin_stream2) GEM_HIP(h, hipStreamSynchronize(h->bin_stream2));
     h->stream = hip_stream ? static_cast<hipStream_t>(hip_stream) : h->own_stream;
+    steady_touch(h);
     return GEM_OK;
 }
 
@@ -295,6 +296,7 @@
     { const int rcd = settle(h); if (rcd) return rcd; }
     const int L = h->L; const float res = h->res;
     h->sensor_z = position[2];
+    steady_touch(h);
     int shift[2]; float aligned[2];
     for (int i = 0; i < 2; ++i) {
         const float d = position[i] - h->center[i];
@@ -603,6 +605,7 @@
     std::lock_guard<std::mutex> lk(h->mu);
     hipSetDevice(h->device);
     { const int rcd = settle(h); if (rcd) return rcd; }
+    steady_touch(h);
     for (int i = 0; i < 2; ++i) {
         const float d = opt_position[i] - h->center[i];
         const int shift = static_cast<int>(static_cast<double>(d / h->res) + 0.5 * (d > 0 ? 1 : -1));
@@ -619,6 +622,7 @@
     std::lock_guard<std::mutex> lk(h->mu);
     hipSetDevice(h->device);
     { const int rcd = settle(h); if (rcd) return rcd; }
+    steady_touch(h);
     for (int i = 0; i < 2; ++i) {
         const float d = update_position[i] - h->center[i];
         const int shift = static_cast<int>(static_cast<double>(d / h->res) + 0.5 * (d > 0 ? 1 : -1));
@@ -780,6 +784,7 @@
     hipSetDevice(h->device);
     { const int rcd = settle(h); if (rcd) return rcd; }
     h->track_lowest = enabled != 0;
+    steady_touch(h);
     return GEM_OK;
 }
 
@@ -806,6 +811,7 @@
     hipSetDevice(h->device);
     { const int rcd = settle(h); if (rcd) return rcd; }
     h->timing = enabled != 0;
+    steady_touch(h);
     h->step_timed = h->timing && h->tp_x != nullptr && h->nranks > 1;
     return GEM_OK;
 }
@@ -817,6 +823,7 @@
     hipSetDevice(h->device);
     { const int rcd = settle(h); if (rcd) return rcd; }
     h->counting = enabled != 0;
+    steady_touch(h);
     return GEM_OK;
 }
 
@@ -845,6 +852,7 @@
     std::lock_guard<std::mutex> lk(h->mu);
     hipSetDevice(h->device);
     { const int rcd = settle(h); if (rcd) return rcd; }
+    steady_touch(h);
     const std::string k(key);
     if (k == "fuse_variant")            { if (value < 10 || value > 12) return fail(h, GEM_ERR_INVALID, "fuse_variant: 10..12"); h->fuse_variant = (int)value; }
     else if (k == "tile_shift")         { if (value != 0 && value != 4 && value != 5) return fail(h, GEM_ERR_INVALID, "tile_shift: 0, 4 or 5"); h->ts = (int)value; }
@@ -854,6 +862,7 @@
     else if (k == "dense_min")          { if (value < 0 || value > 0xffffffffll) return fail(h, GEM_ERR_INVALID, "dense_min: 0 .. 2^32 - 1"); h->dense_min = (unsigned)value; }
     else if (k == "dbg_sweep")          h->dbg_sweep = (int)value;
     else if (k == "dbg_frame")          h->dbg_frame = value != 0;
+    else if (k == "frame_steady")       { if (value < 0 || value > 2) return fail(h, GEM_ERR_INVALID, "frame_steady: 0 (off), 1 (on) or 2 (check against the long way)"); h->frame_steady = (int)value; }
     else if (k == "frame_lean")         { if (value < 0 || value > 2) return fail(h, GEM_ERR_INVALID, "frame_lean: 0 (generic), 1 (lean) or 2 (the host picks)"); h->frame_lean = (int)value; }
     else if (k == "overlap")            h->overlap = value != 0;
     else if (k == "overlap_min_points") { if (value < 0) return fail(h, GEM_ERR_INVALID, "overlap_min_points: >= 0"); h->overlap_min_points = value; h->sort_overlap_min_points = value; }
@@ -920,6 +929,10 @@
     else if (k == "walks_unwaited") *out = h->walks_unwaited;
     else if (k == "frame_lean_launches") *out = h->frame_lean_launches;
     else if (k == "frame_generic_launches") *out = h->frame_generic_launches;
+    else if (k == "frame_steady") *out = h->frame_steady;
+    else if (k == "frame_steady_hits") *out = h->frame_steady_hits;
+    else if (k == "frame_steady_misses") *out = h->frame_steady_misses;
+    else if (k == "frame_steady_mismatch") *out = h->frame_steady_mismatch;
     else if (k == "frame_form_seen") *out = h->form_seen ? (long long)*static_cast<volatile const uint32_t*>(h->form_seen) : 0;
     else if (k == "walks_left") *out = h->walks_left;
     else if (k == "history_cull") *out = h->history_cull ? 1 : 0;
@@ -957,6 +970,7 @@
     hipSetDevice(h->device);
     { const int rcd = settle(h); if (rcd) return rcd; }
     h->dbg_on = enable != 0;
+    steady_touch(h);
     if (out && h->dbg.p) {
         GEM_HIP(h, hipStreamSynchronize(h->stream));
         const int rows = h->dbg_rows ? h->dbg_rows : h->T;
diff --git a/gem_amd/csrc/gem_capi_comm.cpp b/gem_amd/csrc/gem_capi_comm.cpp
--- a/gem_amd/csrc/gem_capi_comm.cpp
+++ b/gem_amd/csrc/gem_capi_comm.cpp
@@ -18,6 +18,7 @@
     for (int k = 0; k <= nranks; ++k)
         h->strip_row[k] = tile_strips ? std::min(h->L, 32 * (int)((long long)tile_rows * k / nranks)) : (int)((long long)h->L * k / nranks);
     h->row0 = h->strip_row[rank]; h->row1 = h->strip_row[rank + 1];
+    steady_touch(h);
     if (nranks > 1)
         for (int g = 0; g < 2; ++g) { const int rc = ensure(h, h->published[g], (size_t)(h->row1 - h->row0) * h->L * 4 * 6 + 256); if (rc) return rc; }
     return GEM_OK;
diff --git a/gem_amd/csrc/gem_capi_core.cpp b/gem_amd/csrc/gem_capi_core.cpp
--- a/gem_amd/csrc/gem_capi_core.cpp
+++ b/gem_amd/csrc/gem_capi_core.cpp
@@ -58,6 +58,7 @@
     if (e != hipSuccess) return fail(h, GEM_ERR_NOMEM, "hipMalloc(arena)", e);
     a.cap = want;
     ++h->arena_allocations;
+    steady_touch(h);
     return GEM_OK;
 }
 
@@ -277,50 +278,11 @@
     return GEM_OK;
 }
 
-void fill_frame(const gem_handle* h, const gem_frame_params* p, FrameConst& f)
-{
-    memset(&f, 0, sizeof(f));
-    if (p) {
-        for (int i = 0; i < 12; ++i) f.T[i] = p->T[i];
-        f.lower = p->lower; f.upper = p->upper;
-        f.lower_f = (float)p->lower; if ((double)f.lower_f > p->lower) f.lower_f = nextafterf(f.lower_f, -INFINITY);
-        f.upper_f = (float)p->upper; if ((double)f.upper_f < p->upper) f.upper_f = nextafterf(f.upper_f, INFINITY);
-        for (int i = 0; i < 8; ++i) f.sp[i] = p->sensor_params[i];
-        for (int i = 0; i < 3; ++i) { f.Js[i] = p->sensor_jacobian[i]; f.P[i] = p->P_mul_C_BM_T[i]; }
-        for (int i = 0; i < 9; ++i) { f.Q[i] = p->rotation_variance[i]; f.C[i] = p->C_SB_T[i]; f.Bs[i] = p->B_r_BS_skew[i]; }
-        f.filter_on = p->filter.enabled;
-        f.fbx = p->filter.box_x; f.fby = p->filter.box_y; f.fband = p->filter.band_y; f.fplane = p->filter.plane_y;
-        f.model = p->sensor_model;
-        f.orig_width = p->original_width;
-    }
-    f.cx = h->center[0]; f.cy = h->center[1];
-    f.sx = h->start[0];  f.sy = h->start[1];
-    f.L = h->L; f.res = h->res;
-    f.row0 = h->row0; f.row1 = h->row1;
-    f.beam_a = (float)f.sp[1]; f.beam_c = (float)f.sp[2];
-    f.t2 = 0.f; f.fast_laser = 0;
-    if (p && f.model == GEM_MODEL_LASER && h->fast_laser) {
-        const float min_r = (float)f.sp[0], vn = min_r * min_r;
-        const float c0 = f.Js[0] * 0.0f, c1 = f.Js[1] * 0.0f, c2 = f.Js[2] * vn;
-        const float b2 = c0 + (c1 + c2);
-        const float t2 = b2 * f.Js[2];
-        auto small = [](float v, float bound) { return std::isfinite(v) && std::fabs(v) <= bound; };
-        bool ok = t2 > 0.f && std::isfinite(t2) && small(f.beam_a, 1e6f) && small(f.beam_c, 1e6f);
-        for (int i = 0; i < 9; ++i) ok = ok && f.Q[i] == 0.0f && small(f.C[i], 1e6f) && small(f.Bs[i], 1e6f);
-        for (int i = 0; i < 3; ++i) ok = ok && small(f.Js[i], 1e6f) && small(f.P[i], 1e6f);
-        for (int i = 0; i < 3 && ok; ++i)
-            for (int j = i; j < 3; ++j) {
-                double d = 0.0;
-                for (int k = 0; k < 3; ++k) d += (double)f.T[4 * i + k] * (double)f.T[4 * j + k];
-                ok = ok && std::fabs(d - (i == j ? 1.0 : 0.0)) <= 0.01;
-            }
-        for (int i = 0; i < 3; ++i) ok = ok && small(f.T[4 * i + 3], 1e9f);
-        ok = ok && std::isfinite(f.lower) && std::isfinite(f.upper) && std::fabs(f.lower) <= 1e9 && std::fabs(f.upper) <= 1e9;
-        ok = ok && small(f.cx, 1e9f) && small(f.cy, 1e9f) && (double)f.L * (double)f.res <= 1e9;
-        ok = ok && f.res >= 9.5367431640625e-7f && f.res <= 1048576.0f && f.L >= 2;
-        if (ok) { f.t2 = t2; f.fast_laser = 1; }
-    }
-}
+FrameMapIn frame_map_in(const gem_handle* h)
+{
+    return FrameMapIn{h->center[0], h->center[1], h->start[0], h->start[1], h->L, h->res, h->row0, h->row1, h->fast_laser};
+}
+void fill_frame(const gem_handle* h, const gem_frame_params* p, FrameConst& f) { (void)fill_frame_from(frame_map_in(h), p, f); }
 
 hipEvent_t get_event(gem_handle* h)
 {
@@ -347,10 +309,15 @@
     h->events.clear();
 }
 
+bool frame_form_lean(const gem_handle* h, bool fused_lean, bool bin_fast)
+{
+    const bool seen = h->form_seen && *static_cast<volatile const uint32_t*>(h->form_seen) != 0u;
+    return fused_lean && bin_fast && (h->frame_lean == 1 || (h->frame_lean == 2 && !seen));
+}
 bool frame_launch_lean(gem_handle* h, bool fused_lean, bool bin_fast)
 {
-    const bool seen = h->form_seen && *static_cast<volatile const uint32_t*>(h->form_seen) != 0u;
-    const bool lean = fused_lean && bin_fast && (h->frame_lean == 1 || (h->frame_lean == 2 && !seen));
+    const bool lean = frame_form_lean(h, fused_lean, bin_fast);
+    if (!lean) steady_touch(h);
     ++(lean ? h->frame_lean_launches : h->frame_generic_launches);
     return lean;
 }
diff --git a/gem_amd/csrc/gem_capi_internal.hpp b/gem_amd/csrc/gem_capi_internal.hpp
--- a/gem_amd/csrc/gem_capi_internal.hpp
+++ b/gem_amd/csrc/gem_capi_internal.hpp
@@ -3,6 +3,7 @@
 #include "../../include/gem_hip.h"
 #include "../../include/gem_hip_debug.h"
 #include "gem_kernels.hpp"
+#include "gem_frame_steady.hpp"
 #include "gem_plan.hpp"
 #include "gem_hostcopy.hpp"
 #include "gem_transport.hpp"
@@ -87,6 +88,11 @@
     uint32_t* form_seen = nullptr;
     int  frame_lean = 2;
     long long frame_lean_launches = 0, frame_generic_launches = 0;
+    unsigned long long steady_gen = 1;
+    FrameSteady steady[2];
+    FrameConstCache frame_cache;
+    int  frame_steady = 1;
+    long long frame_steady_hits = 0, frame_steady_misses = 0, frame_steady_mismatch = 0;
     struct DeferredWalk { bool valid = false; WalkArgs wa{}; bool block_form = false; int attr = 0; unsigned slot = 0; } dwalk;
     bool defer_walk = true;
     long long xbytes_out = 0, xbytes_in = 0, gbytes_out = 0, gbytes_in = 0;
@@ -319,6 +325,7 @@
 namespace gemi {
 
 int fail(gem_handle* h, int code, const char* what, hipError_t e = hipSuccess);
+inline void steady_touch(gem_handle* h) { ++h->steady_gen; }
 
 bool roctx_load();
 void roctx_push(const char* name);
@@ -389,6 +396,8 @@
 void fold_events(gem_handle* h);
 int flush_deferred(gem_handle* h);
 bool frame_launch_lean(gem_handle* h, bool fused_lean, bool bin_fast);
+bool frame_form_lean(const gem_handle* h, bool fused_lean, bool bin_fast);
+FrameMapIn frame_map_in(const gem_handle* h);
 int flush_walk(gem_handle* h);
 int flush_local(gem_handle* h);
 int wait_gather(gem_handle* h);
diff --git a/gem_amd/csrc/gem_capi_pipeline.cpp b/gem_amd/csrc/gem_capi_pipeline.cpp
--- a/gem_amd/csrc/gem_capi_pipeline.cpp
+++ b/gem_amd/csrc/gem_capi_pipeline.cpp
@@ -154,7 +154,7 @@
     if (!leave_walk) { const int rcd = flush_walk(h); if (rcd) return rcd; }
     const int keep_row0 = h->row0, keep_row1 = h->row1;
     struct RestoreRows { gem_handle* h; int r0, r1; ~RestoreRows() { h->row0 = r0; h->row1 = r1; } } restore{h, keep_row0, keep_row1};
-    if (shard) { h->row0 = 0; h->row1 = h->L; }
+    if (shard) { h->row0 = 0; h->row1 = h->L; steady_touch(h); }
     const unsigned seq = overlap ? h->sort_pass++ : 0u;
     const unsigned slot = overlap ? seq % (unsigned)h->sort_ring : 0u;
     gem_handle::PassBuffers& pb = h->pb[slot];
@@ -321,30 +321,67 @@
     return pass_done(h, in.n);
 }
 
+static bool frame_steady_ready(gem_handle* h, const PassInput& in, int attr, FrameSteady& cur, FrameLaunchBuf& buf)
+{
+    if (!h->deferred.valid || !h->deferred.lean_binned || h->deferred.attr != attr) return false;
+    if (in.src != 0 || in.n_sweeps != 1 || !in.device_input || in.rgb || !in.params || in.n <= 0) return false;
+    if (h->timing || h->counting || h->dbg_on || h->step.valid || h->dwalk.valid) return false;
+    const unsigned s = h->pass & 1u;
+    const FrameSteady& prev = h->steady[s ^ 1u];
+    auto holds = [&](const FrameSteady& f) { return f.valid && f.n == in.n && f.attr == attr && f.stream == h->stream && f.gen == h->steady_gen; };
+    if (!holds(cur) || !holds(prev) || h->pb[s].epoch >= kFlagEpochMax) return false;
+    const FrameConst& fc = frame_const_cached(h->frame_cache, frame_map_in(h), *in.params);
+    if (!frame_form_lean(h, true, fc.fast_laser != 0)) return false;
+    const FrameCallWords w{in.xyzi, &fc, h->pb[s].epoch + 1u, h->n_pending, h->pending, (h->n_pending > 0 || h->floor_dirty) ? 1 : 0};
+    frame_steady_patch(prev, cur, w, buf);
+    return true;
+}
+
 int run_pipeline(gem_handle* h, const PassInput& in0)
 {
-    const PlanEnv env = plan_env(h);
-    const PassChoice choice = choose_pass(env, in0.n, in0.n_sweeps, sort_bins_fit);
-    if (choice.fell_back) ++h->sort_fallbacks;
     int attr = 0;
     if (in0.src == 0 && in0.rgb) attr = 1;
     if (in0.src == 1 && in0.f_R && in0.f_G && in0.f_B && in0.f_I) attr = 2;
     if (h->track_lowest) attr |= 4;
+    if (h->frame_steady == 1) {
+        FrameSteady& cur = h->steady[h->pass & 1u];
+        FrameLaunchBuf buf;
+        if (frame_steady_ready(h, in0, attr, cur, buf)) {
+            if (cur.fell_back) ++h->sort_fallbacks;
+            ++h->pb[h->pass++ & 1u].epoch;
+            h->main_reads_pb = true;
+            ++h->frame_lean_launches; ++h->frame_steady_hits;
+            GEM_HIP(h, launch_frame_lean(h->stream, h->device, buf, attr, cur.grid));
+            h->deferred.fa = cur.fa;
+            return pass_done(h, in0.n);
+        }
+    }
+    struct SteadyCheck {
+        gem_handle* h; bool on = false, done = false; FrameSteady next; FrameLaunchBuf buf;
+        ~SteadyCheck() { if (on && !done) ++h->frame_steady_mismatch; }
+    } check{h};
+    if (h->frame_steady == 2) {
+        check.next = h->steady[h->pass & 1u];
+        check.on = frame_steady_ready(h, in0, attr, check.next, check.buf);
+    }
+    const PlanEnv env = plan_env(h);
+    const PassChoice choice = choose_pass(env, in0.n, in0.n_sweeps, sort_bins_fit);
+    if (choice.fell_back) ++h->sort_fallbacks;
     if (choice.geo.ok) return run_sort_pipeline(h, in0, attr, choice.geo);
     { const int rcw = flush_walk(h); if (rcw) return rcw; }
     TilePlan plan = tile_plan(env, in0.n, in0.n_sweeps, in0.offsets);
     if (plan.err) return fail(h, GEM_ERR_INVALID, plan.err == 1 ? "cloud too large" : "lowest tracking: the pass is too large for 16x16 tiles (cut it into smaller calls)");
     PassInput in = in0;
-    std::vector<gem_frame_params> cut_params;
-    std::vector<long long> cut_offsets;
-    std::vector<int> orig0;
+    struct CutSweeps { std::vector<gem_frame_params> params; std::vector<long long> offsets; std::vector<int> orig0; };
+    std::unique_ptr<CutSweeps> cut;
     if (plan.n_sweeps != in.n_sweeps) {
         const int ns = plan.n_sweeps;
-        if (in.src == 0) cut_params.assign(ns, *in.params);
-        cut_offsets.resize(ns + 1); orig0.resize(ns);
-        for (int s = 0; s <= ns; ++s) cut_offsets[s] = std::min<long long>(in.n, (long long)s * kSweepPoints);
-        for (int s = 0; s < ns; ++s) orig0[s] = (int)cut_offsets[s];
-        in.n_sweeps = ns; in.params = in.src == 0 ? cut_params.data() : nullptr; in.offsets = cut_offsets.data(); in.var_updates = nullptr; in.sweep_orig0 = orig0.data();
+        cut.reset(new CutSweeps);
+        if (in.src == 0) cut->params.assign(ns, *in.params);
+        cut->offsets.resize(ns + 1); cut->orig0.resize(ns);
+        for (int s = 0; s <= ns; ++s) cut->offsets[s] = std::min<long long>(in.n, (long long)s * kSweepPoints);
+        for (int s = 0; s < ns; ++s) cut->orig0[s] = (int)cut->offsets[s];
+        in.n_sweeps = ns; in.params = in.src == 0 ? cut->params.data() : nullptr; in.offsets = cut->offsets.data(); in.var_updates = nullptr; in.sweep_orig0 = cut->orig0.data();
     }
     const bool batched = in.n_sweeps > 1;
     const int U = kUnit, B = plan.B, bpad = plan.bpad;
@@ -366,7 +403,8 @@
     const bool defer = h->defer && in.device_input && in.src == 0 && !batched && (attr & 3) == 0 && ts == 4 && !overlap &&
                        !h->counting && (!h->dbg_on || h->dbg_frame);
     if (!defer) { const int rcd = flush_deferred(h); if (rcd) return rcd; }
-    gem_handle::PassBuffers& pb = h->pb[(overlap || defer) ? (h->pass++ & 1u) : 0u];
+    const unsigned set = (overlap || defer) ? (h->pass++ & 1u) : 0u;
+    gem_handle::PassBuffers& pb = h->pb[set];
     hipStream_t sbin = overlap ? h->bin_stream : h->stream;
     int rc;
     if ((rc = switch_to_bin_streams(h, overlap))) return rc;
@@ -427,7 +465,7 @@
     fa.counters = ba.counters;
     fa.srt = static_cast<uint4*>(pb.srt.p); fa.srt_top = ba.srt_top; fa.dense_min = h->dense_min;
     fa.lowest = h->layers.lowest; fa.start0 = h->start[0]; fa.start1 = h->start[1];
-    fa.count_per_pass = orig0.empty() ? 0 : 1;
+    fa.count_per_pass = cut && !cut->orig0.empty() ? 1 : 0;
     fa.dbg = nullptr;
     fa.dbg_sweep = h->dbg_sweep;
     if (h->dbg_on) {
@@ -445,6 +483,23 @@
         if (h->deferred.valid && h->deferred.attr != attr) { const int rcd = flush_deferred(h); if (rcd) return rcd; }
         const bool lean = frame_launch_lean(h, !h->deferred.valid || h->deferred.lean_binned, ba.frame0.fast_laser != 0 && !ba.rgb);
         ba.lean = lean ? 1 : 0;
+        if (check.on && lean && h->deferred.valid) {
+            check.done = true; ++h->frame_steady_hits;
+            h->frame_steady_mismatch += frame_block_mismatches(frame_lean_args(h->deferred.fa, ba), check.buf.la) + frame_block_mismatches(frame_lean_args(fa, ba), check.next.la);
+            const FrameLeanHead hd = frame_lean_head(check.buf.la);
+            const FuseArgs& nf = check.next.fa;
+            h->frame_steady_mismatch += (memcmp(&hd, &check.buf.head, sizeof hd) != 0) + (nf.epoch != fa.epoch) + (nf.xyzi != fa.xyzi) + (nf.n_pending != fa.n_pending) +
+                                        (nf.dense != fa.dense) + (memcmp(nf.pending, fa.pending, sizeof fa.pending) != 0) + (nf.bkt != fa.bkt) + (nf.bcount != fa.bcount) +
+                                        (nf.spill != fa.spill) + (nf.ctl != fa.ctl) + (check.next.grid != frame_tile_blocks(h->deferred.fa.T) + (unsigned)((ba.B + 3) / 4));
+        }
+        FrameSteady& st = h->steady[set];
+        st.valid = lean && h->frame_steady != 0;
+        if (st.valid) {
+            st.n = in.n; st.attr = attr; st.stream = h->stream; st.gen = h->steady_gen;
+            st.grid = (unsigned)(frame_tile_blocks(fa.T) + (ba.B + 3) / 4); st.fell_back = choice.fell_back;
+            st.la = frame_lean_args(fa, ba); st.fa = fa;
+            if (!check.on) ++h->frame_steady_misses;
+        }
         if (h->deferred.valid) { Timed t(h, 2); GEM_HIP(h, launch_frame(h->stream, h->deferred.fa, ba, attr, lean, t.events())); }
         else                   { Timed t(h, 0); GEM_HIP(h, launch_frame(h->stream, FuseArgs{}, ba, attr, lean, t.events())); }
         h->deferred.fa = fa; h->deferred.ts = ts; h->deferred.attr = attr; h->deferred.valid = true; h->deferred.lean_binned = lean;
@@ -469,6 +524,7 @@
     std::lock_guard<std::mutex> lk(h->mu);
     hipSetDevice(h->device);
     { const int rcd = settle(h); if (rcd) return rcd; }
+    steady_touch(h);
     if (max_points == 0) return GEM_OK;
     int rc;
     if ((rc = ensure(h, h->stage, std::max({cloud_layout(max_points, true, true).bytes, stage_words_bytes(max_points, 9), depth_stage_bytes(max_points)})))) return rc;
diff --git a/gem_amd/csrc/gem_frame_lean.hip b/gem_amd/csrc/gem_frame_lean.hip
--- a/gem_amd/csrc/gem_frame_lean.hip
+++ b/gem_amd/csrc/gem_frame_lean.hip
@@ -1,6 +1,9 @@
 #include "gem_frame_tile.hpp"
+#include "gem_frame_steady.hpp"
 
 #include <hip/hip_ext.h>
+
+#include <atomic>
 
 namespace gem {
 
@@ -75,4 +78,33 @@
     return hipGetLastError();
 }
 
+static hipFunction_t frame_lean_function(int device, int attr)
+{
+    constexpr int kDevices = 64;
+    static std::atomic<hipFunction_t> fn[2][kDevices];
+    static std::atomic<bool> failed[2][kDevices];
+    const int v = attr == 4 ? 1 : 0;
+    if (device < 0 || device >= kDevices) return nullptr;
+    hipFunction_t f = fn[v][device].load(std::memory_order_acquire);
+    if (f || failed[v][device].load(std::memory_order_relaxed)) return f;
+    const void* sym = v ? reinterpret_cast<const void*>(&k_frame<4, true>) : reinterpret_cast<const void*>(&k_frame<0, true>);
+    if (hipGetFuncBySymbol(&f, sym) != hipSuccess || !f) { (void)hipGetLastError(); failed[v][device].store(true); return nullptr; }
+    fn[v][device].store(f, std::memory_order_release);
+    return f;
 }
+
+hipError_t launch_frame_lean(hipStream_t st, int device, const FrameLaunchBuf& buf, int attr, unsigned blocks)
+{
+    if (hipFunction_t f = frame_lean_function(device, attr)) {
+        size_t size = sizeof(buf);
+        void* config[] = {HIP_LAUNCH_PARAM_BUFFER_POINTER, const_cast<FrameLaunchBuf*>(&buf), HIP_LAUNCH_PARAM_BUFFER_SIZE, &size, HIP_LAUNCH_PARAM_END};
+        return hipModuleLaunchKernel(f, blocks, 1, 1, 256, 1, 1, (unsigned)kFrameLds, st, nullptr, config);
+    }
+    const dim3 grid(blocks), block(256);
+    const FrameLeanHead& h = buf.head;
+    if (attr == 4) hipLaunchKernelGGL((k_frame<4, true>), grid, block, kFrameLds, st, h.nf, h.T, h.tiles_per_row, h.tile_div, h.center_tr, h.center_tc, h.bkt, h.bcount, h.xyzi, h.B, h.n, buf.la);
+    else           hipLaunchKernelGGL((k_frame<0, true>), grid, block, kFrameLds, st, h.nf, h.T, h.tiles_per_row, h.tile_div, h.center_tr, h.center_tc, h.bkt, h.bcount, h.xyzi, h.B, h.n, buf.la);
+    return hipGetLastError();
+}
+
+}
diff --git a/gem_amd/csrc/gem_frame_lean.hpp b/gem_amd/csrc/gem_frame_lean.hpp
--- a/gem_amd/csrc/gem_frame_lean.hpp
+++ b/gem_amd/csrc/gem_frame_lean.hpp
@@ -66,6 +66,18 @@
 
 __host__ __device__ inline int frame_tile_blocks(int T) { return (T + kFrameGridUnit - 1) & ~(kFrameGridUnit - 1); }
 
+inline void frame_lean_bin_frame(FrameLeanBin& b, const FrameConst& fc)
+{
+    b.filter_on = fc.filter_on;
+    for (int i = 0; i < 12; ++i) b.T[i] = fc.T[i];
+    b.lower_f = fc.lower_f; b.upper_f = fc.upper_f;
+    b.fbx = fc.fbx; b.fby = fc.fby; b.fband = fc.fband; b.fplane = fc.fplane;
+    b.cx = fc.cx; b.cy = fc.cy; b.sx = fc.sx; b.sy = fc.sy; b.L = fc.L; b.res = fc.res;
+    b.row0 = fc.row0; b.row1 = fc.row1;
+    b.beam_a = fc.beam_a; b.beam_c = fc.beam_c; b.t2 = fc.t2;
+    b.Js[0] = fc.Js[0]; b.Js[1] = fc.Js[1];
+}
+
 inline FrameLeanArgs frame_lean_args(const FuseArgs& fa, const BinArgs& ba)
 {
     FrameLeanArgs la{};
@@ -82,18 +94,10 @@
     t.dense = fa.dense; t.mahal = fa.mahal; t.var_floor = fa.var_floor;
     t.nspill = (uint32_t)fa.B_total * (uint32_t)fa.U;
     FrameLeanBin& b = la.b;
-    const FrameConst& fc = ba.frame0;
     b.xyzi = ba.xyzi; b.B = ba.B; b.n = (uint32_t)ba.n;
     b.keep_sentinel = ba.keep_sentinel; b.tile_bits = ba.tile_bits; b.tiles_per_row = ba.tiles_per_row;
-    b.filter_on = fc.filter_on;
     b.bkt = ba.bkt; b.bcount = ba.bcount; b.spill = ba.spill; b.ctl = ba.ctl; b.dbg = ba.dbg;
-    for (int i = 0; i < 12; ++i) b.T[i] = fc.T[i];
-    b.lower_f = fc.lower_f; b.upper_f = fc.upper_f;
-    b.fbx = fc.fbx; b.fby = fc.fby; b.fband = fc.fband; b.fplane = fc.fplane;
-    b.cx = fc.cx; b.cy = fc.cy; b.sx = fc.sx; b.sy = fc.sy; b.L = fc.L; b.res = fc.res;
-    b.row0 = fc.row0; b.row1 = fc.row1;
-    b.beam_a = fc.beam_a; b.beam_c = fc.beam_c; b.t2 = fc.t2;
-    b.Js[0] = fc.Js[0]; b.Js[1] = fc.Js[1];
+    frame_lean_bin_frame(b, ba.frame0);
     return la;
 }
 
diff --git a/gem_amd/csrc/gem_frame_steady.hpp b/gem_amd/csrc/gem_frame_steady.hpp
--- /dev/null
+++ b/gem_amd/csrc/gem_frame_steady.hpp
@@ -0,0 +1,162 @@
+#pragma once
+
+#include "../../include/gem_hip.h"
+#include "gem_frame_lean.hpp"
+
+#include <cmath>
+#include <cstddef>
+#include <cstring>
+
+namespace gem {
+
+struct FrameMapIn {
+    float cx, cy; int sx, sy, L; float res; int row0, row1;
+    bool  fast_laser;
+};
+
+struct FrameStatic { bool ok; float t2; };
+inline FrameStatic frame_static_proof(const FrameConst& f, bool laser_knob, bool have_params)
+{
+    FrameStatic s{false, 0.f};
+    if (!(have_params && f.model == GEM_MODEL_LASER && laser_knob)) return s;
+    const float min_r = (float)f.sp[0], vn = min_r * min_r;
+    const float c0 = f.Js[0] * 0.0f, c1 = f.Js[1] * 0.0f, c2 = f.Js[2] * vn;
+    const float b2 = c0 + (c1 + c2);
+    const float t2 = b2 * f.Js[2];
+    auto small = [](float v, float bound) { return std::isfinite(v) && std::fabs(v) <= bound; };
+    bool ok = t2 > 0.f && std::isfinite(t2) && small(f.beam_a, 1e6f) && small(f.beam_c, 1e6f);
+    for (int i = 0; i < 9; ++i) ok = ok && f.Q[i] == 0.0f && small(f.C[i], 1e6f) && small(f.Bs[i], 1e6f);
+    for (int i = 0; i < 3; ++i) ok = ok && small(f.Js[i], 1e6f) && small(f.P[i], 1e6f);
+    ok = ok && small(f.cx, 1e9f) && small(f.cy, 1e9f) && (double)f.L * (double)f.res <= 1e9;
+    ok = ok && f.res >= 9.5367431640625e-7f && f.res <= 1048576.0f && f.L >= 2;
+    s.ok = ok; s.t2 = t2;
+    return s;
+}
+inline bool frame_pose_proof(const FrameConst& f)
+{
+    auto small = [](float v, float bound) { return std::isfinite(v) && std::fabs(v) <= bound; };
+    bool ok = true;
+    for (int i = 0; i < 3 && ok; ++i)
+        for (int j = i; j < 3; ++j) {
+            double d = 0.0;
+            for (int k = 0; k < 3; ++k) d += (double)f.T[4 * i + k] * (double)f.T[4 * j + k];
+            ok = ok && std::fabs(d - (i == j ? 1.0 : 0.0)) <= 0.01;
+        }
+    for (int i = 0; i < 3; ++i) ok = ok && small(f.T[4 * i + 3], 1e9f);
+    return ok && std::isfinite(f.lower) && std::isfinite(f.upper) && std::fabs(f.lower) <= 1e9 && std::fabs(f.upper) <= 1e9;
+}
+inline void frame_set_pose(FrameConst& f, const gem_frame_params& p)
+{
+    for (int i = 0; i < 12; ++i) f.T[i] = p.T[i];
+    f.lower = p.lower; f.upper = p.upper;
+    f.lower_f = (float)p.lower; if ((double)f.lower_f > p.lower) f.lower_f = nextafterf(f.lower_f, -INFINITY);
+    f.upper_f = (float)p.upper; if ((double)f.upper_f < p.upper) f.upper_f = nextafterf(f.upper_f, INFINITY);
+}
+inline void frame_set_verdict(FrameConst& f, const FrameStatic& s, bool pose_ok)
+{
+    f.t2 = 0.f; f.fast_laser = 0;
+    if (s.ok && pose_ok) { f.t2 = s.t2; f.fast_laser = 1; }
+}
+
+inline FrameStatic fill_frame_from(const FrameMapIn& m, const gem_frame_params* p, FrameConst& f)
+{
+    memset(&f, 0, sizeof(f));
+    if (p) {
+        frame_set_pose(f, *p);
+        for (int i = 0; i < 8; ++i) f.sp[i] = p->sensor_params[i];
+        for (int i = 0; i < 3; ++i) { f.Js[i] = p->sensor_jacobian[i]; f.P[i] = p->P_mul_C_BM_T[i]; }
+        for (int i = 0; i < 9; ++i) { f.Q[i] = p->rotation_variance[i]; f.C[i] = p->C_SB_T[i]; f.Bs[i] = p->B_r_BS_skew[i]; }
+        f.filter_on = p->filter.enabled;
+        f.fbx = p->filter.box_x; f.fby = p->filter.box_y; f.fband = p->filter.band_y; f.fplane = p->filter.plane_y;
+        f.model = p->sensor_model;
+        f.orig_width = p->original_width;
+    }
+    f.cx = m.cx; f.cy = m.cy;
+    f.sx = m.sx; f.sy = m.sy;
+    f.L = m.L; f.res = m.res;
+    f.row0 = m.row0; f.row1 = m.row1;
+    f.beam_a = (float)f.sp[1]; f.beam_c = (float)f.sp[2];
+    const FrameStatic s = frame_static_proof(f, m.fast_laser, p != nullptr);
+    frame_set_verdict(f, s, s.ok && frame_pose_proof(f));
+    return s;
+}
+
+struct FrameConstCache {
+    bool valid = false;
+    gem_frame_params p;
+    FrameMapIn m;
+    FrameStatic s;
+    FrameConst fc;
+};
+constexpr size_t kFramePoseBytes = offsetof(gem_frame_params, sensor_model);
+static_assert(kFramePoseBytes == 16 * sizeof(float) + 2 * sizeof(double), "gem_frame_params: the transform and the window lead");
+inline const FrameConst& frame_const_cached(FrameConstCache& c, const FrameMapIn& m, const gem_frame_params& p)
+{
+    const unsigned char* pb = reinterpret_cast<const unsigned char*>(&p);
+    const unsigned char* cb = reinterpret_cast<const unsigned char*>(&c.p);
+    const bool same_map = c.valid && memcmp(&c.m.cx, &m.cx, sizeof(float)) == 0 && memcmp(&c.m.cy, &m.cy, sizeof(float)) == 0 && c.m.L == m.L &&
+                          memcmp(&c.m.res, &m.res, sizeof(float)) == 0 && c.m.fast_laser == m.fast_laser;
+    if (!same_map || memcmp(pb + kFramePoseBytes, cb + kFramePoseBytes, sizeof(gem_frame_params) - kFramePoseBytes) != 0) {
+        c.s = fill_frame_from(m, &p, c.fc);
+        memcpy(&c.p, &p, sizeof(p)); c.m = m; c.valid = true;
+        return c.fc;
+    }
+    if (memcmp(pb, cb, kFramePoseBytes) != 0) {
+        frame_set_pose(c.fc, p);
+        frame_set_verdict(c.fc, c.s, c.s.ok && frame_pose_proof(c.fc));
+        memcpy(&c.p, &p, kFramePoseBytes);
+    }
+    c.fc.sx = m.sx; c.fc.sy = m.sy; c.fc.row0 = m.row0; c.fc.row1 = m.row1;
+    c.m = m;
+    return c.fc;
+}
+
+struct FrameLaunchBuf { FrameLeanHead head; FrameLeanArgs la; };
+static_assert(offsetof(FrameLaunchBuf, head) == 0 && offsetof(FrameLeanHead, nf) == 0 && offsetof(FrameLeanHead, T) == 4 &&
+              offsetof(FrameLeanHead, tiles_per_row) == 8 && offsetof(FrameLeanHead, tile_div) == 12 && offsetof(FrameLeanHead, center_tr) == 16 &&
+              offsetof(FrameLeanHead, center_tc) == 20 && offsetof(FrameLeanHead, bkt) == 24 && offsetof(FrameLeanHead, bcount) == 32 &&
+              offsetof(FrameLeanHead, xyzi) == 40 && offsetof(FrameLeanHead, B) == 48 && offsetof(FrameLeanHead, n) == 52,
+              "the head of the launch buffer: every parameter at the offset the kernel's signature gives it");
+static_assert(offsetof(FrameLaunchBuf, la) == 4 * kFrameHeadDwords && alignof(FrameLeanArgs) == 8 && (4 * kFrameHeadDwords) % alignof(FrameLeanArgs) == 0 &&
+              sizeof(FrameLaunchBuf) == 4 * kFrameHeadDwords + sizeof(FrameLeanArgs),
+              "the launch buffer: the block follows the head dwords at its natural alignment, nothing behind it");
+
+struct FrameSteady {
+    bool valid = false;
+    long long n = 0; int attr = 0; hipStream_t stream = nullptr; unsigned long long gen = 0;
+    unsigned grid = 0;
+    bool fell_back = false;
+    FrameLeanArgs la{};
+    FuseArgs fa{};
+};
+
+struct FrameCallWords {
+    const float4* xyzi;
+    const FrameConst* fc;
+    uint32_t epoch;
+    int n_pending; const float* pending; int dense;
+};
+
+inline void frame_steady_patch(const FrameSteady& prev, FrameSteady& cur, const FrameCallWords& w, FrameLaunchBuf& out)
+{
+    cur.la.b.xyzi = w.xyzi;
+    frame_lean_bin_frame(cur.la.b, *w.fc);
+    out.la.t = prev.la.t; out.la.b = cur.la.b;
+    out.head = frame_lean_head(out.la);
+    FrameLeanTile& t = cur.la.t;
+    t.n_pending = w.n_pending; t.dense = w.dense;
+    cur.fa.n_pending = w.n_pending; cur.fa.dense = w.dense;
+    for (int i = 0; i < kMaxPending; ++i) { t.pending[i] = w.pending[i]; cur.fa.pending[i] = w.pending[i]; }
+    cur.fa.epoch = w.epoch; cur.fa.xyzi = w.xyzi;
+}
+
+inline int frame_block_mismatches(const FrameLeanArgs& a, const FrameLeanArgs& b)
+{
+    uint32_t wa[sizeof(FrameLeanArgs) / 4], wb[sizeof(FrameLeanArgs) / 4];
+    memcpy(wa, &a, sizeof a); memcpy(wb, &b, sizeof b);
+    int bad = 0;
+    for (size_t i = 0; i + 1 < sizeof(FrameLeanArgs) / 4; ++i) bad += wa[i] != wb[i];
+    return bad;
+}
+
+}
diff --git a/gem_amd/csrc/gem_kernels.hpp b/gem_amd/csrc/gem_kernels.hpp
--- a/gem_amd/csrc/gem_kernels.hpp
+++ b/gem_amd/csrc/gem_kernels.hpp
@@ -211,6 +211,8 @@
 hipError_t launch_fuse(hipStream_t st, const FuseArgs& a, int ts, int attr, int variant, LaunchEvents ev);
 hipError_t launch_frame(hipStream_t st, const FuseArgs& fuse_prev, const BinArgs& bin_this, int attr, bool lean, LaunchEvents ev);
 hipError_t launch_frame_lean(hipStream_t st, const FuseArgs& fuse_prev, const BinArgs& bin_this, int attr, unsigned blocks, LaunchEvents ev);
+struct FrameLaunchBuf;
+hipError_t launch_frame_lean(hipStream_t st, int device, const FrameLaunchBuf& head_and_block, int attr, unsigned blocks);
 size_t     fuse_lds_bytes(int ts, int variant, int attr);
 hipError_t launch_init(hipStream_t st, const LayerPtrs& m, int cells, int clear_lowest);
 hipError_t launch_unpack_aos(hipStream_t st, const void* src, int n, int step, int ox, int oy, int oz, int oi, int orgb, float4* xyzi, uint32_t* rgb);
```

Measured after the change: 25.24 billion, median of 3. Within noise of the previous version (+0.1%).
